# liuhatry/xflow

Hardware: AMD Instinct MI355X
Metric: samples/sec (whole node) + logloss, LR-FTRL Criteo-1TB shape at 1/2/4/8 MI355X (higher is better)
Workload: dtype fp32; 1 GPU; model=LR-FTRL, global_batch=262144, seq_len=39, parallelism=dp1+table-shard1, rows_per_gpu=262144, nnz_per_row=39, slices=1, grad_layout=unique_lr, hashed_features=1000000000, table_slots_per_gpu=2147483648, backend=hip:gfx950:0, a2a_transport=none, input_overlap=False, table_growths=0

## Files before the change

### csrc/engine/engine.cpp

```cpp
#include <cstdlib>
#include "xflow/engine.h"

#include <algorithm>
#include <atomic>
#include <chrono>
#include <cmath>
#include <cstdio>
#include <cstring>
#include <thread>
#include <fstream>
#include <stdexcept>
#include <string>

namespace xflow {

namespace {

uint64_t next_pow2(uint64_t v) {
  uint64_t p = 1;
  while (p < v) p <<= 1;
  return p;
}

constexpr char kMagic[8] = {'X', 'F', 'L', 'O', 'W', 'T', 'B', '1'};
// ... 252 lines not shown
}

void Engine::set_reduction(FwdArgs& fa) const {
  fa.trash_pos = (u32)scratch_.cap;
  if (!red_pairs_) return;
  if (rec_on_) fa.red_records = rec_count_;
  if (red_vmax_) {
    fa.red_vmax = red_vmax_ + vmax_parity_;
    fa.red_vmax_next = red_vmax_ + (vmax_parity_ ^ 1);
    fa.red_dup = red_vmax_ + 2 + vmax_parity_;
    fa.red_dup_next = red_vmax_ + 2 + (vmax_parity_ ^ 1);
    if (mdup_rec_) {
      fa.mdup.rec = mdup_rec_;
      fa.mdup.vmax = red_vmax_ + 4;
      fa.mdup.n = red_vmax_ + 6;
      fa.mdup.acc = mdup_acc_;
      fa.mdup.claim = mdup_claim_;
      fa.mdup.cap = (int64_t)mdup_claim_.capacity();
      fa.mdup.ew = mdup_ew_;
    }
    vmax_parity_ ^= 1;
  }
  fa.red_bcap = ws_->bcap;
  fa.red_cap = scratch_.cap;
  fa.red_nsub = red_nsub_;
  fa.red_pairs = red_pairs_;
  fa.red_sorted = red_sorted_;
  fa.red_sorted_words = (int64_t)red_sorted_.capacity();
  fa.red_hist = red_hist_;
  fa.red_tot = red_tot_;
  fa.red_count = red_count_;
  fa.red_groups = red_groups_;
  fa.red_nb = red_nb_;
  fa.red_maxb = red_maxb_;
  fa.red_rowv = red_rowv_;
}

PullArgs Engine::pull_args(const u64* keys, const int64_t* n_dev, int64_t n, bool insert,
                           u32* out_slot) const {
  PullArgs pa;
  pa.table = table_;
  pa.opt = cfg_.opt;
  pa.keys = keys;
  pa.n_dev = n_dev;
  pa.n_host = n_dev ? 0 : n;
  pa.n_max = n;
  pa.insert = insert;
  pa.out_slot = out_slot;
  return pa;
}

ApplyArgs Engine::apply_args(const u64* keys, const u32* slots, const int64_t* n_dev, int64_t n,
                             int S) const {
  ApplyArgs aa;
  aa.table = table_;
  aa.opt = cfg_.opt;
  aa.keys = keys;
  aa.slots = slots;
  aa.n_dev = n_dev;
  aa.n_host = n_dev ? 0 : n;
  aa.n_max = n;
  aa.S = S;
  aa.pstride = pstride();
  aa.P = cfg_.model.P();
  aa.fm_D = cfg_.model.v_dim;
  return aa;
}

FwdArgs Engine::train_fwd_args(const BatchView& b, const u32* pos, int S) const {
  FwdArgs fa;
  fa.batch = b;
  fa.pos = pos;
  fa.wpull = wpull_;
  fa.grad = grad_;
  fa.stats = stats_;
  fa.model = cfg_.model;
  fa.S = S;
  fa.fx_bad = overflow_;
  fa.fm_vals = fm_vals_;
  set_reduction(fa);
  return fa;
}

FwdArgs Engine::eval_fwd_args(const BatchView& b, float* pctr) const {
  FwdArgs fa;
  fa.batch = b;
  fa.pos = ws_->pos;
  fa.wpull = wpull_;
  fa.pctr = pctr;
  fa.stats = stats_ + 1;
  fa.model = cfg_.model;
  fa.fm_vals = fm_vals_;
  return fa;
}

int Engine::slices_of(const BatchView& b) const {
  if (b.slice_rows <= 0 || b.rows <= 0) return 1;
  return (int)((b.rows + b.slice_rows - 1) / b.slice_rows);
}

const int32_t* Engine::slice_rows_dev(const BatchView& b, int S) {
  if (b.rows == cached_rows_ && b.slice_rows == cached_slice_rows_ && S == cached_S_)
    return slice_rows_;
  const int ng = slice_groups(S);
  slice_rows_.reserve(*be_, (size_t)ng * kSliceGroup, (size_t)ng * kSliceGroup);
  const int64_t sr = b.slice_rows > 0 ? b.slice_rows : b.rows;
  for (int g = 0; g < ng; ++g) {
    int32_t h[kSliceGroup];
    const int n = ng == 1 ? S : kSliceGroup;
    for (int l = 0; l < n; ++l) {
      const int64_t s = (int64_t)g * kSliceGroup + l;
      int64_t rem = s < S ? b.rows - s * sr : 0;
      rem = rem < 0 ? 0 : rem;
      h[l] = (int32_t)(rem < sr ? (rem > 0 ? rem : 1) : sr);
    }
    be_->upload_small(slice_rows_ + (int64_t)g * kSliceGroup, h, sizeof(int32_t) * n);
  }
  cached_S_ = S;
  cached_rows_ = b.rows;
  cached_slice_rows_ = b.slice_rows;
  return slice_rows_;
}

BatchView Engine::group_view(const BatchView& b, int S, int k, const u32*& pos) const {
  if (slice_groups(S) == 1) return b;
  const int64_t sr = b.slice_rows > 0 ? b.slice_rows : b.rows;
  int64_t r0 = (int64_t)k * kSliceGroup * sr;
  r0 = r0 < b.rows ? r0 : b.rows;
  int64_t n = (int64_t)kSliceGroup * sr;
  n = n < b.rows - r0 ? n : b.rows - r0;
  BatchView g = b;
  g.rows = n;
  if (b.row_ptr) {
    g.row_ptr = b.row_ptr + r0;
    g.labels = b.labels + r0;
    return g;
  }
  const int64_t off = b.col_stride > 0 ? r0 : r0 * b.nnz_per_row;
  g.keys = b.keys + off;
  if (b.fgid) g.fgid = b.fgid + off;
  g.labels = b.labels + r0;
  g.nnz = n * b.nnz_per_row;
  pos += off;
  return g;
}

void Engine::ensure_inv() {
  if (ws_->inv) return;
  ws_->inv.alloc(*be_, scratch_.cap + 16);
  be_->memset(ws_->inv + scratch_.cap, 0xFF, 16 * sizeof(u32));
}

void Engine::dedup_(const BatchView& b, int parts, u64* uniq_keys_out, bool want_inv,
                    int64_t* n_copy, bool lead) {
  if (b.nnz > cfg_.max_nnz) throw std::invalid_argument("batch nnz exceeds max_nnz");
  if (b.rows > cfg_.max_rows) throw std::invalid_argument("batch rows exceed max_rows");
  if (b.col_stride > 0 && (b.row_ptr || b.col_stride < b.rows || b.nnz != b.rows * b.nnz_per_row))
    throw std::invalid_argument("field-major batch needs fixed nnz_per_row and col_stride >= rows");
  if (b.nnz == 0) {
    be_->memset(ws_->n_uniq, 0, sizeof(int64_t));
    return;
  }
  const int hb = be_->is_gpu() && parts == 1
                     ? table_.seg_log2 + table_.level + (table_.split > 0 ? 1 : 0)
                     : 0;
  if (parts != scratch_.parts || hb != scratch_.home_bits) {
    be_->fill_u64(scratch_.keys, kEmptyKey, scratch_.cap);
    be_->memset(scratch_.claims, 0, sizeof(unsigned long long));
    scratch_.parts = parts;
    scratch_.home_bits = hb;
  }
  if (++scratch_.epoch > kStampEpochs) {
    scratch_.epoch = 1;
    be_->memset(scratch_.stamps, 0, scratch_.cap);
    if (scratch_.ctl) {
      const unsigned long long z = 0ull;
      be_->upload_small(scratch_.ctl + 4, &z, sizeof(z));
    }
  }
  scratch_.grow = 0.0f;
  if (scratch_.ctl && nnz_seen_ > 0 && b.nnz > nnz_seen_)
    scratch_.grow = (float)((double)b.nnz / (double)nnz_seen_);
  if (b.nnz > nnz_seen_) nnz_seen_ = b.nnz;
  DedupOut o;
  o.pos = ws_->pos;
  o.uniq_keys = uniq_keys_out ? uniq_keys_out : uniq_keys_;
  o.uniq_pos = ws_->uniq_pos;
  o.n_uniq = ws_->n_uniq;
  o.overflow = overflow_;
  o.block_counts = block_counts_;
  o.inv = want_inv ? ws_->inv.get() : nullptr;
  o.n_uniq_copy = n_copy;
  o.cap_out = ws_->bcap;
  o.lead = lead;
  be_->dedup(b.keys, b.nnz, scratch_, o);
}


const char* grad_path_name(GradPath g) {
  switch (g) {
    case GradPath::kCsr: return "csr";
    case GradPath::kUniqueLR: return "unique_lr";
    case GradPath::kUniqueFmBC: return "unique_fm_bc";
    case GradPath::kUniqueRows: return "unique_rows";
    case GradPath::kSlotSums: return "slot_sums";
    case GradPath::kSlotRows: return "slot_rows";
  }
  return "?";
}

StepInputs Engine::step_inputs() const {
  StepInputs in;
  in.gpu = be_->is_gpu();
  in.remaps = be_->remaps_positions();
  in.red_pairs = red_pairs_ != nullptr;
  in.red_rowv = red_rowv_ != nullptr;
  in.fm_vals = fm_vals_;
  in.csr = cfg_.csr;
  in.sum_slices = cfg_.sum_slices;
  in.kind = cfg_.model.kind;
  in.fm_math = cfg_.model.fm_math;
  in.L = table_.L;
  in.scratch_cap = (double)scratch_.cap;
  in.max_nnz = (double)cfg_.max_nnz;
  in.max_rows = (double)cfg_.max_rows;
  in.pstride = pstride();
  in.slice_cap = slice_cap_;
  in.kdim = cfg_.model.kernel_dim();
  in.lead_handoff = cfg_.lead_handoff;
  in.red_rank = cfg_.red_rank;
  in.red_local = cfg_.red_local;
  in.red_apply = cfg_.red_apply;
  return in;
}

StepPlan plan_step(const StepInputs& in, int S) {
  constexpr double k32 = 4294967295.0;
  StepPlan p;
  p.S = S;
  const TableLayout& L = in.L;
  const bool lr16_slot = in.kind == kLR && L.lr16();
  const bool fm_std = in.kind == kFM && in.fm_math == kFmStandard;
  const bool mvm = in.kind == kMVM && in.kdim >= 2;
  const int vnv = fm_std ? 1 + in.kdim : in.kdim;
  const bool std_ok = (fm_std || mvm) && in.gpu && in.red_rowv &&
                      std::ceil(in.max_rows / fmstd_block(vnv - 1)) <= kSegMaxGroups;
  const int csr_min = (in.kind == kLR || fm_std) ? 8 : 4;
  if (in.csr && S >= csr_min && !in.sum_slices && in.red_pairs && in.remaps &&
      (lr16_slot || in.fm_vals || std_ok)) {
    int sl = 0;
    while ((1 << sl) < S) ++sl;
    const int nv = in.fm_vals ? 2 : (std_ok ? vnv : 1);
    if (sl <= red_shift(nv) && in.max_nnz * (double)(1 << sl) < k32) {
      p.csr_slog2 = sl;
      p.csr_rows = std_ok;
      p.grad = GradPath::kCsr;
      return p;
    }
  }
  p.groups = Engine::slice_groups(S);
  p.Sf = p.groups > 1 ? Engine::kSliceGroup : S;
  p.masks = p.Sf > 1 && !in.sum_slices;
  const bool lr16_ok = in.gpu && lr16_slot && in.red_pairs && in.scratch_cap < k32;
  p.upos = in.remaps && in.red_pairs &&
           (p.Sf > 1 || in.kind == kMVM || (in.kind == kFM && in.fm_math == kFmStandard));
  const double key_bound = p.upos ? in.max_nnz : in.scratch_cap;
  const bool red_masks = in.red_pairs && key_bound * in.slice_cap * in.pstride < k32 &&
                         (in.kind == kLR || in.kind == kFM ||
                          (in.kind == kMVM && in.red_rowv && in.kdim >= 2));
  p.lr16 = lr16_ok && (p.Sf == 1 || (p.masks && red_masks));
  p.lr16s = lr16_ok && p.Sf > 1 && !p.lr16;
  p.uqm = p.masks && red_masks;
  p.fmu = in.fm_vals && (p.Sf == 1 || p.uqm);
  p.fm_keep_w = in.fm_vals && p.groups > 1;
  const bool rows_ok = in.gpu && in.red_pairs && key_bound * in.pstride * in.slice_cap < k32;
  p.mvmu = rows_ok && p.Sf == 1 && in.kind == kMVM && in.red_rowv && in.kdim >= 2;
  p.fsu = rows_ok && (p.Sf == 1 || p.uqm) && in.kind == kFM && in.fm_math == kFmStandard;
  p.rowu = p.mvmu || p.fsu;
  p.grpst = in.gpu && L.opt == kFTRL && L.P > 1;
  p.uq = p.Sf > 1 && (p.lr16 || p.fmu || p.fsu);
  p.grad = p.lr16 ? GradPath::kUniqueLR
           : p.fmu ? GradPath::kUniqueFmBC
           : p.rowu ? GradPath::kUniqueRows
           : p.lr16s ? GradPath::kSlotSums
           : GradPath::kSlotRows;
  p.lead = in.lead_handoff && in.gpu && in.kind == kLR && S == 1 && in.red_pairs && !p.upos &&
           in.field_major && in.rows >= kLeadTile && std::fmod(in.rows, (double)kLeadTile) == 0.0 &&
           in.fields >= 1.0 && in.fields <= kLeadMaxFields && in.scratch_cap < 2147483648.0;
  p.red_rank = in.red_rank && in.gpu && S == 1 && in.red_pairs && !p.upos && (p.lr16 || p.fmu);
  p.red_local = in.red_local && p.lead;
  p.red_apply = in.red_apply && p.red_local && p.red_rank && p.lr16;
  return p;
}

void Engine::train_step_csr(const BatchView& b, int S, int slog2) {
  const int32_t* srows = slice_rows_dev(b, S);
  const bool fm = fm_vals_;
  const bool rows = csr_full_rows();
  const int ew = rows ? csr_row_words(table_.L.P) : 0;
  float* stash = fm || rows ? grp_nz_.ensure(*be_, 2 * (size_t)cfg_.max_nnz * table_.L.P)
                            : lr_nz_.ensure(*be_, 2 * (size_t)cfg_.max_nnz);
  PullArgs pa = begin_fused_step(b, true, true);
  pa.out_nz = stash;
  be_->table_pull(pa);

  csr_forward_backward(b, slog2, srows, true);

  ApplyArgs aa = apply_args(uniq_keys_, uniq_slot_, ws_->n_uniq, b.nnz, S);
  aa.fm_compact = fm;
  aa.nz_stash = stash;
  aa.csr_off = csr_off_;
  aa.csr_cnt = csr_cnt_;
  aa.csr_ent = rows ? static_cast<const void*>(csr_vent_.get()) : red_pairs_.get();
  aa.csr_ew = ew;
  aa.csr_long = S > 16 ? csr_long_list(b.nnz) : nullptr;
  aa.csr_long_cap = (int64_t)csr_long_.capacity();
  attach_snapshot(aa);
  be_->table_apply(aa);
  end_step();
}

void Engine::csr_forward_backward(const BatchView& b, int slog2, const int32_t* srows,
                                  bool normalise) {
  csr_off_.ensure(*be_, (size_t)cfg_.max_nnz);
  csr_cnt_.ensure(*be_, (size_t)cfg_.max_nnz);
  FwdArgs fa = train_fwd_args(b, ws_->pos, 1 << slog2);
  fa.agg_ok = true;
  fa.red_nuq = ws_->n_uniq;
  fa.fm_compact = fm_vals_;
  fa.red_csr.off = csr_off_;
  fa.red_csr.cnt = csr_cnt_;
  fa.red_csr.ent = red_pairs_;
  fa.red_csr.slog2 = slog2;
  fa.red_csr.rows = normalise ? srows : nullptr;
  if (csr_full_rows()) {
    const int ew = csr_row_words(table_.L.P);
    fa.red_csr.ent = csr_vent_.ensure(*be_, (size_t)cfg_.max_nnz * ew);
    fa.red_csr.P = table_.L.P;
    fa.red_csr.ew = ew;
  }
  be_->forward_backward(fa);
  ++csr_steps_;
}

u32* Engine::csr_long_list(int64_t n) {
  if (!be_->is_gpu()) return nullptr;
  const int64_t need = 2 * n + (int64_t)(2u << 20) + 4 * 65536;
  csr_long_.reserve(*be_, (size_t)need, (size_t)(need + n / 4));
  return csr_long_;
}

void Engine::w_forward_backward_csr(const BatchView& b, const float* pulled, int64_t n_send,
                                    int S_global, int wb, bool pack, u32* cnt_out, void* ent_out,
                                    const int64_t* counts, int world, bool encoded,
                                    int64_t* totals_out) {
  use_worker_set(wb);
  const int St = S_global > 0 ? S_global : slices_of(b);
  const int sl = csr_slog2(St);
  if (sl < 0 || St < slices_of(b) || St > cfg_.max_slices)
    throw std::invalid_argument("w_forward_backward_csr: S_global off the CSR path");
  if (b.nnz > 0 && !ws_->inv_valid)
    throw std::logic_error("w_forward_backward_csr: needs the partitioned dedup's inv");
  be_->remap_pos(ws_->pos, b.nnz, ws_->inv, (u32)scratch_.cap);
  be_->scatter_rows(pulled, wpull_, nullptr, nullptr, n_send, vstride_);
  csr_forward_backward(b, sl, slice_rows_dev(b, St), true);
  last_nsend_ = n_send;
  if (!pack) return;
  csr_doff_.ensure(*be_, (size_t)cfg_.max_nnz + 1);
  be_->scan_u32(csr_cnt_, csr_doff_, ws_->n_uniq, cfg_.max_nnz);
  be_->csr_pack(csr_off_, csr_cnt_, csr_full_rows() ? static_cast<const void*>(csr_vent_.get()) : red_pairs_.get(),
                csr_doff_, ws_->n_uniq, cfg_.max_nnz, ent_out, csr_entry_bytes());
  be_->copy_d2d(cnt_out, csr_cnt_, sizeof(u32) * (size_t)n_send);
  be_->csr_totals(counts, world, encoded, csr_doff_, totals_out);
}

template <typename Source>
void Engine::apply_by_source(const ApplyArgs& base, const std::vector<int64_t>& src_offsets,
                             int buf, bool stash, const char* need_weights, Source source) {
  const SrvBuf& sb = srv_[buf];
  size_t first_src = 0;
  while (first_src + 1 < src_offsets.size() && src_offsets[first_src + 1] <= src_offsets[first_src])
    ++first_src;
  for (size_t src = 0; src + 1 < src_offsets.size(); ++src) {
    const int64_t o = src_offsets[src], c = src_offsets[src + 1] - o;
    if (c <= 0) continue;
    ApplyArgs aa = base;
    aa.keys = base.keys + o;
    aa.slots = base.slots + o;
    aa.n_host = c;
    aa.n_max = c;
    source(aa, o, c);
    if (aa.fm_compact) {
      aa.pulled = pulled_weights(buf, o);
      if (!aa.pulled && src > first_src) throw std::logic_error(need_weights);
    }
    if (stash) aa.nz_stash = sb.nz + 2 * o;
    stash = false;
    attach_snapshot(aa);
    be_->table_apply(aa);
  }
}

void Engine::s_apply_csr(const u64* recv_keys, const u32* recv_cnt, const void* recv_ent,
                         const std::vector<int64_t>& src_offsets, int S, int buf) {
  if (buf < 0 || buf >= kSrvBufs) throw std::invalid_argument("server buffer must be in [0, kSrvBufs)");
  SrvBuf& sb = srv_[buf];
  sb.keys = nullptr;
  bool stash = sb.nz_fresh;
  stale_stashes();
  const u32* off = csr_off_;
  const u32* cnt = csr_cnt_;
  const void* ent = csr_full_rows() ? static_cast<const void*>(csr_vent_.get()) : red_pairs_.get();
  const int64_t n = src_offsets.empty() ? 0 : src_offsets.back();
  if (n > sb.n) throw std::invalid_argument("s_apply_csr: offsets beyond pull");
  mark_stale_buffer(sb, recv_keys, n);
  if (recv_cnt) {
    csr_roff_.reserve(*be_, (size_t)n + 1, (size_t)(n + n / 4 + 1024));
    be_->scan_u32(recv_cnt, csr_roff_, nullptr, n);
    off = csr_roff_;
    cnt = recv_cnt;
    ent = recv_ent;
  }
  ApplyArgs base = apply_args(recv_keys, sb.slots, nullptr, 0, S);
  base.fm_compact = fm_vals_;
  base.csr_ew = csr_full_rows() ? csr_row_words(table_.L.P) : 0;
  base.csr_ent = ent;
  apply_by_source(base, src_offsets, buf, stash,
                  "s_apply_csr: compact FM rows of several sources need s_pull's weights",
                  [&](ApplyArgs& aa, int64_t o, int64_t c) {
                    aa.csr_off = off + o;
                    aa.csr_cnt = cnt + o;
                    aa.csr_long = S > 16 ? csr_long_list(c) : nullptr;
                    aa.csr_long_cap = (int64_t)csr_long_.capacity();
                  });
}

void Engine::csr_debug(std::vector<u32>& off, std::vector<u32>& cnt, std::vector<u32>& words) {
  off.clear();
  cnt.clear();
  words.clear();
  if (!csr_off_) return;
  const int64_t n = n_unique();
  off.resize((size_t)n);
  cnt.resize((size_t)n);
  be_->copy_d2h(off.data(), csr_off_, sizeof(u32) * (size_t)n);
  be_->copy_d2h(cnt.data(), csr_cnt_, sizeof(u32) * (size_t)n);
  u64 end = 0;
  for (int64_t i = 0; i < n; ++i) end = std::max<u64>(end, (u64)off[i] + cnt[i]);
  const bool rows = csr_vent_ && csr_full_rows();
  const int w = rows ? csr_row_words(table_.L.P) : csr_entry_bytes() / 4;
  words.resize((size_t)end * w);
  if (end) be_->copy_d2h(words.data(), rows ? static_cast<const void*>(csr_vent_.get()) : red_pairs_.get(),
                         sizeof(u32) * (size_t)end * w);
}

std::vector<u64> Engine::unique_keys() {
  std::vector<u64> k((size_t)n_unique());
  if (!k.empty()) be_->copy_d2h(k.data(), uniq_keys_, sizeof(u64) * k.size());
  return k;
}

Engine::RedGeometry Engine::red_geometry(int S, int64_t nuq) {
  RedGeometry g;
  const bool fm_std = cfg_.model.kind == kFM && cfg_.model.fm_math == kFmStandard;
  const bool mvm = cfg_.model.kind == kMVM && cfg_.model.kernel_dim() >= 2;
  const int kd = cfg_.model.kernel_dim();
  const int nv = fm_vals_ ? 2 : (fm_std ? 1 + kd : (mvm ? kd : 1));
  int sl = 0;
  while ((1 << sl) < S) ++sl;
  g.base = red_shift(nv);
  g.maxb = red_maxb_ > 0 ? red_maxb_ : kRedMaxBuckets;
  g.nsub = red_nsub_;
  g.nb = red_nb_;
  g.nuq = nuq >= 0 ? nuq : n_unique();
  const u64 dests = (u64)g.nuq << sl;
  int sh = g.base;
  while (((dests + (1ull << sh) - 1) >> sh) > (u64)kRedMaxBuckets) ++sh;
  if (g.maxb > kRedMaxBuckets && sh - g.base >= 2)
    while (sh > g.base && ((dests + (1ull << (sh - 1)) - 1) >> (sh - 1)) <= (u64)g.maxb) --sh;
  const int min_shift = csr_full_rows() ? kCsrVecMinShift : 0;
  g.shift = sh < min_shift ? min_shift : sh;
  const u64 n = (dests + (1ull << g.shift) - 1) >> g.shift;
  g.needed = (int64_t)n;
  g.buckets = n < (u64)g.nb ? (int)n : g.nb;
  return g;
}

void Engine::train_step(const BatchView& b) {
  stale_stashes();
  use_worker_set(0);
  const int S = slices_of(b);
  if (S > cfg_.max_slices) throw std::invalid_argument("batch has more slices than max_slices");
  if (cfg_.sum_slices && slice_groups(S) > 1)
    throw std::invalid_argument("sum_slices: at most 32 slices per step (ordered pushes: any count)");
  const StepPlan P = plan(S, b.rows, b.nnz_per_row, !b.row_ptr && b.col_stride > 0 && b.col_stride == b.rows);
  if (P.grad == GradPath::kCsr) {
    train_step_csr(b, S, P.csr_slog2);
    return;
  }
  const int ng = P.groups;
  const int ps = pstride();
  const bool masks = P.masks;
  const int32_t* srows = slice_rows_dev(b, S);
  const bool uqm = P.uqm, fm_keep_w = P.fm_keep_w, uq = P.uq, upos = P.upos;
  const double key_bound = upos ? (double)cfg_.max_nnz : (double)scratch_.cap;
  struct {
    float* buf = nullptr;
    int width = 0;
    bool normalised = false;
    bool pull_zeroes = true;
  } uo;
  const size_t un = (size_t)cfg_.max_nnz;
  if (P.red_apply) {
    uo = {nullptr, 1, true, false};
  } else if (P.lr16) {
    uo = {lr_grad_.ensure(*be_, un * slice_cap_), 1, true, true};
  } else if (P.fmu) {
    uo = {fm_grad_.ensure(*be_, 2 * un * slice_cap_), 2, true, true};
  } else if (P.rowu) {
    uo = {row_grad_.ensure(*be_, un * ps * (P.fsu ? slice_cap_ : 1)), ps, false,
          !(P.fsu && P.Sf == 1)};
  }
  float* nz = P.lr16 || P.lr16s ? lr_nz_.ensure(*be_, 2 * un)
              : P.grpst         ? grp_nz_.ensure(*be_, 2 * un * table_.L.P)
                                : nullptr;
  if (fm_keep_w) fm_w_.ensure(*be_, un * ps);
  if (uq) lr_mask_.ensure(*be_, un);

  PullArgs pa = begin_fused_step(b, upos || (uo.buf && !P.red_rank), upos, P.lead);
  if (fm_keep_w) pa.out_w = fm_w_;
  pa.out_nz = nz;
  if (uo.buf && uo.pull_zeroes) {
    pa.zero_out = uo.buf;
    pa.zero_width = uo.width;
  }
  if (uq) {
    pa.zero_out = reinterpret_cast<float*>(lr_mask_.get());
    pa.zero_width = 1;
  }
  be_->table_pull(pa);

  for (int k = 0; k < ng; ++k) {
    const u32* posk = ws_->pos;
    const BatchView bk = group_view(b, S, k, posk);
    const int Sg = group_slices(S, k);
    const int32_t* srk = srows + (int64_t)k * kSliceGroup;
    const bool stash = k == 0;

    FwdArgs fa = train_fwd_args(bk, posk, Sg);
    fa.agg_ok = key_bound * Sg * ps < 4294967295.0;
    if (upos) fa.red_nuq = ws_->n_uniq;
    fa.lead = P.lead;
    fa.red_local = P.red_local;
    if (uq) fa.red_masks = lr_mask_;
    else if (uqm) fa.red_masks = tmask_;
    else if (masks) be_->slice_masks(bk, posk, tmask_);
    fa.fm_compact = fa.red_pairs && fa.agg_ok && cfg_.model.kind == kFM &&
                    cfg_.model.fm_math == kFmReference;
    if (fm_vals_ && !fa.fm_compact) throw std::logic_error("train_step: compact FM rows need the reduction");
    if (uo.buf || P.red_apply) {
      fa.red_out = uo.buf;
      fa.red_inv = upos || P.red_rank ? nullptr : ws_->inv.get();
      if (P.red_rank) {
        fa.red_rank_offs = block_counts_;
        fa.red_rank_stamps = scratch_.stamps;
        fa.red_rank_epoch = scratch_.epoch;
      }
      if (uo.normalised) fa.red_rows = srk;
    }
    if (P.red_apply) {
      fa.red_apply_words = table_.words;
      fa.red_apply_slots = uniq_slot_;
      fa.red_apply_nz = nz;
      fa.red_apply_ftrl = cfg_.opt.ftrl;
      attach_snapshot(fa, b.nnz);
    }
    be_->forward_backward(fa);
    if (P.red_apply) continue;

    ApplyArgs aa = apply_args(uniq_keys_, uniq_slot_, ws_->n_uniq, b.nnz, Sg);
    aa.sum_slices = cfg_.sum_slices;
    aa.fm_compact = fa.fm_compact;
    if (fm_keep_w) aa.pulled = fm_w_;
    aa.nz_stash = stash ? nz : nullptr;
    if (uo.buf) {
      aa.grads = uo.buf;
      aa.gstride = uo.width;
      aa.slice_rows = uo.normalised ? nullptr : srk;
    } else {
      aa.grads = grad_;
      aa.grad_map = upos ? nullptr : ws_->uniq_pos.get();
      aa.zero_after = true;
      aa.slice_rows = srk;
    }
    if (uq) {
      aa.masks = lr_mask_;
      aa.masks_clear = k + 1 < ng;
    } else if (masks) {
      aa.masks = tmask_;
      aa.masks_rw = tmask_;
    }
    attach_snapshot(aa);
    be_->table_apply(aa);
  }
  end_step();
}

PullArgs Engine::begin_fused_step(const BatchView& b, bool want_inv, bool upos, bool lead) {
  if (want_inv) ensure_inv();
  if (lead && upos) throw std::logic_error("begin_fused_step: leader handoff with unique positions");
  dedup_(b, 1, nullptr, want_inv, nullptr, lead);
  ws_->inv_valid = false;
  if (upos) be_->remap_pos(ws_->pos, b.nnz, ws_->inv, (u32)scratch_.cap);
  guard_inserts(b.nnz);
  delta_mark(uniq_keys_, ws_->n_uniq, b.nnz);
  PullArgs pa = pull_args(uniq_keys_, ws_->n_uniq, b.nnz, true, uniq_slot_);
  pa.admit = admit_;
  pa.out_vals = wpull_;
  pa.out_map = upos ? nullptr : ws_->uniq_pos.get();
  pa.pstride = pstride();
  pa.fm_vals = fm_vals_;
  return pa;
}

void Engine::eval_step(const BatchView& b, float* pctr) {
  use_worker_set(0);
  dedup_(b);
  PullArgs pa = pull_args(uniq_keys_, ws_->n_uniq, b.nnz, false, uniq_slot_);
  pa.out_vals = wpull_;
  pa.out_map = ws_->uniq_pos;
  pa.pstride = pstride();
  pa.fm_vals = fm_vals_;
  be_->table_pull(pa);
  be_->forward_backward(eval_fwd_args(b, pctr));
}

void Engine::ensure_host_staging(int64_t n) {
  if (!host_keys_dev_.reserve(*be_, (size_t)n, (size_t)n)) return;
  host_vals_dev_.alloc(*be_, (size_t)n * cfg_.model.P());
  host_slots_dev_.alloc(*be_, (size_t)n);
}

void Engine::push_host(const std::vector<u64>& keys, const std::vector<float>& grads) {
  stale_stashes();
  const int64_t n = (int64_t)keys.size();
  const int P = cfg_.model.P();
  if ((int64_t)grads.size() != n * P) throw std::invalid_argument("push_host: grads != keys*P");
  if (n == 0) return;
  guard_inserts(n);
  ensure_host_staging(n);
  be_->copy_h2d(host_keys_dev_, keys.data(), sizeof(u64) * n);
  be_->copy_h2d(host_vals_dev_, grads.data(), sizeof(float) * n * P);
  delta_mark(host_keys_dev_, nullptr, n);
  be_->table_pull(pull_args(host_keys_dev_, nullptr, n, true, host_slots_dev_));
  ApplyArgs aa = apply_args(host_keys_dev_, host_slots_dev_, nullptr, 1, 1);
  aa.pstride = P;
  for (int64_t i = 0; i < n; ++i) {
    aa.slots = host_slots_dev_ + i;
    aa.grads = host_vals_dev_ + i * P;
    be_->table_apply(aa);
  }
  be_->synchronize();
}

void Engine::prefill(int64_t n, uint64_t seed) {
  if (n > 0) guard_inserts(n);
  if (n < 0 || (uint64_t)n > table_.cap - table_.cap / 16)
    throw std::invalid_argument("prefill: at most 15/16 of the table's slots");
  stale_stashes();
  if (n > 0) delta_needs_full_ = true;
  be_->table_prefill(table_, n, seed);
  be_->synchronize();
  (void)table_size();
}

std::vector<float> Engine::pull_host(const std::vector<u64>& keys) {
  const int64_t n = (int64_t)keys.size();
  const int P = cfg_.model.P();
  std::vector<float> out((size_t)n * P);
  if (n == 0) return out;
  ensure_host_staging(n);
  be_->copy_h2d(host_keys_dev_, keys.data(), sizeof(u64) * n);
  PullArgs pa = pull_args(host_keys_dev_, nullptr, n, false, host_slots_dev_);
  pa.out_vals = host_vals_dev_;
  pa.pstride = P;
  be_->table_pull(pa);
  be_->copy_d2h(out.data(), host_vals_dev_, sizeof(float) * n * P);
  return out;
}

void Engine::w_prepare(const BatchView& b, int world, int64_t* counts_out, u64* send_keys_out,
                       int wb, int64_t seq) {
  if (be_->partitioned_dedup() && (world < 1 || world > kMaxParts))
    throw std::runtime_error("w_prepare: world size " + std::to_string(world) + " outside [1, " +
                             std::to_string(kMaxParts) + "]");
  if (world <= 1) seq = -1;
  use_worker_set(wb);
  if (slices_of(b) > cfg_.max_slices)
    throw std::invalid_argument("batch has more slices than max_slices");
  if (b.nnz == 0) {
    const int64_t c = b.rows == 0 ? -1 : 0;
    be_->fill_u64(reinterpret_cast<u64*>(counts_out), (u64)(seq >= 0 ? encode_count(c, seq) : c),
                  (size_t)(world > 0 ? world : 1));
    be_->memset(ws_->n_uniq, 0, sizeof(int64_t));
    ws_->inv_valid = false;
    ws_->send_map = ws_->uniq_pos;
    return;
  }
  if (be_->partitioned_dedup()) {
    if (red_pairs_ && (cfg_.model.kind == kLR || fm_vals_ || csr_full_rows())) ensure_inv();
    dedup_(b, world, send_keys_out, true, world == 1 ? counts_out : nullptr);
    ws_->inv_valid = ws_->inv != nullptr;
    if (world > 1) be_->partition_counts(scratch_, block_counts_, ws_->n_uniq, counts_out, seq);
    ws_->send_map = ws_->uniq_pos;
    return;
  }
  dedup_(b);
  ws_->inv_valid = false;
  BucketArgs ba;
  ba.uniq_keys = uniq_keys_;
  ba.uniq_pos = ws_->uniq_pos;
  ba.n_dev = ws_->n_uniq;
  ba.n_max = b.nnz;
  ba.world = world;
  ba.counts = counts_out;
  ba.send_keys = send_keys_out;
  ba.send_pos = ws_->send_pos;
  ba.scratch = bucket_ws_;
  ba.seq = seq;
  be_->bucket(ba);
  ws_->send_map = ws_->send_pos;
}

void Engine::ensure_server_capacity(int64_t n, int buf) {
  if (buf < 0 || buf >= kSrvBufs) throw std::invalid_argument("server buffer must be in [0, kSrvBufs)");
  SrvBuf& sb = srv_[buf];
  const size_t cap = (size_t)(n + n / 4 + 1024);
  if (n <= 0 || !sb.slots.reserve(*be_, (size_t)n, cap)) return;
  if (lr16_layout()) sb.nz.alloc(*be_, 2 * cap);
}

bool Engine::lr16_layout() const {
  const TableLayout& L = table_.L;
  return be_->is_gpu() && L.lr16();
}

void Engine::w_forward(const BatchView& b, const float* pulled, int64_t n_send, float* pctr,
                       int wb) {
  use_worker_set(wb);
  be_->scatter_rows(pulled, wpull_, ws_->send_map, nullptr, n_send, vstride_);
  be_->forward_backward(eval_fwd_args(b, pctr));
}

void Engine::s_pull(const u64* recv_keys, int64_t n, float* out_vals, bool insert, int buf,
                    const std::vector<int64_t>& src_offsets, bool keep_weights) {
  ensure_server_capacity(n, buf);
  SrvBuf& sb = srv_[buf];
  sb.n = n;
  sb.vals = out_vals;
  sb.w_valid = false;
  sb.grp = SrcGroups();
  sb.keys = insert && n > 0 ? recv_keys : nullptr;
  if (n == 0) return;
  if (insert) {
    guard_inserts(n);
    group_entries(recv_keys, n, buf, src_offsets);
    delta_mark(recv_keys, nullptr, n);
  }
// ... 800 lines not shown
```

### csrc/hip/hip_backend.hip

```cpp
#include <hip/hip_runtime.h>

#include <cstdlib>
#include <cstring>
#include <vector>

#include "hip_util.h"
#include "kernels.h"
#include "xflow/backend.h"

namespace xflow {

namespace {

class HipBackend final : public Backend {
 public:
  explicit HipBackend(int device) : device_(device) {
    XF_HIP_CHECK(hipSetDevice(device_));
    XF_HIP_CHECK(hipStreamCreateWithFlags(&own_stream_, hipStreamNonBlocking));
    stream_ = own_stream_;
    XF_HIP_CHECK(hipMalloc(&counter_, sizeof(unsigned long long)));
  }
  ~HipBackend() override {
    hipSetDevice(device_);
    if (copy_stream_) (void)hipStreamSynchronize(copy_stream_);
// ... 7 lines not shown
    if (scan_tiles_) {
      (void)hipDeviceSynchronize();
      (void)hipFreeAsync(scan_tiles_, own_stream_);
      (void)hipStreamSynchronize(own_stream_);
    }
    if (split_marks_) (void)hipFree(split_marks_);
    if (own_stream_) (void)hipStreamDestroy(own_stream_);
  }

  void stage_begin(int s) override {
    if (!copy_stream_) {
      XF_HIP_CHECK(hipStreamCreateWithFlags(&copy_stream_, hipStreamNonBlocking));
      for (int i = 0; i < 2; ++i) {
        XF_HIP_CHECK(hipEventCreateWithFlags(&ev_copied_[i], hipEventDisableTiming));
        XF_HIP_CHECK(hipEventCreateWithFlags(&ev_used_[i], hipEventDisableTiming));
      }
    }
    if (copied_pending_[s]) {
      XF_HIP_CHECK(hipEventSynchronize(ev_copied_[s]));
      copied_pending_[s] = false;
    }
    waited_used_[s] = false;
  }
  void* stage_pinned(int s, size_t bytes) override {
    if (bytes > pinned_cap_[s]) {
      if (pinned_[s]) XF_HIP_CHECK(hipHostFree(pinned_[s]));
      pinned_cap_[s] = bytes + bytes / 4;
      XF_HIP_CHECK(hipHostMalloc(&pinned_[s], pinned_cap_[s], hipHostMallocDefault));
    }
    return pinned_[s];
  }
  void stage_copy(int s, void* dst, size_t off, size_t bytes) override {
    if (!bytes) return;
    if (used_pending_[s] && !waited_used_[s]) {
      XF_HIP_CHECK(hipStreamWaitEvent(copy_stream_, ev_used_[s], 0));
      waited_used_[s] = true;
    }
    XF_HIP_CHECK(hipMemcpyAsync(dst, static_cast<char*>(pinned_[s]) + off, bytes,
                                hipMemcpyHostToDevice, copy_stream_));
  }
  void stage_commit(int s) override {
    XF_HIP_CHECK(hipEventRecord(ev_copied_[s], copy_stream_));
    XF_HIP_CHECK(hipStreamWaitEvent(stream_, ev_copied_[s], 0));
    copied_pending_[s] = true;
  }
  void stage_release(int s) override {
    XF_HIP_CHECK(hipEventRecord(ev_used_[s], stream_));
    used_pending_[s] = true;
  }

  bool is_gpu() const override { return true; }
  std::string name() const override { return "hip:gfx950:" + std::to_string(device_); }

  void* alloc(size_t bytes) override {
    void* p = nullptr;
    if (bytes == 0) bytes = 16;
    XF_HIP_CHECK(hipSetDevice(device_));
    XF_HIP_CHECK(hipMalloc(&p, bytes));
    return p;
  }
  void free(void* p) override {
    if (p) (void)hipFree(p);
  }
  void* alloc_stream(size_t bytes) override {
    void* p = nullptr;
    if (bytes == 0) bytes = 16;
    XF_HIP_CHECK(hipSetDevice(device_));
    XF_HIP_CHECK(hipMallocAsync(&p, bytes, stream_));
    return p;
  }
  void free_stream(void* p) override {
    if (p) XF_HIP_CHECK(hipFreeAsync(p, stream_));
  }
  void memset(void* p, int v, size_t bytes) override {
    if (bytes) XF_HIP_CHECK(hipMemsetAsync(p, v, bytes, stream_));
  }
  void fill_u64(u64* p, u64 v, size_t n) override { hip::launch_fill_u64(p, v, n, stream_); }
  void copy_h2d(void* dst, const void* src, size_t bytes) override {
    if (bytes) XF_HIP_CHECK(hipMemcpyAsync(dst, src, bytes, hipMemcpyHostToDevice, stream_));
    XF_HIP_CHECK(hipStreamSynchronize(stream_));
  }
  void copy_d2h(void* dst, const void* src, size_t bytes) override {
    if (bytes) XF_HIP_CHECK(hipMemcpyAsync(dst, src, bytes, hipMemcpyDeviceToHost, stream_));
    XF_HIP_CHECK(hipStreamSynchronize(stream_));
  }
  void copy_d2h_async(void* dst, const void* src, size_t bytes) override {
    if (bytes) XF_HIP_CHECK(hipMemcpyAsync(dst, src, bytes, hipMemcpyDeviceToHost, stream_));
  }
  void copy_h2d_async(void* dst, const void* src, size_t bytes) override {
    if (bytes) XF_HIP_CHECK(hipMemcpyAsync(dst, src, bytes, hipMemcpyHostToDevice, stream_));
  }
  void* staging_alloc(size_t bytes) override {
    void* p = nullptr;
    XF_HIP_CHECK(hipHostMalloc(&p, bytes ? bytes : 16, hipHostMallocDefault));
    return p;
  }
  void staging_free(void* p) override {
    if (p) (void)hipHostFree(p);
  }
  void copy_d2d(void* dst, const void* src, size_t bytes) override {
    if (bytes) XF_HIP_CHECK(hipMemcpyAsync(dst, src, bytes, hipMemcpyDeviceToDevice, stream_));
  }
  void download_small(void* dst, const void* src, size_t bytes) override {
    hip::launch_download_small(dst, src, bytes, stream_);
  }
  void upload_small(void* dst, const void* src, size_t bytes) override {
    hip::launch_upload_small(dst, src, bytes, stream_);
  }
  void synchronize() override { XF_HIP_CHECK(hipStreamSynchronize(stream_)); }
  size_t free_memory() const override {
    size_t fr = 0, tot = 0;
    XF_HIP_CHECK(hipSetDevice(device_));
    XF_HIP_CHECK(hipMemGetInfo(&fr, &tot));
    return fr;
  }
  void snapshot(HostSnap* dst, const u32* mon, unsigned long long seq) override {
    hip::launch_snapshot(dst, mon, seq, stream_);
  }
  void* host_alloc(size_t bytes) override {
    void* p = nullptr;
    XF_HIP_CHECK(hipHostMalloc(&p, bytes ? bytes : 16, hipHostMallocCoherent));
    std::memset(p, 0, bytes ? bytes : 16);
    return p;
  }
  void host_free(void* p) override {
    if (p) (void)hipHostFree(p);
  }
  void* event_create() override {
    hipEvent_t e = nullptr;
    XF_HIP_CHECK(hipEventCreateWithFlags(&e, hipEventDisableTiming));
    return e;
  }
  void event_destroy(void* e) override {
    if (e) (void)hipEventDestroy(static_cast<hipEvent_t>(e));
  }
  void event_record(void* e) override {
    XF_HIP_CHECK(hipEventRecord(static_cast<hipEvent_t>(e), stream_));
  }
  bool event_done(void* e) override {
    const hipError_t r = hipEventQuery(static_cast<hipEvent_t>(e));
    if (r == hipErrorNotReady) return false;
    XF_HIP_CHECK(r);
    return true;
  }
  void set_stream(void* s) override { stream_ = reinterpret_cast<hipStream_t>(s); }
  void* stream() const override { return stream_; }
  void bind_thread() override { XF_HIP_CHECK(hipSetDevice(device_)); }

  void table_clear(const TableView& t) override { hip::launch_table_clear(t, stream_); }
  void dedup(const u64* keys, int64_t nnz, ScratchView s, DedupOut o) override {
    hip::launch_dedup(keys, nnz, s, o, stream_);
  }
  void table_pull(const PullArgs& a) override { hip::launch_table_pull(a, stream_); }
  void table_apply(const ApplyArgs& a) override { hip::launch_table_apply(a, stream_); }
  void forward_backward(const FwdArgs& a) override { hip::launch_forward_backward(a, stream_); }
  void slice_masks(const BatchView& b, const u32* pos, u32* tmask) override {
    hip::launch_slice_masks(b, pos, tmask, stream_);
  }
  void parse_text(const TextParseArgs& a) override { hip::launch_parse_text(a, stream_); }
  bool remaps_positions() const override { return true; }
  void remap_pos(u32* pos, int64_t nnz, const u32* inv, u32 none) override {
    hip::launch_remap_pos(pos, nnz, inv, none, stream_);
  }
  void bucket(const BucketArgs&) override {
    throw std::logic_error("bucket: not on the HIP backend");
  }
  bool partitioned_dedup() const override { return true; }
  void partition_counts(const ScratchView& s, const u32* chunk_offsets, const int64_t* n_uniq,
                        int64_t* counts, int64_t seq) override {
    hip::launch_partition_counts(s, chunk_offsets, n_uniq, counts, seq, stream_);
  }
  bool owner_grouping() const override { return true; }
  void owner_group(const OwnerGroupArgs& a) override { hip::launch_owner_group(a, stream_); }
  void gather_grads(const GatherGradArgs& a) override { hip::launch_gather_grads(a, stream_); }
  bool csr_exchange() const override { return true; }
  void scan_u32(const u32* in, u32* out, const int64_t* n_dev, int64_t n_max) override {
    const size_t words = (size_t)(n_max / 4096 + 4);
    if (words > scan_tiles_words_) {
      if (scan_tiles_) free_stream(scan_tiles_);
      scan_tiles_words_ = words + words / 2;
      scan_tiles_ = static_cast<u32*>(alloc_stream(scan_tiles_words_ * sizeof(u32)));
    }
    hip::launch_scan_u32(in, out, n_dev, n_max, scan_tiles_, stream_);
  }
  void csr_pack(const u32* off, const u32* cnt, const void* src, const u32* doff,
                const int64_t* n_dev, int64_t n_max, void* dst, int entry_bytes) override {
    hip::launch_csr_pack(off, cnt, src, doff, n_dev, n_max, dst, entry_bytes, stream_);
  }
  void csr_totals(const int64_t* counts, int world, bool encoded, const u32* doff,
                  int64_t* totals) override {
    hip::launch_csr_totals(counts, world, encoded, doff, totals, stream_);
  }
  void scatter_rows(const float* src, float* dst, const u32* map, const int64_t* n_dev,
                    int64_t n_max, int width, float* zero_out, int zero_width) override {
    hip::launch_scatter_rows(src, dst, map, n_dev, n_max, width, zero_out, zero_width, stream_);
  }
  void synth_batch(const SynthArgs& a) override { hip::launch_synth(a, stream_); }
  void unpack_block(const UnpackArgs& a) override { hip::launch_unpack_block(a, stream_); }
  void field_major(const void* src, void* dst, int64_t rows, int F, int elem_bytes,
                   bool widen) override {
    hip::launch_field_major(src, dst, rows, F, elem_bytes, widen, stream_);
  }
  void shuffle_rows(const ShuffleArgs& a) override {
    check_shuffle_args(a);
    if (!a.src.row_ptr) {
      hip::launch_shuffle_fixed(a, stream_);
      return;
    }
    if (a.src.rows <= 0) {
      memset(a.row_ptr, 0, sizeof(int32_t));
      return;
    }
    if (!a.len) throw std::invalid_argument("shuffle_rows: a CSR batch needs the len workspace");
    hip::launch_shuffle_len(a, stream_);
    scan_u32(a.len, reinterpret_cast<u32*>(a.row_ptr), nullptr, a.src.rows);
    hip::launch_shuffle_gather(a, stream_);
  }
  void cross_rows(const CrossArgs& a) override {
    check_cross_args(a);
    if (a.src.row_ptr) hip::launch_cross_csr(a, stream_);
    else if (a.src.col_stride > 0) hip::launch_cross_cols(a, stream_);
    else hip::launch_cross_fixed(a, stream_);
  }
  int64_t table_export(const TableView& t, u64* keys_out, u32* words_out,
                       int64_t max_rows) override {
    hip::launch_table_export(t, keys_out, words_out, max_rows, counter_, stream_);
    unsigned long long n = 0;
    copy_d2h(&n, counter_, sizeof(n));
    return (int64_t)n;
  }
  void table_import(const TableView& t, const u64* keys, const u32* words, int64_t n) override {
    hip::launch_table_import(t, keys, words, n, stream_);
  }
  void table_prefill(const TableView& t, int64_t n, u64 seed) override {
    hip::launch_table_prefill(t, n, seed, stream_);
  }
  void table_split(const TableView& t, u64 s0, u64 k) override {
    ensure_marks(t, k);
    hip::launch_table_split(t, s0, k, split_marks_, stream_);
  }
  void table_prune(const TableView& t, const OptSpec& o, float max_n,
                   unsigned long long* dropped) override {
    const int g = t.seg_log2;
    const u64 nseg = t.cap >> g;
    const u64 per_launch = g >= 28 ? 1 : (1ull << (28 - g));
    XF_HIP_CHECK(hipMemsetAsync(counter_, 0, sizeof(unsigned long long), stream_));
    for (u64 s0 = 0; s0 < nseg; s0 += per_launch) {
      const u64 k = nseg - s0 < per_launch ? nseg - s0 : per_launch;
      ensure_marks(t, k);
      hip::launch_table_prune(t, o, max_n, s0, k, split_marks_, counter_, stream_);
    }
    hip::launch_table_prune_finish(t.size, dropped, counter_, stream_);
  }

  void* table_reserve(size_t max_bytes, bool growable) override {
    int vmm = 0;
    XF_HIP_CHECK(hipSetDevice(device_));
    (void)hipDeviceGetAttribute(&vmm, hipDeviceAttributeVirtualMemoryManagementSupported, device_);
    const char* env = std::getenv("XFLOW_TABLE_VMM");
    if ((env && env[0] == '0') || !growable) vmm = 0;
    vm_on_ = false;
    if (vmm) {
      vm_prop_ = hipMemAllocationProp{};
      vm_prop_.type = hipMemAllocationTypePinned;
      vm_prop_.location.type = hipMemLocationTypeDevice;
      vm_prop_.location.id = device_;
      size_t gran = 0;
      if (hipMemGetAllocationGranularity(&gran, &vm_prop_, hipMemAllocationGranularityRecommended) ==
              hipSuccess && gran > 0) {
        vm_gran_ = gran;
        vm_max_ = (max_bytes + gran - 1) / gran * gran;
        void* p = nullptr;
        if (hipMemAddressReserve(&p, vm_max_, gran, nullptr, 0) == hipSuccess) {
          vm_on_ = true;
          vm_base_ = p;
          vm_committed_ = 0;
          return p;
        }
      }
      (void)hipGetLastError();
    }
    fb_bytes_ = 0;
    fb_max_ = max_bytes;
    return nullptr;
  }
  void* table_commit(void* base, size_t bytes) override {
    if (vm_on_) {
      if (bytes <= vm_committed_) return base;
      if (bytes > vm_max_) throw std::runtime_error("xflow: table beyond its reserved range");
      size_t want = (bytes + vm_gran_ - 1) / vm_gran_ * vm_gran_;
      size_t ahead = (vm_committed_ / 8 + vm_gran_ - 1) / vm_gran_ * vm_gran_;
      if (vm_committed_ && want < vm_committed_ + ahead) want = vm_committed_ + ahead;
      if (want > vm_max_) want = vm_max_;
      {
        size_t fr = 0, tot = 0;
        if (hipMemGetInfo(&fr, &tot) == hipSuccess && want - vm_committed_ + (512u << 20) > fr)
          want = (bytes + vm_gran_ - 1) / vm_gran_ * vm_gran_;
      }
      const size_t add = want - vm_committed_;
      char* at = static_cast<char*>(vm_base_) + vm_committed_;
      hipMemGenericAllocationHandle_t h;
      XF_HIP_CHECK(hipMemCreate(&h, add, &vm_prop_, 0));
      XF_HIP_CHECK(hipMemMap(at, add, 0, h, 0));
      hipMemAccessDesc acc{};
      acc.location = vm_prop_.location;
      acc.flags = hipMemAccessFlagsProtReadWrite;
// ... 130 lines not shown
```

### csrc/hip/kernels.h

```cpp
#pragma once

#include <hip/hip_runtime.h>

#include "xflow/backend.h"

namespace xflow {
namespace hip {

void launch_dedup(const u64* keys, int64_t nnz, ScratchView s, DedupOut o, hipStream_t st);
void launch_remap_pos(u32* pos, int64_t nnz, const u32* inv, u32 none, hipStream_t st);
void launch_partition_counts(const ScratchView& s, const u32* chunk_offsets,
                             const int64_t* n_uniq, int64_t* counts, int64_t seq, hipStream_t st);

void launch_table_pull(const PullArgs& a, hipStream_t st);

void launch_table_apply(const ApplyArgs& a, hipStream_t st);
void launch_owner_group(const OwnerGroupArgs& a, hipStream_t st);

void launch_gather_grads(const GatherGradArgs& a, hipStream_t st);
void launch_scatter_rows(const float* src, float* dst, const u32* map, const int64_t* n_dev,
                         int64_t n_max, int width, float* zero_out, int zero_width,
                         hipStream_t st);
void launch_scan_u32(const u32* in, u32* out, const int64_t* n_dev, int64_t n_max, u32* tiles,
                     hipStream_t st);
void launch_csr_pack(const u32* off, const u32* cnt, const void* src, const u32* doff,
                     const int64_t* n_dev, int64_t n_max, void* dst, int entry_bytes,
                     hipStream_t st);
void launch_csr_totals(const int64_t* counts, int world, bool encoded, const u32* doff,
                       int64_t* totals, hipStream_t st);

void launch_fill_u64(u64* p, u64 v, size_t n, hipStream_t st);
void launch_upload_small(void* dst, const void* src, size_t bytes, hipStream_t st);
void launch_download_small(void* host_dst, const void* src, size_t bytes, hipStream_t st);
void launch_snapshot(HostSnap* dst, const u32* mon, unsigned long long seq, hipStream_t st);
void launch_table_clear(const TableView& t, hipStream_t st);
void launch_table_export(const TableView& t, u64* keys_out, u32* words_out, int64_t max_rows,
                         unsigned long long* counter, hipStream_t st);
void launch_table_import(const TableView& t, const u64* keys, const u32* words, int64_t n,
                         hipStream_t st);
void launch_table_prefill(const TableView& t, int64_t n, u64 seed, hipStream_t st);
void launch_table_split(const TableView& t, u64 s0, u64 k, u64* marks, hipStream_t st);
void launch_table_prune(const TableView& t, const OptSpec& o, float max_n, u64 s0, u64 k,
                        u64* marks, unsigned long long* count, hipStream_t st);
void launch_table_prune_finish(unsigned long long* size, unsigned long long* total,
                               const unsigned long long* count, hipStream_t st);
void launch_table_nonzero(const TableView& t, const OptSpec& o, unsigned long long* counter,
                          hipStream_t st);
void launch_delta_mark(u32* bits, int L, const u64* keys, const int64_t* n_dev, int64_t n_host,
                       int64_t n_max, hipStream_t st);
void launch_table_export_marked(const TableView& t, const u32* bits, int L, u64* keys_out,
                                u32* words_out, int64_t max_rows, unsigned long long* counter,
                                hipStream_t st);
void launch_delta_popcount(const u32* bits, int L, unsigned long long* counter, hipStream_t st);

void launch_unpack_block(const UnpackArgs& a, hipStream_t st);
void launch_field_major(const void* src, void* dst, int64_t rows, int F, int elem_bytes, bool widen,
                        hipStream_t st);

void launch_shuffle_fixed(const ShuffleArgs& a, hipStream_t st);
void launch_shuffle_len(const ShuffleArgs& a, hipStream_t st);
void launch_shuffle_gather(const ShuffleArgs& a, hipStream_t st);

void launch_cross_fixed(const CrossArgs& a, hipStream_t st);
void launch_cross_cols(const CrossArgs& a, hipStream_t st);
void launch_cross_csr(const CrossArgs& a, hipStream_t st);

void launch_forward_backward(const FwdArgs& a, hipStream_t st);
void launch_slice_masks(const BatchView& b, const u32* pos, u32* tmask, hipStream_t st);

void launch_parse_text(const TextParseArgs& a, hipStream_t st);

void launch_eval_metrics(const float* pctr, const float* labels, int64_t n, EvalMetrics* out,
                         hipStream_t st);
void launch_eval_grouped(const float* pctr, const float* labels, const u64* groups, int64_t n,
                         GroupedEval* out, GroupTable* table, hipStream_t st);
void launch_row_group_keys(const BatchView& b, int field, u64* out, hipStream_t st);

void launch_synth(const SynthArgs& a, hipStream_t st);

}
}
```

### csrc/hip/kernels_dedup.hip

```cpp
#include "table_common.h"

namespace xflow {
namespace hip {

__device__ __forceinline__ u64 active_cap(const ScratchView& sv) {
  return sv.ctl ? (u64)sv.ctl[0] : sv.cap;
}

__device__ __forceinline__ u64 batch_cap(const ScratchView& sv) {
  return sv.ctl ? (u64)sv.ctl[3] : sv.cap;
}

__device__ __forceinline__ bool batch_spilled(const ScratchView& sv) {
  return sv.ctl && sv.ctl[4] == (unsigned long long)sv.epoch;
}

__global__ void k_scratch_maybe_clear(u64* __restrict__ skeys, u64 cap,
                                      const unsigned long long* __restrict__ claims,
                                      u64 rebuild_at, const unsigned long long* __restrict__ ctl) {
  u64 n = cap;
  if (ctl) {
    n = ctl[2];
    if (n == 0) return;
  } else if (*claims <= rebuild_at) {
    return;
  }
  const u64 stride = (u64)gridDim.x * blockDim.x;
  for (u64 s = (u64)blockIdx.x * blockDim.x + threadIdx.x; s < n; s += stride)
    skeys[s] = kEmptyKey;
}

__global__ void k_scratch_claims_reset(unsigned long long* claims, u64 rebuild_at,
                                       unsigned long long* ctl) {
  if (ctl) {
    if (ctl[2]) {
      ctl[0] = ctl[2];
      ctl[2] = 0ull;
      *claims = 0ull;
    }
  } else if (*claims > rebuild_at) {
    *claims = 0ull;
  }
}

__global__ void k_scratch_grow(unsigned long long* __restrict__ ctl, u64 cap_alloc, float grow) {
  const double need = (double)kScratchHeadroom * (double)ctl[1] * (double)grow;
  u64 want = kScratchMinCap;
  while ((double)want < need && want < cap_alloc) want <<= 1;
  if (want > cap_alloc) want = cap_alloc;
  ctl[2] = want > ctl[0] ? want : 0ull;
}

constexpr int kDedupItems = 4;
constexpr int kDedupChunk = kBlock * kDedupItems;
constexpr int kDedupLog2 = 11;
static_assert((1 << kDedupLog2) == 2 * kDedupChunk, "LDS dedup table sizing");
static_assert(kDedupChunk == kLeadTile, "the handoff's tile is the dedup chunk");

template <bool kLead>
__global__ void __launch_bounds__(kBlock) k_dedup_insert(const u64* __restrict__ keys, int64_t nnz,
                                                         ScratchView sv, u32* __restrict__ pos,
                                                         u32* __restrict__ overflow) {
  constexpr u32 kL = 1u << kDedupLog2;
  __shared__ u64 t_key[kL];
  u64* __restrict__ skeys = sv.keys;
  const u64 cap = active_cap(sv), mask = cap - 1;
  const u32 parts = (u32)sv.parts;
  const u64 R = parts > 1 ? cap / parts : cap;
  const int clog = 63 - __clzll((long long)cap);
  const int hshift = sv.home_bits > clog ? sv.home_bits - clog : 0;
  const int64_t base = (int64_t)blockIdx.x * kDedupChunk + threadIdx.x;
  for (u32 i = threadIdx.x; i < kL; i += kBlock) t_key[i] = kEmptyKey;
  u64 k[kDedupItems], s[kDedupItems];
  u32 h[kDedupItems];
#pragma unroll
  for (int j = 0; j < kDedupItems; ++j) {
    int64_t i = base + (int64_t)j * kBlock;
    k[j] = i < nnz ? sanitize_key(keys[i]) : 0ull;
    const u64 f = fmix64(k[j]);
    s[j] = parts > 1 ? (u64)((u32)(f >> 32) % parts) * R + (((f & 0xffffffffull) * R) >> 32)
                     : (f >> hshift) & mask;
    h[j] = (u32)(f >> (64 - kDedupLog2));
  }
  __syncthreads();
  u32 lead = 0;
#pragma unroll
  for (int j = 0; j < kDedupItems; ++j) {
    if (base + (int64_t)j * kBlock >= nnz) continue;
    u32 x = h[j];
    while (true) {
      const u64 prev = atomicCAS((unsigned long long*)&t_key[x], (unsigned long long)kEmptyKey,
                                 (unsigned long long)k[j]);
      if (prev == kEmptyKey) {
        lead |= 1u << j;
        break;
      }
      if (prev == k[j]) break;
      x = (x + 1) & (kL - 1);
    }
    h[j] = x;
  }
  __syncthreads();
  u64 cur[kDedupItems];
#pragma unroll
  for (int j = 0; j < kDedupItems; ++j) cur[j] = (lead >> j) & 1u ? skeys[s[j]] : k[j];
  unsigned int claimed = 0;
#pragma unroll
  for (int j = 0; j < kDedupItems; ++j) {
    if (!((lead >> j) & 1u)) continue;
    u64 sj = s[j], c = cur[j];
    u64 n = 0;
    while (c != k[j]) {
      if (c == kEmptyKey) {
        u64 prev = atomicCAS((unsigned long long*)&skeys[sj], (unsigned long long)kEmptyKey,
                             (unsigned long long)k[j]);
        if (prev == kEmptyKey) {
          ++claimed;
          break;
        }
        if (prev == k[j]) break;
      }
      if (++n >= R) {
        if (sv.ctl && parts == 1 && cap < sv.cap && n == R) {
          sv.ctl[4] = sv.epoch;
          const u64 Z = sv.cap - cap;
          sj = cap + fmix64(k[j]) % Z;
          c = skeys[sj];
          for (u64 m = 0; c != k[j]; ) {
            if (c == kEmptyKey) {
              u64 prev = atomicCAS((unsigned long long*)&skeys[sj], (unsigned long long)kEmptyKey,
                                   (unsigned long long)k[j]);
              if (prev == kEmptyKey) {
                ++claimed;
                break;
              }
              if (prev == k[j]) break;
            }
            if (++m >= Z) {
              sj = sv.cap;
              break;
            }
            if (++sj == sv.cap) sj = cap;
            c = skeys[sj];
          }
          if (sj < sv.cap) break;
        }
        *overflow = 1u;
        sj = sv.cap;
        break;
      }
      if (parts > 1) {
        ++sj;
        if (sj % R == 0) sj -= R;
      } else {
        sj = (sj + 1) & mask;
      }
      c = skeys[sj];
    }
    XF_DASSERT(sj <= sv.cap);
    if constexpr (kLead) {
      XF_DASSERT(sj < kLeadBit);
      t_key[h[j]] = sj | ((u64)(j * kBlock + (int)threadIdx.x) << 32);
    } else {
      t_key[h[j]] = sj;
    }
    if (sj < sv.cap) sv.stamps[sj] = (unsigned char)sv.epoch;
  }
  __syncthreads();
#pragma unroll
  for (int j = 0; j < kDedupItems; ++j) {
    int64_t i = base + (int64_t)j * kBlock;
    if (i >= nnz) continue;
    const u64 e = t_key[h[j]];
    if constexpr (kLead) pos[i] = (lead >> j) & 1u ? (u32)e : kLeadBit | (u32)(e >> 32);
    else pos[i] = (u32)e;
  }
  block_count_add<kBlock>(sv.claims, claimed);
}

constexpr int kCompactItems = 16;
constexpr int kCompactChunk = kBlock * kCompactItems;
static_assert(kCompactChunk == 1 << kCompactChunkLog2, "k_red_sum ranks slots by these chunks");

__device__ __forceinline__ unsigned int compact_hits(const ScratchView& sv, u64 base, u64 cap,
                                                     unsigned int& cnt) {
  unsigned int hit = 0;
  cnt = 0;
  if (base >= cap) return 0;
  const uint4 q = *reinterpret_cast<const uint4*>(sv.stamps + base);
  const u32 w[4] = {q.x, q.y, q.z, q.w};
  const u32 e = sv.epoch & 0xFFu;
#pragma unroll
  for (int j = 0; j < 16; ++j) hit |= (unsigned int)(((w[j >> 2] >> (8 * (j & 3))) & 0xFFu) == e) << j;
  cnt = __popc(hit);
  return hit;
}

__global__ void __launch_bounds__(kBlock) k_compact_count(ScratchView sv,
                                                          unsigned int* __restrict__ counts) {
  const u64 base = (u64)blockIdx.x * kCompactChunk + (u64)threadIdx.x * kCompactItems;
  unsigned int cnt;
  compact_hits(sv, base, batch_spilled(sv) ? sv.cap : active_cap(sv), cnt);
  unsigned int tot;
  block_exclusive_scan<kBlock>(cnt, &tot);
  if (threadIdx.x == 0) counts[blockIdx.x] = tot;
}

constexpr u64 kCarryRebuildEighths = 3;
static_assert(kCarryRebuildEighths <= 4, "stale claims <= cur / 2 at a batch start");

__global__ void __launch_bounds__(kScanBlock) k_compact_scan(
    unsigned int* __restrict__ counts, int nb, unsigned long long* __restrict__ n_out,
    unsigned long long* __restrict__ claims, unsigned long long* __restrict__ ctl,
    u64 cap_alloc, unsigned long long* __restrict__ n_copy,
    unsigned long long* __restrict__ cap_out, u32 epoch, bool carry_on) {
  if (ctl) {
    const u64 lim = ctl[4] == epoch ? cap_alloc : (u64)ctl[0];
    const u64 nbl = (lim + kCompactChunk - 1) / kCompactChunk;
    if (nbl < (u64)nb) nb = (int)nbl;
  }
  unsigned long long carry = 0;
  for (int c0 = 0; c0 < nb; c0 += kScanBlock) {
    int i = c0 + (int)threadIdx.x;
    unsigned int v = i < nb ? counts[i] : 0u;
    unsigned int tot;
    unsigned int ex = block_exclusive_scan<kScanBlock>(v, &tot);
    if (i < nb) counts[i] = (unsigned int)(carry + ex);
    carry += tot;
  }
  if (threadIdx.x == 0) {
    *n_out = carry;
    if (n_copy) *n_copy = carry;
    if (ctl) {
      const u64 mx = ctl[1] > carry ? ctl[1] : carry;
      ctl[1] = mx;
      u64 want = kScratchMinCap;
      while (want < kScratchHeadroom * mx && want < cap_alloc) want <<= 1;
      if (want > cap_alloc) want = cap_alloc;
      const u64 cur = ctl[0];
      const bool resize = want > cur || want * 4 <= cur;
      const u64 full_at = carry_on ? cur * kCarryRebuildEighths / 8 : cur / 2;
      const bool rebuild = *claims > full_at || resize;
      const bool keep = carry_on && rebuild && !resize && ctl[4] != epoch &&
                        carry * kScratchHeadroom <= cur;
      ctl[3] = cur;
      ctl[2] = rebuild ? want : 0ull;
      ctl[5] = keep ? 1ull : 0ull;
      if (rebuild) {
        ctl[0] = want;
        *claims = keep ? carry : 0ull;
        ctl[6] += 1ull;
        ctl[7] = keep ? carry : 0ull;
      }
    }
    if (cap_out) *cap_out = ctl && ctl[4] != epoch ? ctl[3] : cap_alloc;
  }
}

__global__ void __launch_bounds__(kBlock) k_compact_write(ScratchView sv,
                                                          const unsigned int* __restrict__ offs,
                                                          u64* __restrict__ uk,
                                                          u32* __restrict__ up,
                                                          u32* __restrict__ inv) {
  const u64 base = (u64)blockIdx.x * kCompactChunk + (u64)threadIdx.x * kCompactItems;
  unsigned int cnt;
  unsigned int hit = compact_hits(sv, base, batch_spilled(sv) ? sv.cap : batch_cap(sv), cnt);
  unsigned int tot;
  unsigned int ex = block_exclusive_scan<kBlock>(cnt, &tot);
  unsigned long long dst = (unsigned long long)offs[blockIdx.x] + ex;
  u32 iv[kCompactItems];
  u64 kv[kCompactItems];
  if (hit) {
    const ulonglong2* kp = reinterpret_cast<const ulonglong2*>(sv.keys + base);
#pragma unroll
    for (int q = 0; q < kCompactItems / 2; ++q) {
      const ulonglong2 v = kp[q];
      kv[2 * q] = v.x;
      kv[2 * q + 1] = v.y;
    }
  }
#pragma unroll
  for (int j = 0; j < kCompactItems; ++j) {
    iv[j] = 0xFFFFFFFFu;
    if (!(hit & (1u << j))) continue;
    u64 s = base + (u64)j;
    uk[dst] = kv[j];
    up[dst] = (u32)s;
    iv[j] = (u32)dst;
    ++dst;
  }
  if (inv && hit) {
    uint4* ip = reinterpret_cast<uint4*>(inv + base);
#pragma unroll
    for (int j = 0; j < kCompactItems / 4; ++j)
      ip[j] = make_uint4(iv[4 * j], iv[4 * j + 1], iv[4 * j + 2], iv[4 * j + 3]);
  }
  const u64 fresh = sv.ctl ? (u64)sv.ctl[2] : 0ull;
  if (base < fresh) {
    ulonglong2* kp = reinterpret_cast<ulonglong2*>(sv.keys + base);
    if (hit && sv.ctl[5]) {
#pragma unroll
      for (int j = 0; j < kCompactItems / 2; ++j)
        kp[j] = make_ulonglong2(hit & (1u << (2 * j)) ? kv[2 * j] : kEmptyKey,
                                hit & (1u << (2 * j + 1)) ? kv[2 * j + 1] : kEmptyKey);
    } else {
#pragma unroll
      for (int j = 0; j < kCompactItems / 2; ++j) kp[j] = make_ulonglong2(kEmptyKey, kEmptyKey);
    }
  }
}

constexpr int kRemapPer = 4;

__global__ void __launch_bounds__(kBlock) k_remap_pos(u32* __restrict__ pos, int64_t nnz,
                                                      const u32* __restrict__ inv, u32 none) {
  const int64_t i = ((int64_t)blockIdx.x * kBlock + threadIdx.x) * kRemapPer;
  auto map = [&](u32 u) { return u == 0xFFFFFFFFu ? none : u; };
  if (i + kRemapPer <= nnz) {
    uint4 p[kRemapPer / 4];
#pragma unroll
    for (int q = 0; q < kRemapPer / 4; ++q) p[q] = reinterpret_cast<const uint4*>(pos + i)[q];
    u32 u[kRemapPer];
#pragma unroll
    for (int q = 0; q < kRemapPer / 4; ++q) {
      u[4 * q] = inv[p[q].x];
      u[4 * q + 1] = inv[p[q].y];
      u[4 * q + 2] = inv[p[q].z];
      u[4 * q + 3] = inv[p[q].w];
    }
#pragma unroll
    for (int q = 0; q < kRemapPer / 4; ++q)
      reinterpret_cast<uint4*>(pos + i)[q] =
          make_uint4(map(u[4 * q]), map(u[4 * q + 1]), map(u[4 * q + 2]), map(u[4 * q + 3]));
  } else {
    for (int64_t j = i; j < nnz; ++j) pos[j] = map(inv[pos[j]]);
  }
}

void launch_remap_pos(u32* pos, int64_t nnz, const u32* inv, u32 none, hipStream_t st) {
  if (nnz <= 0) return;
  if (reinterpret_cast<uintptr_t>(pos) & 15) throw std::runtime_error("remap_pos: pos must be 16-byte aligned");
  const int64_t lanes = (nnz + kRemapPer - 1) / kRemapPer;
  hipLaunchKernelGGL(k_remap_pos, dim3((unsigned)((lanes + kBlock - 1) / kBlock)), dim3(kBlock), 0,
                     st, pos, nnz, inv, none);
  XF_HIP_CHECK(hipGetLastError());
}

constexpr int kPartBlock = 1024;

__global__ void __launch_bounds__(kPartBlock) k_partition_counts(
    ScratchView sv, const unsigned int* __restrict__ offs, const int64_t* __restrict__ n_uniq,
    int64_t* __restrict__ counts, int64_t seq) {
  __shared__ int64_t start[kMaxParts + 1];
  const u32 parts = (u32)sv.parts;
  const u64 R = batch_cap(sv) / parts;
  const int lane = threadIdx.x % kWave, w = threadIdx.x / kWave;
  for (u32 o = w; o <= parts; o += kPartBlock / kWave) {
    if (o == 0 || o == parts) {
      if (lane == 0) start[o] = o == 0 ? 0 : *n_uniq;
      continue;
    }
    const u64 b = (u64)o * R, c = b / kCompactChunk, c0 = c * kCompactChunk;
    unsigned int hits = 0;
    for (u64 q = c0 + (u64)lane * 64; q < c0 + (u64)lane * 64 + 64; ++q)
      hits += (q < b && sv.stamps[q] == (unsigned char)sv.epoch) ? 1u : 0u;
#pragma unroll
    for (int d = 32; d > 0; d >>= 1) hits += __shfl_xor(hits, d);
    if (lane == 0) start[o] = (int64_t)offs[c] + hits;
  }
  __syncthreads();
  for (u32 o = threadIdx.x; o < parts; o += kPartBlock) {
    XF_DASSERT(start[o + 1] >= start[o]);
    const int64_t c = start[o + 1] - start[o];
    counts[o] = seq >= 0 ? encode_count(c, seq) : c;
  }
}

void launch_partition_counts(const ScratchView& s, const u32* chunk_offsets,
                             const int64_t* n_uniq, int64_t* counts, int64_t seq, hipStream_t st) {
  if (s.parts < 2 || s.parts > kMaxParts) throw std::runtime_error("partition_counts: bad parts");
  hipLaunchKernelGGL(k_partition_counts, dim3(1), dim3(kPartBlock), 0, st, s, chunk_offsets,
                     n_uniq, counts, seq);
  XF_HIP_CHECK(hipGetLastError());
}

void launch_dedup(const u64* keys, int64_t nnz, ScratchView s, DedupOut o, hipStream_t st) {
  if (nnz <= 0) return;
  if (!s.ctl || s.grow > 0.0f) {
    if (s.ctl) hipLaunchKernelGGL(k_scratch_grow, dim3(1), dim3(1), 0, st, s.ctl, s.cap, s.grow);
    hipLaunchKernelGGL(k_scratch_maybe_clear, dim3(grid_for((int64_t)s.cap)), dim3(kBlock), 0, st,
                       s.keys, s.cap, s.claims, s.rebuild_at, s.ctl);
    hipLaunchKernelGGL(k_scratch_claims_reset, dim3(1), dim3(1), 0, st, s.claims, s.rebuild_at,
                       s.ctl);
  }
  int g1 = (int)((nnz + kDedupChunk - 1) / kDedupChunk);
  if (o.lead) {
    if (nnz % kDedupChunk || s.cap >= kLeadBit || s.parts != 1)
      throw std::runtime_error("dedup: the leader handoff needs whole tiles and < 2^31 slots");
    hipLaunchKernelGGL(k_dedup_insert<true>, dim3(g1), dim3(kBlock), 0, st, keys, nnz, s, o.pos,
                       o.overflow);
  } else {
    hipLaunchKernelGGL(k_dedup_insert<false>, dim3(g1), dim3(kBlock), 0, st, keys, nnz, s, o.pos,
                       o.overflow);
  }
  if (!o.block_counts) throw std::runtime_error("dedup: block_counts workspace missing");
  int g2 = (int)((s.cap + kCompactChunk - 1) / kCompactChunk);
  hipLaunchKernelGGL(k_compact_count, dim3(g2), dim3(kBlock), 0, st, s, o.block_counts);
  hipLaunchKernelGGL(k_compact_scan, dim3(1), dim3(kScanBlock), 0, st, o.block_counts, g2,
                     reinterpret_cast<unsigned long long*>(o.n_uniq), s.claims, s.ctl, s.cap,
                     reinterpret_cast<unsigned long long*>(o.n_uniq_copy), o.cap_out, s.epoch,
                     s.carry);
  hipLaunchKernelGGL(k_compact_write, dim3(g2), dim3(kBlock), 0, st, s, o.block_counts,
                     o.uniq_keys, o.uniq_pos, o.inv);
  XF_HIP_CHECK(hipGetLastError());
}

}
}
```

### csrc/hip/kernels_pull.hip

```cpp
#include "table_common.h"

namespace xflow {
namespace hip {

constexpr int kPullItems = 2;
constexpr int kPullChunk = kBlock * kPullItems;
constexpr int kLineSlots = 4;

__global__ void __launch_bounds__(kBlock) k_pull_lr16(TableView t, FtrlParams fp,
                                                      const u64* __restrict__ keys,
                                                      const int64_t* n_dev, int64_t n_host,
                                                      int64_t n_max, bool insert,
                                                      u32* __restrict__ out_slot,
                                                      float* __restrict__ out_vals,
                                                      const u32* __restrict__ out_map,
                                                      float2* __restrict__ out_nz,
                                                      float* __restrict__ zero_out) {
  const int64_t n = dev_count(n_dev, n_host, n_max);
  if ((int64_t)blockIdx.x * kPullChunk >= n) return;
  const u64 segm = (1ull << t.seg_log2) - 1;
  uint4* slots = reinterpret_cast<uint4*>(t.words);
  const int64_t base = (int64_t)blockIdx.x * kPullChunk + threadIdx.x;
  u64 key[kPullItems], s[kPullItems];
  uint4 v[kPullItems];
#pragma unroll
  for (int j = 0; j < kPullItems; ++j) {
    int64_t i = base + (int64_t)j * kBlock;
    key[j] = i < n ? sanitize_key(keys[i]) : 0ull;
    s[j] = table_home(t, fmix64(key[j]));
  }
#pragma unroll
  for (int j = 0; j < kPullItems; ++j) {
    int64_t i = base + (int64_t)j * kBlock;
    if (i < n) v[j] = slots[s[j]];
  }
  u32 orow[kPullItems];
#pragma unroll
  for (int j = 0; j < kPullItems; ++j) {
    int64_t i = base + (int64_t)j * kBlock;
    orow[j] = (out_map && i < n) ? out_map[i] : (u32)i;
  }
  unsigned int claims = 0;
#pragma unroll
  for (int j = 0; j < kPullItems; ++j) {
    int64_t i = base + (int64_t)j * kBlock;
    if (i >= n) continue;
    u32 slot = kNoSlot;
    float w = 0.0f;
    float2 nz = make_float2(0.0f, 0.0f);
    u64 sj = s[j];
    int q0 = (int)(sj & (kLineSlots - 1)), q1 = q0 + 1;
    uint4 ln[kLineSlots];
#pragma unroll
    for (int q = 0; q < kLineSlots; ++q) ln[q] = v[j];
    bool done = false;
    for (u64 c = 0; c < t.probe_limit && !done;) {
#pragma unroll
      for (int q = 0; q < kLineSlots; ++q) {
        if (q < q0 || q >= q1 || done || c + (u64)(q - q0) >= t.probe_limit) continue;
        const u64 cur = (u64)ln[q].x | ((u64)ln[q].y << 32);
        const u64 sq = (sj & ~(u64)(kLineSlots - 1)) + (u64)q;
        if (cur == key[j]) {
          slot = (u32)sq;
          nz = make_float2(__uint_as_float(ln[q].z), __uint_as_float(ln[q].w));
          w = ftrl_weight(nz.y, nz.x, fp);
          done = true;
        } else if (cur == kEmptyKey) {
          if (!insert) {
            done = true;
          } else {
            const u64 prev = atomicCAS(reinterpret_cast<unsigned long long*>(&slots[sq]),
                                       (unsigned long long)kEmptyKey, (unsigned long long)key[j]);
            if (prev == kEmptyKey) {
              ++claims;
              slot = (u32)sq;
              done = true;
            } else if (prev == key[j]) {
              slot = (u32)sq;
              done = true;
            }
          }
        }
      }
      if (done) break;
      c += (u64)(q1 - q0);
      if (q1 < kLineSlots) {
        q0 = q1;
      } else {
        sj = (sj & ~segm) | (((sj | (u64)(kLineSlots - 1)) + 1) & segm);
        q0 = 0;
      }
      q1 = kLineSlots;
      const uint4* line = slots + (sj & ~(u64)(kLineSlots - 1));
#pragma unroll
      for (int q = 0; q < kLineSlots; ++q)
        if (q >= q0) ln[q] = line[q];
    }
    if (insert && slot == kNoSlot) *t.overflow = 1u;
    if (out_slot) out_slot[i] = slot;
    if (out_vals) out_vals[out_map ? (int64_t)orow[j] : i] = w;
    if (out_nz) out_nz[i] = nz;
    if (zero_out) zero_out[i] = 0.0f;
  }
  block_count_add<kBlock>(t.size, claims);
}

__global__ void __launch_bounds__(kBlock) k_pull_generic(PullArgs a) {
  int64_t n = dev_count(a.n_dev, a.n_host, a.n_max);
  const TableView& t = a.table;
  const TableLayout& L = t.L;
  const int64_t stride = (int64_t)gridDim.x * blockDim.x;
  unsigned int claims = 0;
  for (int64_t i = (int64_t)blockIdx.x * blockDim.x + threadIdx.x; i < n; i += stride) {
    u64 key = sanitize_key(a.keys[i]);
    bool claimed = false;
    u32 slot = probe(t, key, a.insert, claimed);
    claims += claimed;
    if (a.out_slot) a.out_slot[i] = slot;
    if (a.out_vals) {
      float* dst = a.out_vals + (size_t)(a.out_map ? a.out_map[i] : i) * a.pstride;
      if (slot == kNoSlot) {
        for (int p = 0; p < L.P; ++p) dst[p] = absent_weight(key, p, L, a.opt);
      } else {
        const u32* sp = t.words + (u64)slot * L.stride;
        for (int p = 0; p < L.P; ++p) dst[p] = slot_weight(sp, key, p, L, a.opt);
      }
    }
  }
  block_count_add<kBlock>(t.size, claims);
}

constexpr int kProbeItems = 2;
__global__ void __launch_bounds__(kBlock) k_pull_probe(TableView t, const u64* __restrict__ keys,
                                                       const int64_t* n_dev, int64_t n_host,
                                                       int64_t n_max, bool insert,
                                                       u32* __restrict__ out_slot) {
  const int64_t n = dev_count(n_dev, n_host, n_max);
  const int64_t base = (int64_t)blockIdx.x * (kBlock * kProbeItems) + threadIdx.x;
  if ((int64_t)blockIdx.x * (kBlock * kProbeItems) >= n) return;
  unsigned int claims = 0;
#pragma unroll
  for (int j = 0; j < kProbeItems; ++j) {
    int64_t i = base + (int64_t)j * kBlock;
    if (i >= n) continue;
    bool claimed = false;
    out_slot[i] = probe(t, sanitize_key(keys[i]), insert, claimed);
    claims += claimed;
  }
  block_count_add<kBlock>(t.size, claims);
}

__global__ void __launch_bounds__(kBlock) k_pull_values(PullArgs a) {
  const int64_t n = dev_count(a.n_dev, a.n_host, a.n_max);
  const TableLayout& L = a.table.L;
  const PackedLane pl = packed_lane(L.P);
  const int p = pl.p;
  const int gbase = (threadIdx.x % kWave) - p;
  int64_t i = pl.on ? pl.first : n;
  RowPipe pipe;
  pipe.stride = pl.stride;
  pipe.n = n;
  pipe.start(a.out_slot, a.table.words, i, p, L);
  u32 om_nx = (a.out_map && i < n) ? a.out_map[i] : 0u;
  for (; i < n; i += pl.stride) {
    RowPre rp;
    const u32 slot = pipe.next(a.out_slot, a.table.words, i, p, L, rp);
    const u32 om = om_nx;
    if (a.out_map && i + pl.stride < n) om_nx = a.out_map[i + pl.stride];
    float v;
    if (slot == kNoSlot) {
      v = absent_weight(sanitize_key(a.keys[i]), p, L, a.opt);
    } else {
      v = state_weight(rp.key, rp.flag != 0u, rp.s0, rp.s1, p, L, a.opt);
    }
    if (a.out_nz)
      reinterpret_cast<float2*>(a.out_nz)[(size_t)i * L.P + p] =
          make_float2(slot != kNoSlot && rp.flag ? rp.s0 : -1.0f, slot != kNoSlot ? rp.s1 : 0.0f);
    if (a.out_w) {
      a.out_w[(size_t)i * a.pstride + p] = v;
      for (int c = L.P + p; c < a.pstride; c += L.P) a.out_w[(size_t)i * a.pstride + c] = 0.0f;
    }
    if (a.zero_out)
      for (int c = p; c < a.zero_width; c += L.P) a.zero_out[(size_t)i * a.zero_width + c] = 0.0f;
    if (!a.out_vals) continue;
    const size_t row = a.out_map ? (size_t)om : (size_t)i;
    if (a.fm_vals) {
      float sv = 0.0f, qv = 0.0f;
      for (int j = L.p_w; j < L.P; ++j) {
        const float x = __shfl(v, gbase + j);
        sv += x;
        qv += x * x;
      }
      if (p == 0) reinterpret_cast<float4*>(a.out_vals)[row] = make_float4(v, sv, qv, 0.0f);
    } else {
      a.out_vals[row * a.pstride + p] = v;
      for (int c = L.P + p; c < a.pstride; c += L.P) a.out_vals[row * a.pstride + c] = 0.0f;
    }
  }
}

constexpr int kAdmitItems = 2;
constexpr int kAdmitChunk = kBlock * kAdmitItems;

__device__ __forceinline__ void admit_bump(u32* __restrict__ word, int shift, u32 seen) {
  while (((seen >> shift) & 0xFFu) != 0xFFu) {
    const u32 prev = atomicCAS(word, seen, seen + (1u << shift));
    if (prev == seen) break;
    seen = prev;
  }
}

__global__ void __launch_bounds__(kBlock) k_admit_count(AdmitView av,
                                                        const u64* __restrict__ keys,
                                                        const int64_t* n_dev, int64_t n_host,
                                                        int64_t n_max,
                                                        const u32* __restrict__ slots) {
  const int64_t n = dev_count(n_dev, n_host, n_max);
  if ((int64_t)blockIdx.x * kAdmitChunk >= n) return;
  u32* words = reinterpret_cast<u32*>(av.counters);
  const int64_t base = (int64_t)blockIdx.x * kAdmitChunk + threadIdx.x;
  bool on[kAdmitItems];
  AdmitPos pos[kAdmitItems];
  u32 w0[kAdmitItems], w1[kAdmitItems];
#pragma unroll
  for (int j = 0; j < kAdmitItems; ++j) {
    const int64_t i = base + (int64_t)j * kBlock;
    on[j] = i < n && slots[i] == kNoSlot;
    pos[j] = admit_pos(on[j] ? sanitize_key(keys[i]) : 0ull, av.log2);
  }
#pragma unroll
  for (int j = 0; j < kAdmitItems; ++j) {
    if (!on[j]) continue;
    w0[j] = words[pos[j].c0 >> 2];
    w1[j] = words[pos[j].c1 >> 2];
  }
#pragma unroll
  for (int j = 0; j < kAdmitItems; ++j) {
    if (!on[j]) continue;
    admit_bump(words + (pos[j].c0 >> 2), (int)(pos[j].c0 & 3u) * 8, w0[j]);
    admit_bump(words + (pos[j].c1 >> 2), (int)(pos[j].c1 & 3u) * 8, w1[j]);
  }
}

__global__ void __launch_bounds__(kBlock) k_admit_insert(TableView t, AdmitView av,
                                                         const u64* __restrict__ keys,
                                                         const int64_t* n_dev, int64_t n_host,
                                                         int64_t n_max, u32* __restrict__ slots) {
  const int64_t n = dev_count(n_dev, n_host, n_max);
  if ((int64_t)blockIdx.x * kAdmitChunk >= n) return;
  const int64_t base = (int64_t)blockIdx.x * kAdmitChunk + threadIdx.x;
  bool on[kAdmitItems];
  u64 key[kAdmitItems];
  AdmitPos pos[kAdmitItems];
  unsigned int c0[kAdmitItems], c1[kAdmitItems];
// ... 71 lines not shown
```

### csrc/hip/table_common.h

```cpp
#pragma once
#include <cstdlib>
#include <cstring>
#include <type_traits>

#include "kernels.h"
#include "hip_util.h"

namespace xflow {
namespace hip {

constexpr int kGroupGridCap = 8192;

constexpr int kScanBlock = 1024;

__device__ __forceinline__ u32 probe(const TableView& t, u64 key, bool insert, bool& claimed) {
  u64 s = table_home(t, fmix64(key));
  const int stride = t.L.stride;
  for (u64 n = 0; n < t.probe_limit; ++n) {
    u64* kp = reinterpret_cast<u64*>(t.words + s * (u64)stride);
    u64 cur = *kp;
    if (cur == key) return (u32)s;
    if (cur == kEmptyKey) {
      if (!insert) return kNoSlot;
      u64 prev = atomicCAS((unsigned long long*)kp, (unsigned long long)kEmptyKey,
                           (unsigned long long)key);
      if (prev == kEmptyKey) { claimed = true; return (u32)s; }
      if (prev == key) return (u32)s;
    }
    s = table_next(t, s);
  }
  if (insert) *t.overflow = 1u;
  return kNoSlot;
}

struct PackedLane {
  int P, K, g, p;
  bool on;
  int64_t first, stride;
};

__device__ __forceinline__ PackedLane packed_lane(int P) {
  PackedLane r;
  r.P = P;
  r.K = kWave / P;
  const int lane = threadIdx.x % kWave;
  r.g = lane / P;
  r.p = lane - r.g * P;
  r.on = r.g < r.K;
  const int64_t waves = (int64_t)(blockDim.x / kWave);
  r.first = ((int64_t)blockIdx.x * waves + threadIdx.x / kWave) * r.K + r.g;
  r.stride = (int64_t)gridDim.x * waves * r.K;
  return r;
}

struct RowPre {
  u64 key = 0;
  u32 flag = 1;
  float s0 = 0.0f, s1 = 0.0f;
};

__device__ __forceinline__ RowPre row_pre(const u32* __restrict__ words, u32 slot, int p,
                                          const TableLayout& L) {
  RowPre r;
  if (slot == kNoSlot) return r;
  const u32* sp = words + (u64)slot * L.stride;
  r.key = *reinterpret_cast<const u64*>(sp);
  if (L.has_flag) r.flag = sp[L.flag_word];
  if (L.opt == kFTRL) {
    const float2 nz = *reinterpret_cast<const float2*>(sp + 2 + 2 * p);
    r.s0 = nz.x;
    r.s1 = nz.y;
  } else {
    r.s0 = __uint_as_float(sp[2 + p]);
  }
  return r;
}

__device__ __forceinline__ RowPre row_stash(const float2* __restrict__ stash,
                                            const u64* __restrict__ keys, int64_t i, int p,
                                            int P) {
  RowPre r;
  const float2 nz = stash[(size_t)i * P + p];
  r.key = keys[i];
  r.flag = nz.x >= 0.0f ? 1u : 0u;
  r.s0 = nz.x >= 0.0f ? nz.x : 0.0f;
  r.s1 = nz.y;
  return r;
}

struct RowPipe {
  int64_t stride, n;
  u32 s_cur, s_nx;
  RowPre r_nx;
  const float2* stash = nullptr;
  const u64* keys = nullptr;
  __device__ __forceinline__ RowPre row(const u32* words, u32 slot, int64_t i, int p,
                                        const TableLayout& L) const {
    return stash ? row_stash(stash, keys, i, p, L.P) : row_pre(words, slot, p, L);
  }
  __device__ __forceinline__ void start(const u32* __restrict__ slots, const u32* words,
                                        int64_t i, int p, const TableLayout& L) {
    s_cur = i < n ? slots[i] : kNoSlot;
    s_nx = i + stride < n ? slots[i + stride] : kNoSlot;
    if (i < n) r_nx = row(words, s_cur, i, p, L);
  }
  __device__ __forceinline__ u32 next(const u32* __restrict__ slots, const u32* words, int64_t i,
                                      int p, const TableLayout& L, RowPre& r) {
    const u32 slot = s_cur;
    r = r_nx;
    s_cur = s_nx;
    if (i + stride < n) r_nx = row(words, s_cur, i + stride, p, L);
    if (i + 2 * stride < n) s_nx = slots[i + 2 * stride];
    return slot;
  }
};

static int packed_grid(int64_t n, int P) {
  const int64_t keys_per_block = (int64_t)(kBlock / kWave) * (kWave / P);
  const int64_t g = (n + keys_per_block - 1) / keys_per_block;
  return (int)(g < 1 ? 1 : (g < kGroupGridCap ? g : kGroupGridCap));
}

__device__ __forceinline__ float norm_grad(float raw, const int32_t* slice_rows, int s) {
  if (!slice_rows) return raw;
  const int32_t r = slice_rows[s];
  return r < (1 << 24) ? raw / (float)r : (float)((double)raw / (double)r);
}

}
}
```

### csrc/include/xflow/backend.h

```cpp
#pragma once

#include <stddef.h>
#include <stdint.h>

#include <memory>
#include <stdexcept>
#include <string>
#include <vector>

#include "xflow/types.h"

namespace xflow {

constexpr u64 kMaxProbe = 1ull << 16;
constexpr int kMaxSegLog2 = 20;

struct TableView {
  u32* words = nullptr;
  u64 cap = 0;
  TableLayout L;
  unsigned long long* size = nullptr;
  u32* overflow = nullptr;
  u64 probe_limit = 0;
  int seg_log2 = 0;
  int level = 0;
  u64 split = 0;
};

XF_HD u64 table_home(const TableView& t, u64 h) {
  const u64 hi = h >> t.seg_log2;
  u64 b = hi & ((1ull << t.level) - 1);
  if (b < t.split) b = hi & ((2ull << t.level) - 1);
  return (b << t.seg_log2) | (h & ((1ull << t.seg_log2) - 1));
}
XF_HD u64 table_next(const TableView& t, u64 s) {
  const u64 m = (1ull << t.seg_log2) - 1;
  return (s & ~m) | ((s + 1) & m);
}

struct ScratchView {
  u64* keys = nullptr;
  unsigned char* stamps = nullptr;
  u64 cap = 0;
  u32 epoch = 1;
  unsigned long long* claims = nullptr;
  u64 rebuild_at = 0;
  unsigned long long* ctl = nullptr;
  bool carry = false;
  float grow = 0.0f;
  int parts = 1;
  int home_bits = 0;
};
constexpr int kMaxParts = 1024;

constexpr int kCountBits = 40;
constexpr int64_t kSeqMask = (1ll << 23) - 1;
XF_HD int64_t encode_count(int64_t count, int64_t seq) {
  return ((seq & kSeqMask) << kCountBits) | (count + 1);
}
constexpr u32 kStampEpochs = 255;
constexpr u64 kScratchHeadroom = 4;
constexpr u64 kScratchMinCap = 1ull << 16;
constexpr int kScratchCtlWords = 8;
constexpr int kCompactChunkLog2 = 12;

struct DedupOut {
  u32* pos = nullptr;
  u64* uniq_keys = nullptr;
  u32* uniq_pos = nullptr;
  int64_t* n_uniq = nullptr;
  u32* overflow = nullptr;
  u32* block_counts = nullptr;
  u32* inv = nullptr;
  int64_t* n_uniq_copy = nullptr;
  unsigned long long* cap_out = nullptr;
  bool lead = false;
};
constexpr int kLeadTile = 1024;
constexpr u32 kLeadBit = 0x80000000u;
constexpr int kLeadMaxFields = 40;

struct CsrOut {
  u32* off = nullptr;
  u32* cnt = nullptr;
  void* ent = nullptr;
  int slog2 = 0;
  const int32_t* rows = nullptr;
  int ew = 0, P = 0;
};
constexpr int csr_row_words(int P) { return (1 + P + 3) & ~3; }

struct MvmDup {
  float* rec = nullptr;
  u32* n = nullptr;
  u32* vmax = nullptr;
  long long* acc = nullptr;
  u32* claim = nullptr;
  int64_t cap = 0;
  int ew = 0;
};

struct FwdArgs {
  BatchView batch;
  MvmDup mdup;
  const u32* pos = nullptr;
  bool lead = false;
  bool red_local = false;
  u32 trash_pos = 0xFFFFFFFFu;
  const float* wpull = nullptr;
  bool fm_vals = false;
  float* grad = nullptr;
  float* pctr = nullptr;
  LossStats* stats = nullptr;
  ModelSpec model;
  int S = 1;
  bool agg_ok = false;
  u64* red_pairs = nullptr;
  u64* red_sorted = nullptr;
  u32* red_hist = nullptr;
  u32* red_tot = nullptr;
  u32* red_count = nullptr;
  int red_nb = 0;
  int red_maxb = 0;
  int64_t red_sorted_words = 0;
  const unsigned long long* red_bcap = nullptr;
  uint64_t red_cap = 0;
  const int64_t* red_nuq = nullptr;
  unsigned long long* red_records = nullptr;
  u32* red_vmax = nullptr;
  u32* red_vmax_next = nullptr;
  u32* red_dup = nullptr;
  u32* red_dup_next = nullptr;
  int red_nsub = 1;
  int red_groups = 0;
  u32* red_masks = nullptr;
  float* red_out = nullptr;
  const u32* red_inv = nullptr;
  const int32_t* red_rows = nullptr;
  const u32* red_rank_offs = nullptr;
  const unsigned char* red_rank_stamps = nullptr;
  u32 red_rank_epoch = 0;
  u32* red_apply_words = nullptr;
  const u32* red_apply_slots = nullptr;
  const float* red_apply_nz = nullptr;
  FtrlParams red_apply_ftrl;
  struct HostSnap* snap = nullptr;
  const u32* snap_mon = nullptr;
  unsigned long long snap_seq = 0;
  bool fm_compact = false;
  float* red_rowv = nullptr;
  CsrOut red_csr;
  u32* fx_bad = nullptr;
};
constexpr int kRedShift = 14;
constexpr int kRedMaxBuckets = 4096;
constexpr int kCsrVecMinShift = 14;
constexpr int red_shift(int nv) {
  return nv == 1 ? kRedShift : (nv == 2 ? kRedShift - 1 : (nv <= 14 ? 10 : (nv <= 28 ? 9 : 8)));
}
constexpr int fmstd_block(int D) { return D <= 10 ? 512 : (D <= 16 ? 256 : 128); }
constexpr int kSegMaxGroups = 2048;
constexpr int64_t fmstd_lds_at(int D, int slots, int maxb) {
  return (int64_t)slots * 8 * (2 + D) + 2 * fmstd_block(D) + (int64_t)maxb * 4 + 1024;
}
constexpr int fmstd_slots(int D) {
  for (int q = 8; q >= 5; --q)
    if (fmstd_lds_at(D, fmstd_block(D) * q / 4, kRedMaxBuckets) <= 80 * 1024)
      return fmstd_block(D) * q / 4;
  return 2 * fmstd_block(D);
}
constexpr int64_t fmstd_lds(int D, int maxb) { return fmstd_lds_at(D, fmstd_slots(D), maxb); }
constexpr int vec_red_max_buckets(int D) {
  return fmstd_lds(D, 2 * kRedMaxBuckets) <= 160 * 1024 &&
                 (160 * 1024) / fmstd_lds(D, 2 * kRedMaxBuckets) ==
                     (160 * 1024) / fmstd_lds(D, kRedMaxBuckets)
             ? 2 * kRedMaxBuckets
             : kRedMaxBuckets;
}
constexpr int fmstd_slots32(int D) {
  for (int q = 16; q >= 5; --q)
    if ((int64_t)(fmstd_block(D) * q / 4) * (4 + 4 * (1 + D) + 1) +
            (int64_t)vec_red_max_buckets(D) * 4 + 2048 <= 80 * 1024)
      return fmstd_block(D) * q / 4;
  return fmstd_slots(D);
}
constexpr int vec_rec_words(int nv) { return (1 + nv + 3) & ~3; }
constexpr int kLrGroupRows = 1024;
constexpr int kFmGroupRows = 1024;
constexpr int kFmStdMinGroupRows = 128;
constexpr int kMvmGroupRows = 512;

struct AdmitView {
  unsigned char* counters = nullptr;
  int log2 = 0;
  int min_count = 1;
};

struct PullArgs {
  TableView table;
  AdmitView admit;
  OptSpec opt;
  const u64* keys = nullptr;
  const int64_t* n_dev = nullptr;
  int64_t n_host = 0;
  int64_t n_max = 0;
  bool insert = true;
  u32* out_slot = nullptr;
  float* out_vals = nullptr;
  const u32* out_map = nullptr;
  int pstride = 1;
  float* out_nz = nullptr;
  float* zero_out = nullptr;
  int zero_width = 1;
  bool fm_vals = false;
  float* out_w = nullptr;
};

constexpr int kMaxGroupSources = 64;
struct SrcGroups {
  const u32* opos = nullptr;
  const u64* oidx = nullptr;
  int nsrc = 0;
  u32 epoch = 0;
  int64_t offs[kMaxGroupSources + 1] = {};
};

struct OwnerGroupArgs {
  const u64* keys = nullptr;
  int64_t n = 0;
// ... 189 lines not shown
};
struct GroupTable {
  std::vector<u64> key;
  std::vector<int64_t> n, pos;
  std::vector<uint64_t> area2;
  std::vector<int64_t> sump;
};
XF_HD double group_auc_term(int64_t n, int64_t pos, uint64_t area2) {
  return ((double)n * (double)area2) / (2.0 * (double)pos * (double)(n - pos));
}
XF_HD double group_cal_term(int64_t sump, int64_t pos) {
  const double d = (double)sump * (1.0 / 4294967296.0) - (double)pos;
  return d < 0 ? -d : d;
}
XF_HD int64_t group_fx(float p) {
  const double d = (double)(p > 0.0f ? p : 0.0f) * 4294967296.0;
  return (int64_t)__builtin_rint(d);
}
XF_HD u64 row_group_key(const BatchView& b, int64_t r, int field) {
  const RowSpan s = row_span(b, r);
  if (!b.fgid) return field >= 0 && field < s.len ? b.keys[s.at(field)] : kNoGroup;
  for (int j = 0; j < s.len; ++j)
    if (b.fgid[s.at(j)] == field) return b.keys[s.at(j)];
  return kNoGroup;
}

constexpr int kMaxCrosses = 16;
constexpr int kMaxCrossArity = 4;
constexpr int kCrossMaxFields = 64;
struct CrossSpec {
  int n = 0;
  int arity[kMaxCrosses] = {};
  int32_t field[kMaxCrosses][kMaxCrossArity] = {};
  int32_t fgid_base = 0;
};
struct CrossArgs {
  BatchView src;
  int key_bytes = 8;
  CrossSpec spec;
  bool has_seed = false;
  u64 seed = 0;
  u64* keys = nullptr;
  int32_t* fgid = nullptr;
  float* labels = nullptr;
  int32_t* row_ptr = nullptr;
  bool field_major_out = false;
  int64_t col_stride_out = 0;
};
inline int64_t cross_out_stride(const CrossArgs& a) {
  return a.col_stride_out > 0 ? a.col_stride_out
                              : (a.src.col_stride > 0 ? a.src.col_stride : a.src.rows);
}
inline void check_cross_args(const CrossArgs& a) {
  const BatchView& s = a.src;
  const CrossSpec& x = a.spec;
  if (x.n < 1 || x.n > kMaxCrosses) throw std::invalid_argument("cross_rows: 1 to 16 crosses");
  for (int c = 0; c < x.n; ++c) {
    if (x.arity[c] < 2 || x.arity[c] > kMaxCrossArity)
      throw std::invalid_argument("cross_rows: a cross has 2 to 4 fields");
    for (int i = 0; i < x.arity[c]; ++i)
      if (x.field[c][i] < 0) throw std::invalid_argument("cross_rows: a negative field id");
  }
  if (s.rows < 0 || s.nnz < 0 || s.nnz + (int64_t)x.n * s.rows > 0x7fffffffll)
    throw std::invalid_argument("cross_rows: bad batch size (nnz + crosses * rows must fit int32)");
  if (a.fgid && !s.fgid && s.nnz > 0) throw std::invalid_argument("cross_rows: field ids out need field ids in");
  if (s.row_ptr) {
    if (!s.fgid && s.nnz > 0)
      throw std::invalid_argument("cross_rows: a CSR batch needs its field ids (fgid)");
    if (a.key_bytes != 8) throw std::invalid_argument("cross_rows: CSR keys are 8 bytes");
    if (a.field_major_out) throw std::invalid_argument("cross_rows: a CSR batch stays CSR");
    if (a.has_seed) throw std::invalid_argument("cross_rows: a CSR batch is shuffled by shuffle_rows first");
    if (!a.row_ptr) throw std::invalid_argument("cross_rows: a CSR batch needs row_ptr out");
  } else {
    if (s.nnz_per_row <= 0 || s.nnz != s.rows * s.nnz_per_row)
      throw std::invalid_argument("cross_rows: fixed width needs nnz == rows * nnz_per_row");
    if (s.col_stride > 0) {
      if (s.col_stride < s.rows) throw std::invalid_argument("cross_rows: col_stride < rows");
      if (s.fgid || a.has_seed || a.key_bytes != 8 || !a.field_major_out)
        throw std::invalid_argument("cross_rows: a field-major source has u64 keys, no fgid and "
                                    "no seed, and stays field-major");
      if (s.rows > 0 && a.keys == s.keys && cross_out_stride(a) != s.col_stride)
        throw std::invalid_argument("cross_rows: in place needs the source's col_stride");
    } else {
      if (a.key_bytes != 8 && a.key_bytes != 4)
        throw std::invalid_argument("cross_rows: 4- or 8-byte keys");
      if (s.rows > 0 && s.nnz_per_row + x.n > kCrossMaxFields)
        throw std::invalid_argument("cross_rows: fields + crosses exceed 64");
      if (s.rows > 0 && (const void*)a.keys == (const void*)s.keys)
        throw std::invalid_argument("cross_rows: a row-major source is not crossed in place");
    }
    if (a.field_major_out && cross_out_stride(a) < s.rows)
      throw std::invalid_argument("cross_rows: col_stride_out < rows");
  }
  if ((s.rows > 0 && (!s.labels || !a.labels)) || (s.nnz > 0 && !s.keys) ||
      (s.rows > 0 && !a.keys))
    throw std::invalid_argument("cross_rows: null array");
}
XF_HD void row_cross_keys(const BatchView& b, int64_t r, const CrossSpec& x, u64* out) {
  for (int c = 0; c < x.n; ++c) {
    u64 ops[kMaxCrossArity];
    for (int i = 0; i < x.arity[c]; ++i) ops[i] = row_group_key(b, r, x.field[c][i]);
    out[c] = cross_key(x.field[c], ops, x.arity[c]);
  }
}

class Backend {
 public:
  virtual ~Backend() = default;
  virtual bool is_gpu() const = 0;
  virtual std::string name() const = 0;

  virtual void* alloc(size_t bytes) = 0;
  virtual void free(void* p) = 0;
  virtual void* alloc_stream(size_t bytes) { return alloc(bytes); }
  virtual void free_stream(void* p) { free(p); }
  virtual void memset(void* p, int v, size_t bytes) = 0;
  virtual void fill_u64(u64* p, u64 v, size_t n) = 0;
  virtual void copy_h2d(void* dst, const void* src, size_t bytes) = 0;
  virtual void copy_d2h(void* dst, const void* src, size_t bytes) = 0;
  virtual void copy_d2d(void* dst, const void* src, size_t bytes) = 0;
  virtual void copy_d2h_async(void* dst, const void* src, size_t bytes) { copy_d2h(dst, src, bytes); }
  virtual void copy_h2d_async(void* dst, const void* src, size_t bytes) { copy_h2d(dst, src, bytes); }
  virtual void* staging_alloc(size_t bytes) { return host_alloc(bytes); }
  virtual void staging_free(void* p) { host_free(p); }
  virtual void upload_small(void* dst, const void* src, size_t bytes) = 0;
  virtual void download_small(void* host_dst, const void* src, size_t bytes) = 0;
  virtual void synchronize() = 0;
  virtual void set_stream(void* stream) = 0;
  virtual void* stream() const = 0;
  virtual void bind_thread() {}
  virtual size_t free_memory() const { return ~(size_t)0; }
  virtual void snapshot(HostSnap* dst, const u32* mon, unsigned long long seq) = 0;

  virtual void* host_alloc(size_t bytes) = 0;
  virtual void host_free(void* p) = 0;
  virtual void* event_create() { return nullptr; }
  virtual void event_destroy(void* e) { (void)e; }
  virtual void event_record(void* e) { (void)e; }
  virtual bool event_done(void* e) { (void)e; return true; }
  void event_spin(void* e) {
    while (!event_done(e)) {
    }
  }

  virtual void stage_begin(int s) { (void)s; }
  virtual void* stage_pinned(int s, size_t bytes) = 0;
  virtual void stage_copy(int s, void* dst, size_t off, size_t bytes) = 0;
  virtual void stage_commit(int s) { (void)s; }
  virtual void stage_release(int s) { (void)s; }

  virtual void table_clear(const TableView& t) = 0;
  virtual void dedup(const u64* keys, int64_t nnz, ScratchView s, DedupOut o) = 0;
  virtual void table_pull(const PullArgs& a) = 0;
  virtual void table_apply(const ApplyArgs& a) = 0;
  virtual void forward_backward(const FwdArgs& a) = 0;
  virtual void slice_masks(const BatchView& b, const u32* pos, u32* tmask) = 0;
  virtual void parse_text(const TextParseArgs& a) = 0;
  virtual bool remaps_positions() const { return false; }
  virtual void remap_pos(u32* pos, int64_t nnz, const u32* inv, u32 none) {
    (void)pos, (void)nnz, (void)inv, (void)none;
    throw std::runtime_error("remap_pos is not supported by this backend");
  }
  virtual void bucket(const BucketArgs& a) = 0;
  virtual bool partitioned_dedup() const { return false; }
  virtual void partition_counts(const ScratchView& s, const u32* chunk_offsets,
                                const int64_t* n_uniq, int64_t* counts, int64_t seq) {
    (void)s, (void)chunk_offsets, (void)n_uniq, (void)counts, (void)seq;
    throw std::runtime_error("partitioned dedup is not supported by this backend");
  }
  virtual bool owner_grouping() const { return false; }
  virtual void owner_group(const OwnerGroupArgs& a) {
    (void)a;
    throw std::runtime_error("owner grouping is not supported by this backend");
  }
  virtual bool csr_exchange() const { return false; }
  virtual void scan_u32(const u32* in, u32* out, const int64_t* n_dev, int64_t n_max) {
    (void)in, (void)out, (void)n_dev, (void)n_max;
    throw std::runtime_error("scan_u32 is not supported by this backend");
  }
  virtual void csr_pack(const u32* off, const u32* cnt, const void* src, const u32* doff,
                        const int64_t* n_dev, int64_t n_max, void* dst, int entry_bytes) {
    (void)off, (void)cnt, (void)src, (void)doff, (void)n_dev, (void)n_max, (void)dst,
        (void)entry_bytes;
    throw std::runtime_error("csr_pack is not supported by this backend");
  }
  virtual void csr_totals(const int64_t* counts, int world, bool encoded, const u32* doff,
                          int64_t* totals) {
    (void)counts, (void)world, (void)encoded, (void)doff, (void)totals;
    throw std::runtime_error("csr_totals is not supported by this backend");
  }
  virtual void gather_grads(const GatherGradArgs& a) = 0;
  virtual void scatter_rows(const float* src, float* dst, const u32* map,
                            const int64_t* n_dev, int64_t n_max, int width,
                            float* zero_out = nullptr, int zero_width = 1) = 0;
  virtual void synth_batch(const SynthArgs& a) = 0;
  virtual void field_major(const void* src, void* dst, int64_t rows, int F, int elem_bytes,
                           bool widen = false) = 0;
  virtual void unpack_block(const UnpackArgs& a) = 0;
  virtual void shuffle_rows(const ShuffleArgs& a) = 0;
  virtual void cross_rows(const CrossArgs& a) = 0;
  virtual int64_t table_export(const TableView& t, u64* keys_out, u32* words_out,
                               int64_t max_rows) = 0;
  virtual int64_t table_nonzero(const TableView& t, const OptSpec& o) = 0;
  virtual void table_import(const TableView& t, const u64* keys, const u32* words,
                            int64_t n) = 0;
  virtual void delta_mark(u32* bits, int L, const u64* keys, const int64_t* n_dev,
                          int64_t n_host, int64_t n_max) = 0;
  virtual int64_t table_export_marked(const TableView& t, const u32* bits, int L, u64* keys_out,
                                      u32* words_out, int64_t max_rows) = 0;
  virtual int64_t delta_popcount(const u32* bits, int L) = 0;
  virtual void table_prefill(const TableView& t, int64_t n, u64 seed) = 0;
  virtual void table_split(const TableView& t, u64 s0, u64 k) = 0;
  virtual void table_prune(const TableView& t, const OptSpec& o, float max_n,
                           unsigned long long* dropped) = 0;
  virtual void* table_reserve(size_t max_bytes, bool growable) = 0;
  virtual void* table_commit(void* base, size_t bytes) = 0;
  virtual void table_release(void* base) = 0;
  virtual size_t table_committed() const = 0;
  virtual bool table_in_place() const { return true; }
  virtual EvalMetrics eval_metrics(const float* pctr, const float* labels, int64_t n) = 0;
  virtual GroupedEval eval_grouped(const float* pctr, const float* labels, const u64* groups,
                                   int64_t n, GroupTable* table) = 0;
  virtual void row_group_keys(const BatchView& b, int field, u64* out) = 0;
};

std::unique_ptr<Backend> make_cpu_backend();
std::unique_ptr<Backend> make_hip_backend(int device);
bool hip_backend_available();

}
```

### csrc/include/xflow/engine.h

```cpp
#pragma once

#include <memory>
#include <string>
#include <vector>

#include "xflow/backend.h"
#include "xflow/device_buffer.h"

namespace xflow {

struct EngineConfig {
  ModelSpec model;
  OptSpec opt;
  int table_log2_cap = 20;
  int64_t max_rows = 1 << 16;
  int64_t max_nnz = 1 << 22;
  int max_slices = 1;
  bool sum_slices = false;
  double scratch_factor = 2.5;
  int device = -1;
  bool table_grow = true;
  double grow_load = 0.8;
  double grow_start = 0.6;
  int max_log2_cap = 0;
  int monitor_lag = 2;
  int owner_group = 0;
  bool csr = true;
  int admit_min_count = 1;
  int admit_log2 = 0;
  bool lead_handoff = true;
  bool scratch_carry = true;
  bool red_rank = true;
  bool red_local = true;
  bool red_apply = true;
  bool delta_track = false;
  int delta_log2 = 0;
};

struct DeltaStats {
  int log2 = 0;
  int64_t bits_set = 0;
  bool needs_full = false;
};

struct ScratchStats {
  int64_t capacity = 0;
  int64_t occupancy = 0;
  int64_t rebuilds = 0;
  int64_t carried = 0;
};

struct StepInputs {
  bool gpu = false;
  bool remaps = false;
  bool red_pairs = false;
  bool red_rowv = false;
  bool fm_vals = false;
  bool csr = true;
  bool sum_slices = false;
  int kind = kLR;
  int fm_math = kFmReference;
  TableLayout L;
  double scratch_cap = 0.0, max_nnz = 0.0, max_rows = 0.0;
  int pstride = 1, slice_cap = 1;
  int kdim = 1;
  bool lead_handoff = true;
  bool field_major = false;
  double rows = 0.0, fields = 0.0;
  bool red_rank = true;
  bool red_local = true;
  bool red_apply = true;
};

enum class GradPath : int { kCsr = 0, kUniqueLR, kUniqueFmBC, kUniqueRows, kSlotSums, kSlotRows };
const char* grad_path_name(GradPath g);

struct StepPlan {
  int S = 1, groups = 1, Sf = 1;
  int csr_slog2 = -1;
  bool csr_rows = false;
  GradPath grad = GradPath::kSlotRows;
  bool masks = false;
  bool upos = false;
  bool lr16 = false;
  bool lr16s = false;
  bool uqm = false;
  bool fmu = false;
  bool fm_keep_w = false;
  bool mvmu = false, fsu = false, rowu = false;
  bool grpst = false;
  bool uq = false;
  bool lead = false;
  bool red_rank = false;
  bool red_local = false;
  bool red_apply = false;
};

StepPlan plan_step(const StepInputs& in, int S);

class Engine {
 public:
  explicit Engine(const EngineConfig& cfg);
  ~Engine();
  Engine(const Engine&) = delete;
  Engine& operator=(const Engine&) = delete;

  const EngineConfig& config() const { return cfg_; }
  Backend& backend() { return *be_; }
  bool is_gpu() const { return be_->is_gpu(); }
  void set_stream(void* s) { be_->set_stream(s); }
  void synchronize() { be_->synchronize(); }

  void train_step(const BatchView& b);
  void eval_step(const BatchView& b, float* pctr);

  void push_host(const std::vector<u64>& keys, const std::vector<float>& grads);
  void prefill(int64_t n, uint64_t seed);
  void download_small(void* host_dst, const void* src, size_t bytes) {
    be_->download_small(host_dst, src, bytes);
  }
  std::vector<float> pull_host(const std::vector<u64>& keys);

  void w_prepare(const BatchView& b, int world, int64_t* counts_out, u64* send_keys_out,
                 int wb = 0, int64_t seq = -1);
  void s_pull(const u64* recv_keys, int64_t n, float* out_vals, bool insert = true, int buf = 0,
              const std::vector<int64_t>& src_offsets = {}, bool keep_weights = false);
  void w_forward(const BatchView& b, const float* pulled, int64_t n_send, float* pctr, int wb = 0);
  void w_forward_backward(const BatchView& b, const float* pulled, int64_t n_send,
                          float* grads_out, u32* masks_out, int S_global = 0, int wb = 0,
                          int group = 0);
  int csr_slog2(int S) const { return plan(S).csr_slog2; }
  StepInputs step_inputs() const;
  StepPlan plan(int S) const { return plan_step(step_inputs(), S); }
  StepPlan plan(int S, int64_t rows, int64_t fields, bool field_major) const {
    StepInputs in = step_inputs();
    in.rows = (double)rows;
    in.fields = (double)fields;
    in.field_major = field_major;
    return plan_step(in, S);
  }
  int csr_entry_bytes() const {
    return csr_full_rows() ? 4 * csr_row_words(table_.L.P) : (fm_vals_ ? 12 : 8);
  }
  bool csr_full_rows() const {
    return (cfg_.model.kind == kFM && cfg_.model.fm_math == kFmStandard) ||
           (cfg_.model.kind == kMVM && cfg_.model.kernel_dim() >= 2);
  }
  void w_forward_backward_csr(const BatchView& b, const float* pulled, int64_t n_send,
                              int S_global, int wb, bool pack, u32* cnt_out, void* ent_out,
                              const int64_t* counts, int world, bool encoded, int64_t* totals_out);
  void s_apply_csr(const u64* recv_keys, const u32* recv_cnt, const void* recv_ent,
                   const std::vector<int64_t>& src_offsets, int S, int buf = 0);
  void s_apply(const u64* recv_keys, const float* recv_grads, const u32* recv_masks,
               const std::vector<int64_t>& src_offsets, int S, int buf = 0);
  void w_finish();

  EvalMetrics eval_metrics(const float* pctr, const float* labels, int64_t n) {
    return be_->eval_metrics(pctr, labels, n);
  }
  GroupedEval eval_grouped(const float* pctr, const float* labels, const u64* groups, int64_t n,
                           GroupTable* table = nullptr) {
    return be_->eval_grouped(pctr, labels, groups, n, table);
  }
  void row_group_keys(const BatchView& b, int field, u64* out) {
    if (!b.fgid && b.row_ptr)
      throw std::invalid_argument("row_group_keys: a CSR batch needs its field ids (fgid)");
    be_->row_group_keys(b, field, out);
  }

  void shuffle_rows(const BatchView& src, u64 seed, u64* keys, int32_t* fgid, float* labels,
                    int32_t* row_ptr, bool field_major_out, int key_bytes = 8);

  void cross_rows(const CrossArgs& a);

  LossStats read_stats(bool reset, int which = 0);
  int64_t n_unique();
  int64_t table_size();
  int64_t scratch_capacity();
  int64_t batch_capacity();
  ScratchStats scratch_stats();
  uint64_t table_capacity() const { return table_.cap; }
  size_t table_bytes() const { return table_bytes_; }
  bool overflowed();
  int64_t table_growths() const { return growths_; }
  int64_t csr_steps() const { return csr_steps_; }
  void csr_debug(std::vector<u32>& off, std::vector<u32>& cnt, std::vector<u32>& words);
  std::vector<u64> unique_keys();
  struct RedGeometry {
    int base = 0, shift = 0, buckets = 0, maxb = 0, nsub = 1, nb = 0;
    int64_t nuq = 0, needed = 0;
  };
  RedGeometry red_geometry(int S, int64_t nuq = -1);
  int64_t table_splits() const { return splits_; }
  size_t admit_bytes() const { return admit_.counters ? (size_t)1 << admit_.log2 : 0; }
  int admit_log2() const { return admit_.counters ? admit_.log2 : 0; }
  std::vector<uint8_t> admit_counts(const std::vector<u64>& keys);
  void admit_export(uint8_t* dst);
  void admit_import(const uint8_t* src);
  std::vector<u32> server_slots(int buf);
  std::vector<int64_t> table_geometry() const {
    return {table_.seg_log2, table_.level, (int64_t)table_.split,
            (int64_t)(table_.cap >> table_.seg_log2)};
  }
  size_t table_committed() const;
  double grow_seconds() const { return grow_s_; }
  int64_t monitor_waits() const { return monitor_waits_; }
  double monitor_wait_seconds() const { return monitor_wait_s_; }
  void count_records(bool on);
  int64_t take_records();
  void grow_table(int log2_cap);
  int64_t prune(float max_n = -1.0f);
  int64_t pruned_keys() const { return pruned_keys_; }
  void end_step();
  int64_t nonzero_weights() { return be_->table_nonzero(table_, cfg_.opt); }
  int pstride() const { return cfg_.model.pstride(); }
  int value_width() const { return vstride_; }
  int grad_width() const { return sharded_fm_compact() ? 2 : pstride(); }
  int slices_of(const BatchView& b) const;
  static constexpr int kSliceGroup = 32;
  static int slice_groups(int S) { return S <= kSliceGroup ? 1 : (S + kSliceGroup - 1) / kSliceGroup; }
  static int group_slices(int S, int group) {
    if (S <= kSliceGroup) return S;
    const int n = S - group * kSliceGroup;
    return n >= kSliceGroup ? kSliceGroup : (n < 2 ? 2 : n);
  }

  void export_table(std::vector<u64>& keys, std::vector<u32>& words);
  void import_table(const std::vector<u64>& keys, const std::vector<u32>& words);
  void export_into(u64* keys, u32* words, int64_t n);
  void import_from(const u64* keys, const u32* words, int64_t n);
  int state_words() const { return table_.L.stride - 2; }
  const TableLayout& layout() const { return table_.L; }
  void save(const std::string& path);
  void load(const std::string& path);
  int64_t delta_count();
  void delta_export(std::vector<u64>& keys, std::vector<u32>& words);
  void save_delta(const std::string& path);
  void delta_clear();
  DeltaStats delta_stats();
  int delta_log2() const { return delta_log2_; }
  bool delta_needs_full() const { return delta_bits_ && delta_needs_full_; }

  std::vector<int64_t> parse_text(const char* text, int64_t n, u64* keys, int32_t* fgid,
                                  int32_t* row_ptr, float* labels, int64_t max_rows,
                                  int64_t max_nnz, int64_t row_mod = 1);

  BatchView synth_batch(const SynthArgs& a, int64_t slice_rows);
  BatchView stage_host_batch(const BatchView& host);
  BatchView stage_host_batch_async(const BatchView& host);
  void stage_release();

 private:
  static const EngineConfig& validated(const EngineConfig& cfg);
  EngineConfig cfg_;
  std::unique_ptr<Backend> be_;
  TableView table_;
  struct TableRange {
    Engine* e = nullptr;
    ~TableRange() {
      if (e) e->be_->table_release(e->table_.words);
    }
  } table_range_;
  AdmitView admit_;
  size_t table_bytes_ = 0;
  ScratchView scratch_;
  DeviceBuffer<unsigned char> admit_counters_;
  DeviceBuffer<u32> delta_bits_;
  int delta_log2_ = 0;
  bool delta_needs_full_ = false;
  uint64_t delta_gen_ = 0;
  void delta_mark(const u64* keys, const int64_t* n_dev, int64_t n) {
    if (delta_bits_) be_->delta_mark(delta_bits_, delta_log2_, keys, n_dev, n, n);
  }
  int64_t delta_to_device(DeviceBuffer<u64>& dk, DeviceBuffer<u32>& dw);
  DeviceBuffer<u64> scratch_keys_;
  DeviceBuffer<unsigned char> scratch_stamps_;
  DeviceBuffer<unsigned long long> scratch_claims_, scratch_ctl_;

  template <typename Sink>
  void d2h_stream(const void* src, size_t bytes, Sink sink);
  template <typename Fill>
  void h2d_stream(void* dst, size_t bytes, Fill fill);
  void table_from_device(const u64* dk, const u32* dw, int64_t n);
  DeviceBuffer<char, Mem::kStaging> stage_io_[2];
  void ensure_host_staging(int64_t n);
  void ensure_server_capacity(int64_t n, int buf = 0);
  struct WorkerSet {
    DeviceBuffer<u32> pos;
    DeviceBuffer<u32> uniq_pos;
    DeviceBuffer<u32> inv;
    DeviceBuffer<int64_t> n_uniq;
    DeviceBuffer<u32> send_pos;
    const u32* send_map = nullptr;
    bool inv_valid = false;
    DeviceBuffer<unsigned long long> bcap;
  };
  WorkerSet wset_[2];
  WorkerSet* ws_ = &wset_[0];
  void use_worker_set(int wb);
  DeviceBuffer<u64> own_keys_;
  int64_t own_fill_ = 0;
  int own_nsrc_ = 0;
  u32 own_epoch_ = 0;
  bool group_entries(const u64* recv_keys, int64_t n, int buf,
                     const std::vector<int64_t>& src_offsets);
  const int32_t* slice_rows_dev(const BatchView& b, int S);
  BatchView group_view(const BatchView& b, int S, int k, const u32*& pos) const;
  int slice_cap_ = 1;
  void dedup_(const BatchView& b, int parts = 1, u64* uniq_keys_out = nullptr,
              bool want_inv = false, int64_t* n_copy = nullptr, bool lead = false);
  bool sharded_fm_compact() const {
    return red_pairs_ && cfg_.model.kind == kFM && cfg_.model.fm_math == kFmReference &&
           (double)scratch_.cap * slice_cap_ * pstride() < 4294967295.0;
  }
  bool fm_vals_ = false;
  int vstride_ = 1;
  const float* pulled_weights(int buf, int64_t off) const;

  DeviceBuffer<u64> uniq_keys_;
  DeviceBuffer<u32> uniq_slot_;
  DeviceBuffer<u32> block_counts_;
  DeviceBuffer<u32> mon_;
  u32* overflow_ = nullptr;
  DeviceBuffer<float> wpull_;
  DeviceBuffer<float> grad_;
  DeviceBuffer<u32> tmask_;
  DeviceBuffer<u64> red_pairs_;
  DeviceBuffer<u64> red_sorted_;
  DeviceBuffer<u32> red_hist_;
  DeviceBuffer<u32> red_tot_;
  DeviceBuffer<u32> red_count_;
  DeviceBuffer<float> red_rowv_;
  DeviceBuffer<float> lr_grad_;
  DeviceBuffer<float> lr_nz_;
  int64_t nnz_seen_ = 0;
  DeviceBuffer<u32> lr_mask_;
  DeviceBuffer<float> fm_grad_;
  DeviceBuffer<float> row_grad_;
  DeviceBuffer<float> fm_w_;
  int red_nb_ = 0;
  int red_nsub_ = 1;
  int red_maxb_ = 0;
  int red_groups_ = 0;
  void set_reduction(FwdArgs& fa) const;
  PullArgs pull_args(const u64* keys, const int64_t* n_dev, int64_t n, bool insert,
                     u32* out_slot) const;
  ApplyArgs apply_args(const u64* keys, const u32* slots, const int64_t* n_dev, int64_t n,
                       int S) const;
  FwdArgs train_fwd_args(const BatchView& b, const u32* pos, int S) const;
  FwdArgs eval_fwd_args(const BatchView& b, float* pctr) const;
  PullArgs begin_fused_step(const BatchView& b, bool want_inv, bool upos, bool lead = false);
  template <typename Source>
  void apply_by_source(const ApplyArgs& base, const std::vector<int64_t>& src_offsets, int buf,
                       bool stash, const char* need_weights, Source source);
  DeviceBuffer<u32> csr_off_;
  DeviceBuffer<u32> csr_cnt_;
  DeviceBuffer<float> csr_vent_;
  DeviceBuffer<float> mdup_rec_;
  DeviceBuffer<long long> mdup_acc_;
  DeviceBuffer<u32> mdup_claim_;
  int mdup_ew_ = 0;
  int64_t csr_steps_ = 0;
  void train_step_csr(const BatchView& b, int S, int slog2);
  DeviceBuffer<u32> csr_doff_;
  StreamBuffer<u32> csr_long_;
  u32* csr_long_list(int64_t n);
  StreamBuffer<u32> csr_roff_;
  void csr_forward_backward(const BatchView& b, int slog2, const int32_t* srows, bool normalise);
  bool reduction_masks(bool unique_positions) const;
  void ensure_inv();
  DeviceBuffer<LossStats> stats_;
  DeviceBuffer<int64_t> bucket_ws_;
  DeviceBuffer<int32_t> slice_rows_;
  int64_t cached_rows_ = -1, cached_slice_rows_ = -1;
  int cached_S_ = -1;
  int64_t last_nsend_ = 0;

  struct StageSet {
    DeviceBuffer<u64> keys;
    DeviceBuffer<int32_t> rowptr;
    DeviceBuffer<int32_t> fgid;
    DeviceBuffer<float> labels;
  };
  StageSet aset_[2];
  int astage_next_ = 0, astage_last_ = -1;
  DeviceBuffer<u64> st_keys_;
  DeviceBuffer<int32_t> st_rowptr_;
  DeviceBuffer<int32_t> st_fgid_;
  DeviceBuffer<float> st_labels_;

 public:
  static constexpr int kSrvBufs = 64;
 private:
  struct SrvBuf {
    DeviceBuffer<u32> slots;
    int64_t n = 0;
    const u64* keys = nullptr;
    DeviceBuffer<float> nz;
    bool nz_fresh = false;
    const float* vals = nullptr;
    DeviceBuffer<float> w;
    bool w_valid = false;
    DeviceBuffer<u32> own_pos;
    DeviceBuffer<u64> own_idx;
    SrcGroups grp;
    uint64_t delta_gen = 0;
  };
  SrvBuf srv_[kSrvBufs];
  void stale_stashes() {
    for (SrvBuf& b : srv_) b.nz_fresh = false;
  }
  void mark_stale_buffer(SrvBuf& sb, const u64* keys, int64_t n) {
    if (!delta_bits_ || sb.delta_gen == delta_gen_ || n <= 0) return;
    delta_mark(keys, nullptr, n < sb.n ? n : sb.n);
    sb.delta_gen = delta_gen_;
  }
  bool lr16_layout() const;

  static constexpr int kSnaps = 64;
  HostBuffer<HostSnap> snaps_;
  int64_t snap_adds_[kSnaps] = {};
  bool snap_carried_ = false;
  bool snap_ready(int64_t seq) const;
  void close_snapshot();
  void attach_snapshot(ApplyArgs& aa);
  void attach_snapshot(FwdArgs& fa, int64_t n_max);
  template <typename Args>
  void attach_snapshot_to(Args& a, int64_t n_max);
  int64_t snap_seq_ = 0;
  int64_t snap_seen_ = 0;
  int64_t known_size_ = 0;
  int64_t known_adds_ = 0;
  int64_t queued_adds_ = 0;
  int64_t growths_ = 0, splits_ = 0, monitor_waits_ = 0;
  DeviceBuffer<unsigned long long> pruned_dev_;
  int64_t pruned_keys_ = 0;
  double grow_s_ = 0.0;
  u64 max_segs_ = 0;
  double monitor_wait_s_ = 0.0;
  DeviceBuffer<float> grp_nz_;
  DeviceBuffer<unsigned long long> rec_count_;
  DeviceBuffer<u32> red_vmax_;
  DeviceBuffer<u32> text_ws_;
  DeviceBuffer<long long> text_counts_;
  DeviceBuffer<u32> shuf_len_;
  mutable int vmax_parity_ = 0;
  bool rec_on_ = false;
  int log2_cap_ = 0, max_log2_cap_ = 31;
  void poll_snapshots(int64_t wait_upto);
  void guard_inserts(int64_t n);
  void remap_server_slots();
  u64 segments_for(double keys, double u0, double u1) const;
  static constexpr double kHardLoad = 0.9;
  void split_to(u64 nseg);

  DeviceBuffer<u64> host_keys_dev_;
  DeviceBuffer<float> host_vals_dev_;
  DeviceBuffer<u32> host_slots_dev_;
};

}
```

### csrc/python/module.cpp

```cpp
#include <pybind11/numpy.h>
#include <pybind11/pybind11.h>
#include <pybind11/stl.h>

#include <algorithm>
#include <atomic>
#include <charconv>
#include <cstdint>
#include <cstdio>
#include <cstring>
#include <thread>
#include <vector>
#include <string>

#include "../comm/async_ps.h"
#include "../comm/rccl_comm.h"
#include "../comm/sharded_step.h"
#include "xflow/engine.h"
#include "xflow/reader.h"
#include "xflow/trainer.h"

namespace py = pybind11;
using namespace xflow;

namespace {

template <typename T>
T* P(uintptr_t a) {
  return reinterpret_cast<T*>(a);
}

template <typename T>
py::array_t<T> to_np(const std::vector<T>& v) {
  py::array_t<T> a((py::ssize_t)v.size());
  if (!v.empty()) std::memcpy(a.mutable_data(), v.data(), sizeof(T) * v.size());
  return a;
}

py::dict block_to_dict(const CsrBlock& b) {
  py::dict d;
  d["row_ptr"] = to_np(b.row_ptr);
  d["keys"] = to_np(b.keys);
  d["fgid"] = to_np(b.fgid);
  d["labels"] = to_np(b.labels);
  d["max_fgid"] = b.max_fgid;
  return d;
}

py::dict stats_dict(const LossStats& s) {
  py::dict d;
  d["ln_loss"] = s.ln_loss;
  d["log2_lik"] = s.log2_lik;
  d["rows"] = s.rows;
  d["positives"] = s.positives;
  return d;
}

ModelSpec model_from(py::dict d) {
  ModelSpec m;
  if (d.contains("kind")) m.kind = d["kind"].cast<int>();
  if (d.contains("v_dim")) m.v_dim = d["v_dim"].cast<int>();
  if (d.contains("fm_math")) m.fm_math = d["fm_math"].cast<int>();
  if (d.contains("mvm_math")) m.mvm_math = d["mvm_math"].cast<int>();
  if (d.contains("fm_mfma")) m.fm_mfma = d["fm_mfma"].cast<bool>() ? 1 : 0;
  return m;
}

OptSpec opt_from(py::dict d) {
  OptSpec o;
  if (d.contains("kind")) o.kind = d["kind"].cast<int>();
  if (d.contains("alpha")) o.ftrl.alpha = d["alpha"].cast<float>();
  if (d.contains("beta")) o.ftrl.beta = d["beta"].cast<float>();
  if (d.contains("lambda1")) o.ftrl.lambda1 = d["lambda1"].cast<float>();
  if (d.contains("lambda2")) o.ftrl.lambda2 = d["lambda2"].cast<float>();
  if (d.contains("lr")) o.sgd.lr = d["lr"].cast<float>();
  if (d.contains("sgd_v_init")) o.sgd.v_init = d["sgd_v_init"].cast<float>();
  if (d.contains("v_init_scale")) o.v_init_scale = d["v_init_scale"].cast<float>();
  if (d.contains("seed")) o.seed = d["seed"].cast<uint64_t>();
  return o;
}

py::dict plan_dict(const StepPlan& p) {
  py::dict d;
  d["S"] = p.S;
  d["groups"] = p.groups;
  d["Sf"] = p.Sf;
  d["csr_slog2"] = p.csr_slog2;
  d["csr_rows"] = p.csr_rows;
  d["grad"] = grad_path_name(p.grad);
  d["masks"] = p.masks;
  d["upos"] = p.upos;
  d["lr16"] = p.lr16;
  d["lr16s"] = p.lr16s;
  d["uqm"] = p.uqm;
  d["fmu"] = p.fmu;
  d["fm_keep_w"] = p.fm_keep_w;
  d["mvmu"] = p.mvmu;
  d["fsu"] = p.fsu;
  d["rowu"] = p.rowu;
  d["grpst"] = p.grpst;
  d["uq"] = p.uq;
  d["lead"] = p.lead;
  d["red_rank"] = p.red_rank;
  return d;
}

StepInputs inputs_from(py::dict d) {
  StepInputs in;
  const ModelSpec m = model_from(d["model"].cast<py::dict>());
  const OptSpec o = opt_from(d["opt"].cast<py::dict>());
  in.kind = m.kind;
  in.fm_math = m.fm_math;
  in.L = TableLayout::make(m, o);
  in.pstride = m.pstride();
  auto flag = [&](const char* k, bool def) { return d.contains(k) ? d[k].cast<bool>() : def; };
  in.gpu = flag("gpu", true);
  in.remaps = flag("remaps", in.gpu);
  in.red_pairs = flag("red_pairs", in.gpu);
  in.red_rowv = flag("red_rowv", in.gpu && (m.kind == kMVM || (m.kind == kFM && m.fm_math == kFmStandard)));
  in.fm_vals = flag("fm_vals", in.gpu && m.kind == kFM && m.fm_math == kFmReference);
  in.csr = flag("csr", true);
  in.sum_slices = flag("sum_slices", false);
  in.max_nnz = d.contains("max_nnz") ? d["max_nnz"].cast<double>() : (double)(1 << 22);
  in.scratch_cap = d.contains("scratch_cap") ? d["scratch_cap"].cast<double>() : 4.0 * in.max_nnz;
  in.slice_cap = d.contains("slice_cap") ? d["slice_cap"].cast<int>() : Engine::kSliceGroup;
  in.max_rows = d.contains("max_rows") ? d["max_rows"].cast<double>() : (double)(1 << 16);
  in.kdim = m.kernel_dim();
  in.lead_handoff = flag("lead_handoff", true);
  in.red_rank = flag("red_rank", true);
  in.red_local = flag("red_local", true);
  in.red_apply = flag("red_apply", true);
  in.field_major = flag("field_major", false);
  in.rows = d.contains("rows") ? d["rows"].cast<double>() : 0.0;
  in.fields = d.contains("fields") ? d["fields"].cast<double>() : 0.0;
  return in;
}

}

PYBIND11_MODULE(_xflow_native, m) {
  m.doc() = "xflow-amd native core: HBM hash-table engine, gfx950 kernels, libffm reader";

  m.def("hip_available", &hip_backend_available);
  m.def(
      "plan_step",
      [](py::dict inputs, int S, bool batch) {
        const StepPlan p = plan_step(inputs_from(inputs), S);
        py::dict d = plan_dict(p);
        if (batch) {
          d["red_local"] = p.red_local;
          d["red_apply"] = p.red_apply;
        }
        return d;
      },
      py::arg("inputs"), py::arg("S"), py::arg("batch") = false);
  m.def("write_pred", [](const std::string& path, py::array_t<float> pctr,
                         py::array_t<int32_t> labels) {
    const int64_t n = pctr.size();
    if (labels.size() != n) throw std::invalid_argument("write_pred: lengths differ");
    const float* p = pctr.data();
    const int32_t* y = labels.data();
    py::gil_scoped_release nogil;
    const int64_t per = 1 << 18;
    const int64_t nchunk = (n + per - 1) / per;
    std::vector<std::string> out((size_t)nchunk);
    std::atomic<int64_t> next{0};
    auto work = [&]() {
      for (int64_t c = next++; c < nchunk; c = next++) {
        const int64_t lo = c * per, hi = lo + per < n ? lo + per : n;
        std::string& b = out[(size_t)c];
        b.resize((size_t)(hi - lo) * 24);
        char* q = &b[0];
        for (int64_t i = lo; i < hi; ++i) {
          q = std::to_chars(q, q + 16, (double)p[i], std::chars_format::general, 6).ptr;
          const int yi = y[i] ? 1 : 0;
          *q++ = '\t';
          *q++ = (char)('0' + (1 - yi));
          *q++ = '\t';
          *q++ = (char)('0' + yi);
          *q++ = '\n';
        }
        b.resize((size_t)(q - &b[0]));
      }
    };
    const unsigned hw = std::thread::hardware_concurrency();
    const int nt = (int)std::min<int64_t>(nchunk, hw ? (hw < 16 ? hw : 16) : 4);
    std::vector<std::thread> th;
    for (int t = 1; t < nt; ++t) th.emplace_back(work);
    work();
    for (std::thread& t : th) t.join();
    FILE* f = std::fopen(path.c_str(), "wb");
    if (!f) throw std::runtime_error("write_pred: cannot open " + path);
    bool ok = true;
    for (const std::string& b : out) ok = ok && std::fwrite(b.data(), 1, b.size(), f) == b.size();
    ok = (std::fclose(f) == 0) && ok;
    if (!ok) throw std::runtime_error("write_pred: write failed " + path);
  });
  m.def("shuffle_permutation", [](int64_t n, uint64_t seed) {
    if (n < 0) throw std::invalid_argument("shuffle_permutation: n < 0");
    py::array_t<int64_t> out((py::ssize_t)n);
    int64_t* o = out.mutable_data();
    const ShufflePerm pi = shuffle_perm((u64)n, seed);
    for (int64_t i = 0; i < n; ++i) o[i] = (int64_t)pi.at((u64)i);
    return out;
  }, py::arg("n"), py::arg("seed"));
  m.def("feature_hash", [](py::bytes b) {
    std::string s = b;
    return feature_hash(s.data(), s.size());
  });
  m.def("parse_libffm", [](py::bytes b) {
    std::string s = b;
    CsrBlock blk;
    parse_libffm(s.data(), s.size(), blk);
    return block_to_dict(blk);
  });
  m.def("reference_auc", [](py::array_t<int32_t> labels, py::array_t<float> pctr) {
    auto l = labels.unchecked<1>();
    auto p = pctr.unchecked<1>();
    std::vector<std::pair<int, float>> v;
    for (py::ssize_t i = 0; i < l.shape(0); ++i) v.emplace_back(l(i), p(i));
    EvalResult r = reference_auc(v);
    py::dict d;
    d["logloss_printed"] = r.logloss_printed;
    d["ln_logloss"] = r.ln_logloss;
    d["auc"] = r.auc;
    d["tp"] = r.tp;
    d["n"] = r.n;
    d["line"] = r.line;
    return d;
  });

  py::class_<BatchView>(m, "BatchView")
      .def(py::init<>())
      .def_property("keys", [](const BatchView& b) { return (uintptr_t)b.keys; },
                    [](BatchView& b, uintptr_t v) { b.keys = P<const u64>(v); })
      .def_property("row_ptr", [](const BatchView& b) { return (uintptr_t)b.row_ptr; },
                    [](BatchView& b, uintptr_t v) { b.row_ptr = P<const int32_t>(v); })
      .def_property("fgid", [](const BatchView& b) { return (uintptr_t)b.fgid; },
                    [](BatchView& b, uintptr_t v) { b.fgid = P<const int32_t>(v); })
      .def_property("labels", [](const BatchView& b) { return (uintptr_t)b.labels; },
                    [](BatchView& b, uintptr_t v) { b.labels = P<const float>(v); })
      .def_readwrite("rows", &BatchView::rows)
      .def_readwrite("nnz", &BatchView::nnz)
      .def_readwrite("nnz_per_row", &BatchView::nnz_per_row)
      .def_readwrite("slice_rows", &BatchView::slice_rows)
      .def_readwrite("col_stride", &BatchView::col_stride);

  py::class_<RcclComm>(m, "RcclComm")
      .def_static("unique_id",
                  []() {
                    auto v = RcclComm::unique_id();
                    return py::bytes(reinterpret_cast<const char*>(v.data()), v.size());
                  })
      .def(py::init([](py::bytes id, int world, int rank, int device) {
             std::string s = id;
             std::vector<uint8_t> v(s.begin(), s.end());
             py::gil_scoped_release nogil;
             return new RcclComm(v, world, rank, device);
           }),
           py::arg("id"), py::arg("world"), py::arg("rank"), py::arg("device"))
      .def_property_readonly("world", &RcclComm::world)
      .def_property_readonly("rank", &RcclComm::rank)
      .def("alltoallv",
           [](RcclComm& c, uintptr_t send, std::vector<int64_t> sc, uintptr_t recv,
              std::vector<int64_t> rc, int elem_bytes, uintptr_t stream) {
             c.alltoallv(P<const void>(send), sc, P<void>(recv), rc, elem_bytes, stream);
           })
      .def("alltoall",
           [](RcclComm& c, uintptr_t send, uintptr_t recv, int64_t count, int elem_bytes,
              uintptr_t stream) { c.alltoall(P<const void>(send), P<void>(recv), count,
                                             elem_bytes, stream); })
      .def("alltoallv_group",
           [](RcclComm& c, std::vector<uintptr_t> sends, std::vector<uintptr_t> recvs,
              std::vector<int> elem_bytes, std::vector<std::vector<int64_t>> sc,
              std::vector<std::vector<int64_t>> rc, uintptr_t stream) {
             std::vector<RcclComm::A2AOp> ops;
             const size_t n = sends.size();
             if (recvs.size() != n || elem_bytes.size() != n || sc.size() != n || rc.size() != n)
               throw std::invalid_argument("alltoallv_group: list lengths differ");
             for (size_t i = 0; i < n; ++i)
               ops.push_back({P<const void>(sends[i]), sc[i], P<void>(recvs[i]), rc[i],
                              elem_bytes[i]});
             c.alltoallv_group(ops, stream);
           })
      .def("send_recv",
           [](RcclComm& c, std::vector<int> peers, std::vector<uintptr_t> sends,
              std::vector<int64_t> send_bytes, std::vector<uintptr_t> recvs,
              std::vector<int64_t> recv_bytes, uintptr_t stream) {
             c.send_recv(peers, sends, send_bytes, recvs, recv_bytes, stream);
           })
      .def("abort", &RcclComm::abort);

  py::class_<ShardedStep>(m, "ShardedStep")
      .def(py::init([](Engine& e, RcclComm* comm, int world, int rank, bool early_keys,
                       int staleness) {
             return new ShardedStep(e, comm, world, rank, early_keys, staleness);
           }),
           py::arg("engine"), py::arg("comm"), py::arg("world"), py::arg("rank"),
           py::arg("early_keys") = true, py::arg("staleness") = 0, py::keep_alive<1, 2>(),
           py::keep_alive<1, 3>())
      .def("flush", &ShardedStep::flush, py::call_guard<py::gil_scoped_release>())
      .def_readwrite("p2p_ops", &ShardedStep::p2p_ops)
      .def("train_step",
           [](ShardedStep& s, const BatchView& b, int64_t id, int S, py::object next,
              int64_t next_id, py::object prefetch) {
             BatchView nv;
             const bool has = !next.is_none();
             if (has) nv = next.cast<BatchView>();
             std::function<void()> pf;
             if (!prefetch.is_none()) {
               pf = [prefetch]() {
                 py::gil_scoped_acquire gil;
                 prefetch();
               };
             }
             bool ok;
             {
               py::gil_scoped_release nogil;
               ok = s.train_step(b, id, S, has ? &nv : nullptr, next_id, pf);
             }
             return ok;
           },
           py::arg("batch"), py::arg("id"), py::arg("S"), py::arg("next") = py::none(),
           py::arg("next_id") = 0, py::arg("prefetch") = py::none())
      .def("eval_step",
           [](ShardedStep& s, const BatchView& b, uintptr_t pctr) {
             return s.eval_step(b, P<float>(pctr));
           },
           py::call_guard<py::gil_scoped_release>())
      .def_readwrite("host_waits", &ShardedStep::host_waits)
      .def_readwrite("mid_step_waits", &ShardedStep::mid_step_waits)
      .def_readwrite("buffer_growths", &ShardedStep::buffer_growths)
      .def_readwrite("csr_exchanges", &ShardedStep::csr_exchanges)
      .def_readwrite("csr_waits", &ShardedStep::csr_waits)
      .def_readwrite("csr_wait_s", &ShardedStep::csr_wait_s)
      .def_readwrite("early_key_exchanges", &ShardedStep::early_key_exchanges)
      .def_readwrite("inline_prepares", &ShardedStep::inline_prepares)
      .def_readwrite("empty_steps", &ShardedStep::empty_steps)
      .def_readwrite("bytes_moved", &ShardedStep::bytes_moved)
      .def_readwrite("drop_exchanges", &ShardedStep::drop_exchanges)
      .def_readwrite("host_wait_s", &ShardedStep::host_wait_s)
      .def_readonly("last_send", &ShardedStep::last_send)
      .def_readonly("last_recv", &ShardedStep::last_recv);

  py::class_<AsyncPS>(m, "AsyncPS")
      .def(py::init([](Engine& worker, Engine& server, int world, int rank, int staleness,
                       int slices, std::string name, double timeout_s, int slow_ms,
                       double pair_frac, int device) {
             AsyncPS::Config c;
             c.world = world;
             c.rank = rank;
             c.staleness = staleness;
             c.slices = slices;
             c.name = name;
             c.timeout_s = timeout_s;
             c.slow_ms = slow_ms;
             c.pair_frac = pair_frac;
             c.device = device;
             return new AsyncPS(worker, server, c);
           }),
           py::arg("worker"), py::arg("server"), py::arg("world"), py::arg("rank"),
           py::arg("staleness"), py::arg("slices"), py::arg("name"), py::arg("timeout_s") = 600.0,
           py::arg("slow_ms") = 0, py::arg("pair_frac") = 1.0, py::arg("device") = -1,
           py::keep_alive<1, 2>(), py::keep_alive<1, 3>())
      .def("handle",
           [](const AsyncPS& a) {
             auto v = a.handle();
             return py::bytes(reinterpret_cast<const char*>(v.data()), v.size());
           })
      .def("connect",
           [](AsyncPS& a, std::vector<py::bytes> hs) {
             std::vector<std::vector<uint8_t>> v;
             for (auto& h : hs) {
               std::string s = h;
               v.emplace_back(s.begin(), s.end());
             }
             a.connect(v);
           })
      .def("start", &AsyncPS::start)
      .def("train_step", &AsyncPS::train_step, py::call_guard<py::gil_scoped_release>())
      .def("eval_step",
           [](AsyncPS& a, const BatchView& b, uintptr_t pctr) { return a.eval_step(b, P<float>(pctr)); },
           py::call_guard<py::gil_scoped_release>())
      .def("finish", &AsyncPS::finish, py::call_guard<py::gil_scoped_release>())
      .def("stop", &AsyncPS::stop, py::call_guard<py::gil_scoped_release>())
      .def("log", [](const AsyncPS& a) { return to_np(a.log()); })
      .def_property_readonly("serving", &AsyncPS::serving)
      .def_property_readonly("transport", &AsyncPS::transport)
      .def_property_readonly("csr", &AsyncPS::csr)
      .def_readonly("steps", &AsyncPS::steps)
      .def_readonly("evals", &AsyncPS::evals)
      .def_readwrite("bytes_moved", &AsyncPS::bytes_moved)
      .def_readwrite("max_staleness", &AsyncPS::max_staleness)
      .def_readwrite("max_lead", &AsyncPS::max_lead)
      .def_readwrite("wait_slot_s", &AsyncPS::wait_slot_s)
      .def_readwrite("wait_pull_s", &AsyncPS::wait_pull_s)
      .def_readwrite("sync_s", &AsyncPS::sync_s)
      .def_readonly("served_pulls", &AsyncPS::served_pulls)
      .def_readonly("applied_pushes", &AsyncPS::applied_pushes)
      .def_readonly("server_busy_s", &AsyncPS::server_busy_s);

  py::class_<Engine>(m, "Engine")
      .def(py::init([](py::dict model, py::dict opt, int table_log2_cap, int64_t max_rows,
                       int64_t max_nnz, int max_slices, bool sum_slices, double scratch_factor,
                       int device, bool table_grow, double grow_load, int max_log2_cap,
                       int monitor_lag, int owner_group, double grow_start, bool csr,
                       int admit_min_count, int admit_log2, bool lead_handoff,
                       bool scratch_carry, bool red_rank, bool delta_track, int delta_log2,
                       bool red_local, bool red_apply) {
             EngineConfig c;
             c.red_local = red_local;
             c.red_apply = red_apply;
             c.delta_track = delta_track;
             c.delta_log2 = delta_log2;
             c.red_rank = red_rank;
             c.lead_handoff = lead_handoff;
             c.scratch_carry = scratch_carry;
             c.admit_min_count = admit_min_count;
             c.admit_log2 = admit_log2;
             c.owner_group = owner_group;
             c.csr = csr;
             c.table_grow = table_grow;
             c.grow_load = grow_load;
             c.grow_start = grow_start;
             c.max_log2_cap = max_log2_cap;
             c.monitor_lag = monitor_lag;
             c.model = model_from(model);
             c.opt = opt_from(opt);
             c.table_log2_cap = table_log2_cap;
             c.max_rows = max_rows;
             c.max_nnz = max_nnz;
             c.max_slices = max_slices;
             c.sum_slices = sum_slices;
             c.scratch_factor = scratch_factor;
             c.device = device;
             return new Engine(c);
           }),
           py::arg("model"), py::arg("opt"), py::arg("table_log2_cap") = 20,
           py::arg("max_rows") = 1 << 16, py::arg("max_nnz") = 1 << 22,
           py::arg("max_slices") = 1, py::arg("sum_slices") = false,
           py::arg("scratch_factor") = 2.5, py::arg("device") = -1,
           py::arg("table_grow") = true, py::arg("grow_load") = 0.8, py::arg("max_log2_cap") = 0,
           py::arg("monitor_lag") = 2, py::arg("owner_group") = 0, py::arg("grow_start") = 0.6,
           py::arg("csr") = true, py::arg("admit_min_count") = 1, py::arg("admit_log2") = 0,
           py::arg("lead_handoff") = true, py::arg("scratch_carry") = true,
           py::arg("red_rank") = true, py::arg("delta_track") = false,
           py::arg("delta_log2") = 0, py::arg("red_local") = true,
           py::arg("red_apply") = true)
      .def("delta_count", &Engine::delta_count, py::call_guard<py::gil_scoped_release>())
      .def("delta_export",
           [](Engine& e) {
             std::vector<u64> k;
             std::vector<u32> w;
             {
               py::gil_scoped_release nogil;
               e.delta_export(k, w);
             }
             return py::make_tuple(to_np(k), to_np(w));
           })
      .def("save_delta", &Engine::save_delta, py::call_guard<py::gil_scoped_release>())
      .def_property_readonly("delta_log2", &Engine::delta_log2)
      .def_property_readonly("delta_needs_full", &Engine::delta_needs_full)
      .def("delta_clear", &Engine::delta_clear, py::call_guard<py::gil_scoped_release>())
      .def("delta_stats",
           [](Engine& e) {
             DeltaStats s;
             {
               py::gil_scoped_release nogil;
               s = e.delta_stats();
             }
             py::dict d;
             d["log2"] = s.log2;
             d["bits_set"] = s.bits_set;
             d["needs_full"] = s.needs_full;
             return d;
           })
      .def_property_readonly("admit_bytes", &Engine::admit_bytes)
      .def_property_readonly("admit_log2", &Engine::admit_log2)
      .def("admit_counts",
           [](Engine& e, py::array_t<uint64_t, py::array::c_style | py::array::forcecast> keys) {
             std::vector<u64> k(keys.data(), keys.data() + keys.size());
             return to_np(e.admit_counts(k));
           })
      .def("admit_export",
           [](Engine& e) {
             py::array_t<uint8_t> a((py::ssize_t)e.admit_bytes());
             uint8_t* p = a.mutable_data();
             {
               py::gil_scoped_release nogil;
               e.admit_export(p);
             }
             return a;
           })
      .def("admit_import",
           [](Engine& e, py::array_t<uint8_t, py::array::c_style | py::array::forcecast> a) {
             if ((size_t)a.size() != e.admit_bytes())
               throw std::invalid_argument("admit_import: size mismatch");
             const uint8_t* p = a.data();
             py::gil_scoped_release nogil;
             e.admit_import(p);
           })
      .def("server_slots", [](Engine& e, int buf) { return to_np(e.server_slots(buf)); },
           py::arg("buf") = 0)
      .def_property_readonly("table_growths", &Engine::table_growths)
      .def_property_readonly("csr_steps", &Engine::csr_steps)
      .def("step_plan",
           [](const Engine& e, int S, int64_t rows, int64_t fields, bool field_major) {
             const StepPlan p = e.plan(S, rows, fields, field_major);
             py::dict d = plan_dict(p);
             d["red_local"] = p.red_local;
             d["red_apply"] = p.red_apply;
             return d;
           },
           py::arg("S"), py::arg("rows") = 0, py::arg("fields") = 0, py::arg("field_major") = false)
      .def_property_readonly("table_splits", &Engine::table_splits)
      .def_property_readonly("table_geometry", &Engine::table_geometry)
      .def_property_readonly("table_committed", &Engine::table_committed)
      .def_property_readonly("grow_seconds", &Engine::grow_seconds)
      .def_property_readonly("monitor_waits", &Engine::monitor_waits)
      .def_property_readonly("monitor_wait_seconds", &Engine::monitor_wait_seconds)
      .def("parse_text",
           [](Engine& e, uintptr_t text, int64_t n, uintptr_t keys, uintptr_t fgid,
              uintptr_t row_ptr, uintptr_t labels, int64_t max_rows, int64_t max_nnz,
              int64_t row_mod) {
             return e.parse_text(P<const char>(text), n, P<u64>(keys), P<int32_t>(fgid),
                                 P<int32_t>(row_ptr), P<float>(labels), max_rows, max_nnz,
                                 row_mod);
           },
           py::arg("text"), py::arg("n"), py::arg("keys"), py::arg("fgid"), py::arg("row_ptr"),
           py::arg("labels"), py::arg("max_rows"), py::arg("max_nnz"), py::arg("row_mod") = 1,
           py::call_guard<py::gil_scoped_release>())
      .def("count_records", &Engine::count_records)
      .def("take_records", &Engine::take_records, py::call_guard<py::gil_scoped_release>())
      .def("grow_table", &Engine::grow_table, py::call_guard<py::gil_scoped_release>())
      .def("prune", &Engine::prune, py::arg("max_n") = -1.0f,
           py::call_guard<py::gil_scoped_release>())
      .def_property_readonly("pruned_keys", &Engine::pruned_keys)
      .def("end_step", &Engine::end_step, py::call_guard<py::gil_scoped_release>())
      .def_property_readonly("is_gpu", &Engine::is_gpu)
      .def_property_readonly("backend_name", [](Engine& e) { return e.backend().name(); })
      .def_property_readonly("pstride", &Engine::pstride)
      .def_property_readonly("grad_width", &Engine::grad_width)
      .def_property_readonly("value_width", &Engine::value_width)
      .def_property_readonly("P", [](Engine& e) { return e.config().model.P(); })
      .def_property_readonly("state_words", &Engine::state_words)
      .def_property_readonly("table_capacity", &Engine::table_capacity)
      .def_property_readonly("table_bytes", &Engine::table_bytes)
      .def_property_readonly("layout", [](Engine& e) {
        const TableLayout& L = e.layout();
        py::dict d;
        d["kind"] = e.config().model.kind;
        d["P"] = L.P;
        d["opt"] = L.opt;
        d["stride"] = L.stride;
        return d;
      })
      .def("set_stream", [](Engine& e, uintptr_t s) { e.set_stream(reinterpret_cast<void*>(s)); })
      .def("synchronize", &Engine::synchronize, py::call_guard<py::gil_scoped_release>())
      .def("train_step", &Engine::train_step, py::call_guard<py::gil_scoped_release>())
      .def("eval_step",
           [](Engine& e, const BatchView& b, uintptr_t pctr) { e.eval_step(b, P<float>(pctr)); },
           py::call_guard<py::gil_scoped_release>())
      .def("slices_of", &Engine::slices_of)
      .def_static("slice_groups", &Engine::slice_groups)
      .def_static("group_slices", &Engine::group_slices)
      .def_readonly_static("slice_group", &Engine::kSliceGroup)
      .def("push_host",
           [](Engine& e, py::array_t<uint64_t> keys, py::array_t<float> grads) {
             std::vector<u64> k(keys.data(), keys.data() + keys.size());
             std::vector<float> g(grads.data(), grads.data() + grads.size());
             e.push_host(k, g);
           })
      .def("eval_metrics",
           [](Engine& e, uintptr_t pctr, uintptr_t labels, int64_t n) {
             EvalMetrics m;
             {
               py::gil_scoped_release nogil;
               m = e.eval_metrics(P<const float>(pctr), P<const float>(labels), n);
             }
             EvalResult r = eval_result(m);
             py::dict d;
             d["n"] = m.n;
             d["tp"] = m.tp;
             d["area"] = m.area;
             d["log2_sum"] = m.log2_sum;
             d["ln_sum"] = m.ln_sum;
             d["logloss_printed"] = r.logloss_printed;
             d["ln_logloss"] = r.ln_logloss;
             d["auc"] = r.auc;
             d["line"] = r.line;
             return d;
           })
      .def("eval_grouped",
           [](Engine& e, uintptr_t pctr, uintptr_t labels, uintptr_t groups, int64_t n,
              bool per_group) {
             GroupedEval g;
             GroupTable t;
             {
               py::gil_scoped_release nogil;
               g = e.eval_grouped(P<const float>(pctr), P<const float>(labels),
                                  P<const u64>(groups), n, per_group ? &t : nullptr);
             }
             py::dict d;
             d["n"] = g.n;
             d["n_nogroup"] = g.n_nogroup;
             d["groups"] = g.groups;
             d["groups_used"] = g.groups_used;
             d["rows_used"] = g.rows_used;
             d["gauc_num"] = g.gauc_num;
             d["cal_abs"] = g.cal_abs;
             if (per_group) {
               py::dict p;
               p["key"] = to_np(t.key);
               p["n"] = to_np(t.n);
               p["pos"] = to_np(t.pos);
               p["area2"] = to_np(t.area2);
               p["sump"] = to_np(t.sump);
               d["per_group"] = p;
             }
             return d;
           },
           py::arg("pctr"), py::arg("labels"), py::arg("groups"), py::arg("n"),
           py::arg("per_group") = false)
      .def("row_group_keys",
           [](Engine& e, const BatchView& b, int field, uintptr_t out) {
             e.row_group_keys(b, field, P<u64>(out));
           },
           py::call_guard<py::gil_scoped_release>())
      .def("shuffle_rows",
           [](Engine& e, const BatchView& b, uint64_t seed, uintptr_t keys, uintptr_t fgid,
              uintptr_t labels, uintptr_t row_ptr, bool field_major_out, int key_bytes) {
             e.shuffle_rows(b, seed, P<u64>(keys), P<int32_t>(fgid), P<float>(labels),
                            P<int32_t>(row_ptr), field_major_out, key_bytes);
           },
           py::arg("batch"), py::arg("seed"), py::arg("keys"), py::arg("fgid"), py::arg("labels"),
           py::arg("row_ptr"), py::arg("field_major_out"), py::arg("key_bytes") = 8,
           py::call_guard<py::gil_scoped_release>())
      .def("cross_rows",
           [](Engine& e, const BatchView& b, const std::vector<std::vector<int32_t>>& crosses,
              int32_t fgid_base, py::object seed, uintptr_t keys, uintptr_t fgid, uintptr_t labels,
              uintptr_t row_ptr, bool field_major_out, int key_bytes, int64_t col_stride_out) {
             CrossArgs a;
             a.src = b;
             a.key_bytes = key_bytes;
             if (crosses.size() > (size_t)kMaxCrosses)
               throw std::invalid_argument("cross_rows: 1 to 16 crosses");
             a.spec.n = (int)crosses.size();
             for (size_t c = 0; c < crosses.size(); ++c) {
               if (crosses[c].size() > (size_t)kMaxCrossArity)
                 throw std::invalid_argument("cross_rows: a cross has 2 to 4 fields");
               a.spec.arity[c] = (int)crosses[c].size();
               for (size_t i = 0; i < crosses[c].size(); ++i) a.spec.field[c][i] = crosses[c][i];
             }
             a.spec.fgid_base = fgid_base;
             a.has_seed = !seed.is_none();
             if (a.has_seed) a.seed = seed.cast<uint64_t>();
             a.keys = P<u64>(keys);
             a.fgid = P<int32_t>(fgid);
             a.labels = P<float>(labels);
             a.row_ptr = P<int32_t>(row_ptr);
             a.field_major_out = field_major_out;
             a.col_stride_out = col_stride_out;
             py::gil_scoped_release nogil;
             e.cross_rows(a);
// ... 319 lines not shown
```

### xflow_amd/config.py

```python
from __future__ import annotations

import dataclasses
import os
from dataclasses import dataclass, field

MODEL_KINDS = {"lr": 0, "fm": 1, "mvm": 2}
MODEL_NAMES = {v: k for k, v in MODEL_KINDS.items()}
OPT_KINDS = {"ftrl": 0, "sgd": 1}
FM_MATH = {"reference": 0, "standard": 1}
MVM_MATH = {"compat": 0, "fixed": 1}


def model_kind(m) -> int:
    if isinstance(m, int):
        if m not in MODEL_NAMES:
            raise ValueError(f"model index must be 0 (LR), 1 (FM) or 2 (MVM), got {m}")
        return m
    m = str(m).lower()
    if m in ("0", "1", "2"):
        return int(m)
    if m not in MODEL_KINDS:
        raise ValueError(f"unknown model {m!r}; expected lr/fm/mvm")
    return MODEL_KINDS[m]


MAX_CROSSES = 16
MAX_CROSS_ARITY = 4


def check_crosses(crosses) -> list:
    out = [tuple(int(f) for f in c) for c in crosses]
    if not 1 <= len(out) <= MAX_CROSSES:
        raise ValueError(f"crosses: 1 to {MAX_CROSSES} crosses, got {len(out)}")
    for c in out:
        if not 2 <= len(c) <= MAX_CROSS_ARITY:
            raise ValueError(f"cross {c}: a cross has 2 to {MAX_CROSS_ARITY} fields")
        if min(c) < 0 or max(c) >= 1 << 31:
            raise ValueError(f"cross {c}: field ids are non-negative int32")
        if len(set(c)) != len(c):
            raise ValueError(f"cross {c}: a field is repeated")
    if len(set(out)) != len(out):
        raise ValueError(f"crosses {out}: a cross is given twice")
    return out


def parse_crosses(text: str) -> list:
    text = (text or "").strip()
    if not text:
        return []
    try:
        raw = [tuple(int(f) for f in c.split("x")) for c in text.split(",")]
    except ValueError:
        raise ValueError(f"--cross {text!r}: crosses are field ids joined by 'x', separated by "
                         f"commas (3x7,1x2x5)") from None
    return check_crosses(raw)


def format_crosses(crosses) -> str:
    return ",".join("x".join(str(f) for f in c) for c in crosses)


@dataclass
class ModelConfig:
    kind: str = "lr"
    v_dim: int = 10
    fm_math: str = "reference"
    mvm_math: str = "compat"
    fm_mfma: bool = False

    def native(self) -> dict:
        return {"kind": model_kind(self.kind), "v_dim": int(self.v_dim),
                "fm_math": FM_MATH[self.fm_math], "mvm_math": MVM_MATH[self.mvm_math],
                "fm_mfma": bool(self.fm_mfma)}

    @property
    def params_per_key(self) -> int:
        k = model_kind(self.kind)
        return 1 if k == 0 else (1 + self.v_dim if k == 1 else self.v_dim)


@dataclass
class OptimConfig:
    kind: str = "ftrl"
    alpha: float = 5e-2
    beta: float = 1.0
    lambda1: float = 5e-5
    lambda2: float = 10.0
    lr: float = 1e-3
    sgd_v_init: float = 1e-3
    v_init_scale: float = 1e-2
    seed: int = 0x5EED

    def native(self) -> dict:
        d = dataclasses.asdict(self)
        d["kind"] = OPT_KINDS[self.kind]
        return d


@dataclass
class EngineConfig:
    table_log2_cap: int = 22
    max_rows: int = 1 << 16
    max_nnz: int = 1 << 22
    max_slices: int = 1
    sum_slices: bool = False
    scratch_factor: float = 2.5
    table_grow: bool = True
    grow_load: float = 0.8
    grow_start: float = 0.6
    max_log2_cap: int = 0
    monitor_lag: int = 2
    owner_group: int = 0
    csr: bool = True
    admit_min_count: int = 1
    admit_log2: int = 0
    lead_handoff: bool = True
    scratch_carry: bool = True
    red_rank: bool = True
    red_local: bool = True
    red_apply: bool = True
    delta_track: bool = False
    delta_log2: int = 0


@dataclass
class TrainConfig:
    train_prefix: str = ""
    test_prefix: str = ""
    epochs: int = 60
    threads: int = 0
    train_block_bytes: int = 2 << 20
    block_rows: int = 0
    fixed_width: bool = True
    resident: bool = False
    shuffle: bool = False
    shuffle_seed: int = 0
    copy_threads: int = 8
    gpu_parse: bool = False
    test_block_bytes: int = 0
    serial_slices: bool = False
    keep_remainder: bool = False
    mvm_predict_compat: bool = False
    init_push: bool = True
    pred_dir: str = "."
    write_pred: bool = True
    checkpoint_dir: str = ""
    save_every: int = 0
    resume_dir: str = ""
    save_delta: bool = False
    delta_full_every: int = 8
    prune_every: int = 0
    prune_max_n: float = -1.0
    gauc_field: int = -1
    crosses: list = field(default_factory=list)
    cross_field_base: int = -1
    metrics_file: str = ""
    async_p2p: bool = False
    async_ps: bool = False
    staleness: int = 1
    model: ModelConfig = field(default_factory=ModelConfig)
    optim: OptimConfig = field(default_factory=OptimConfig)
    engine: EngineConfig = field(default_factory=EngineConfig)

    def resolved_threads(self) -> int:
        if self.threads > 0:
            return self.threads
        hc = int(os.environ.get("XFLOW_HARDWARE_CONCURRENCY", "0") or 0)
        return hc if hc > 0 else (os.cpu_count() or 1)

    def resolved_test_block(self) -> int:
        if self.test_block_bytes > 0:
            return self.test_block_bytes
        return (4 << 20) if model_kind(self.model.kind) == 0 else (2 << 20)
```

### xflow_amd/engine.py

```python
from __future__ import annotations

from dataclasses import dataclass
from typing import Optional

import numpy as np
import torch

from xflow_amd import native
from xflow_amd.config import EngineConfig, ModelConfig, OptimConfig, check_crosses


@dataclass
class Batch:

    keys: torch.Tensor
    labels: torch.Tensor
    row_ptr: Optional[torch.Tensor] = None
    fgid: Optional[torch.Tensor] = None
    nnz_per_row: int = 0
    slice_rows: int = 0
    field_major: bool = False

    @property
    def rows(self) -> int:
        return int(self.labels.numel())

    @property
    def nnz(self) -> int:
        return int(self.keys.numel())

    def view(self):
        n = native.load()
        v = n.BatchView()
        v.keys = self.keys.data_ptr()
        v.labels = self.labels.data_ptr()
        v.row_ptr = self.row_ptr.data_ptr() if self.row_ptr is not None else 0
        v.fgid = self.fgid.data_ptr() if self.fgid is not None else 0
        v.rows = self.rows
        v.nnz = self.nnz
        v.nnz_per_row = self.nnz_per_row
        v.slice_rows = self.slice_rows
        v.col_stride = self.rows if self.field_major else 0
        return v

    def check(self, device: torch.device, compact_ok: bool = False) -> None:
        for name, t, dt in (("keys", self.keys, torch.int64), ("labels", self.labels, torch.float32),
                            ("row_ptr", self.row_ptr, torch.int32), ("fgid", self.fgid, torch.int32)):
            if t is None:
                continue
            if name == "keys" and compact_ok and t.dtype == torch.int32:
                dt = torch.int32
            if t.dtype != dt:
                raise TypeError(f"batch.{name} must be {dt}, got {t.dtype}")
            if t.device != device:
                raise ValueError(f"batch.{name} on {t.device}, engine on {device}")
            if not t.is_contiguous():
                raise ValueError(f"batch.{name} must be contiguous")
        if self.row_ptr is None:
            if self.nnz_per_row <= 0 or self.nnz != self.rows * self.nnz_per_row:
                raise ValueError("fixed-width batch needs nnz == rows * nnz_per_row")
        elif self.row_ptr.numel() != self.rows + 1:
            raise ValueError("row_ptr must have rows+1 entries")
        if self.field_major and self.row_ptr is not None:
            raise ValueError("field-major batches are fixed-width (no row_ptr)")

    def to_field_major(self, engine: "Engine | None" = None) -> "Batch":
        if self.field_major:
            return self
        if self.row_ptr is not None:
            raise ValueError("only fixed-width batches have a field-major form")
        F = self.nnz_per_row
        if engine is not None and F <= 64:
            def t(x, widen=False):
                if x is None:
                    return None
                y = (torch.empty(x.numel(), dtype=torch.int64, device=x.device) if widen
                     else torch.empty_like(x))
                engine._sync_stream()
                engine.native.field_major(x.data_ptr(), y.data_ptr(), self.rows, F,
                                          x.element_size(), widen)
                return y
        else:
            def t(x, widen=False):
                if x is None:
                    return None
                y = x.view(self.rows, F).t().contiguous().view(-1)
                return widen_keys(y) if widen else y
        return Batch(keys=t(self.keys, self.keys.dtype == torch.int32), labels=self.labels,
                     fgid=t(self.fgid), nnz_per_row=F, slice_rows=self.slice_rows,
                     field_major=True)


def widen_keys(keys: torch.Tensor) -> torch.Tensor:
    if keys.dtype == torch.int64:
        return keys
    if keys.dtype != torch.int32:
        raise TypeError(f"keys must be int64 or compact int32, got {keys.dtype}")
    return keys.to(torch.int64) & 0xFFFFFFFF


def shuffle_permutation(n: int, seed: int) -> np.ndarray:
    return native.load().shuffle_permutation(int(n), int(seed) & 0xFFFFFFFFFFFFFFFF)


CROSS_SALT = 0xC3A5C85C97CB3127
_M64 = (1 << 64) - 1


def _fmix64(h: int) -> int:
    h &= _M64
    h ^= h >> 33
    h = (h * 0xFF51AFD7ED558CCD) & _M64
    h ^= h >> 33
    h = (h * 0xC4CEB9FE1A85EC53) & _M64
    h ^= h >> 33
    return h


def cross_keys(fields, ops) -> np.ndarray:
    fields = [int(f) for f in fields]
    if isinstance(ops, np.ndarray):
        a = ops if ops.dtype == np.uint64 else ops.astype(np.int64).view(np.uint64)
    else:
        flat = np.array(ops, dtype=object).reshape(-1)
        a = np.array([int(v) & _M64 for v in flat], dtype=np.uint64)
    a = a.reshape(-1, len(fields))
    out = np.empty(len(a), dtype=np.uint64)
    h0 = _fmix64(CROSS_SALT + len(fields))
    for r, row in enumerate(a.tolist()):
        h = h0
        for f, v in zip(fields, row):
            h = _fmix64(h ^ (f & 0xFFFFFFFF))
            h = _fmix64(h ^ v)
        out[r] = sanitize_key(h)
    return out


def sanitize_key(k: int) -> int:
    return _M64 - 1 if k == _M64 else k


def _device_index(device: torch.device) -> int:
    if device.type == "cpu":
        return -1
    if device.type != "cuda":
        raise ValueError(f"unsupported device {device}")
    return device.index if device.index is not None else torch.cuda.current_device()


class Engine:

    def __init__(self, model: ModelConfig | None = None, optim: OptimConfig | None = None,
                 engine: EngineConfig | None = None, device: str | torch.device = "cpu"):
        self.model = model or ModelConfig()
        self.optim = optim or OptimConfig()
        self.cfg = engine or EngineConfig()
        self.device = torch.device(device)
        if self.device.type == "cuda":
            native.require_hip()
            if self.device.index is None:
                self.device = torch.device("cuda", torch.cuda.current_device())
        n = native.load()
        self._e = n.Engine(self.model.native(), self.optim.native(),
                           table_log2_cap=self.cfg.table_log2_cap, max_rows=self.cfg.max_rows,
                           max_nnz=self.cfg.max_nnz, max_slices=self.cfg.max_slices,
                           sum_slices=self.cfg.sum_slices, scratch_factor=self.cfg.scratch_factor,
                           device=_device_index(self.device), table_grow=self.cfg.table_grow,
                           grow_load=self.cfg.grow_load, max_log2_cap=self.cfg.max_log2_cap,
                           monitor_lag=self.cfg.monitor_lag, owner_group=self.cfg.owner_group,
                           grow_start=self.cfg.grow_start, csr=self.cfg.csr,
                           admit_min_count=self.cfg.admit_min_count,
                           admit_log2=self.cfg.admit_log2,
                           lead_handoff=self.cfg.lead_handoff,
                           scratch_carry=self.cfg.scratch_carry,
                           red_rank=self.cfg.red_rank,
                           red_local=self.cfg.red_local,
                           red_apply=self.cfg.red_apply,
                           delta_track=self.cfg.delta_track,
                           delta_log2=self.cfg.delta_log2)
        if self.is_gpu != (self.device.type == "cuda"):
            raise RuntimeError("native engine backend does not match the requested device")

    @property
    def native(self):
        return self._e

    @property
    def is_gpu(self) -> bool:
        return bool(self._e.is_gpu)

    @property
    def backend_name(self) -> str:
        return self._e.backend_name

    @property
    def pstride(self) -> int:
        return int(self._e.pstride)

    @property
    def grad_width(self) -> int:
        return int(self._e.grad_width)

    @property
    def value_width(self) -> int:
        return int(self._e.value_width)

    @property
    def params_per_key(self) -> int:
        return int(self._e.P)

    def _sync_stream(self) -> None:
        if self.is_gpu:
            self._e.set_stream(torch.cuda.current_stream(self.device).cuda_stream)

    def train_step(self, batch: Batch) -> None:
        batch.check(self.device)
        self._sync_stream()
        self._e.train_step(batch.view())

    def eval_step(self, batch: Batch, pctr: torch.Tensor | None = None) -> torch.Tensor:
        batch.check(self.device)
        if pctr is None:
            pctr = torch.empty(batch.rows, dtype=torch.float32, device=self.device)
        self._sync_stream()
        self._e.eval_step(batch.view(), pctr.data_ptr())
        return pctr

    def train_view(self, view) -> None:
        self._sync_stream()
        self._e.train_step(view)

    def synth_batch(self, rows: int, vocab, zipf_s, hash_space: int, seed: int, step: int,
                    planted_scale: float = 0.3, planted_bias: float = -1.2, slice_rows: int = 0,
                    out: Batch | None = None, field_major: bool = False):
        self._sync_stream()
        kw = {}
        if out is not None:
            kw = dict(keys=out.keys.data_ptr(), labels=out.labels.data_ptr(),
                      fgid=out.fgid.data_ptr() if out.fgid is not None else 0)
        v = self._e.synth_batch(int(rows), [int(x) for x in vocab], [float(s) for s in zipf_s],
                                int(hash_space), int(seed), int(step), float(planted_scale),
                                float(planted_bias), int(slice_rows), field_major=bool(field_major),
                                **kw)
        if out is None:
            return v
        out.nnz_per_row = len(vocab)
        out.slice_rows = int(slice_rows)
        out.field_major = bool(field_major)
        return out

    def push(self, keys, grads) -> None:
        self._e.push_host(np.asarray(keys, dtype=np.uint64),
                          np.asarray(grads, dtype=np.float32).reshape(-1))

    def prefill(self, n: int, seed: int = 0x5eed) -> None:
        self._sync_stream()
        self._e.prefill(int(n), int(seed))

    def admit_bytes(self) -> int:
        return int(self._e.admit_bytes)

    @property
    def admit_log2(self) -> int:
        return int(self._e.admit_log2)

    def admit_counts(self, keys) -> np.ndarray:
        self._sync_stream()
        return self._e.admit_counts(np.ascontiguousarray(keys, dtype=np.uint64))

    def admit_export(self) -> np.ndarray:
        self._sync_stream()
        return self._e.admit_export()

    def admit_import(self, counters: np.ndarray) -> None:
        self._sync_stream()
        self._e.admit_import(np.ascontiguousarray(counters, dtype=np.uint8))

    def delta_stats(self) -> dict:
        self._sync_stream()
        d = self._e.delta_stats()
        return {"log2": int(d["log2"]), "bits_set": int(d["bits_set"]),
                "needs_full": bool(d["needs_full"])}

    @property
    def delta_log2(self) -> int:
        return int(self._e.delta_log2)

    @property
    def delta_needs_full(self) -> bool:
        return bool(self._e.delta_needs_full)

    def delta_count(self) -> int:
        self._sync_stream()
        return int(self._e.delta_count())

    def delta_export(self):
        self._sync_stream()
        return self._e.delta_export()

    def save_delta(self, path: str) -> None:
        self._sync_stream()
        self._e.save_delta(path)

    def delta_clear(self) -> None:
        self._sync_stream()
        self._e.delta_clear()

    def server_slots(self, buf: int = 0) -> np.ndarray:
        self._sync_stream()
        return self._e.server_slots(int(buf))

    def pull(self, keys) -> np.ndarray:
        k = np.asarray(keys, dtype=np.uint64)
        return self._e.pull_host(k).reshape(len(k), self.params_per_key)

    def w_prepare(self, batch: Batch, world: int, counts: torch.Tensor, send_keys: torch.Tensor,
                  wb: int = 0, seq: int = -1):
        batch.check(self.device)
        self._sync_stream()
        self._e.w_prepare(batch.view(), world, counts.data_ptr(), send_keys.data_ptr(), int(wb),
                          int(seq))

    def s_pull(self, recv_keys: torch.Tensor, n: int, out_vals: torch.Tensor,
               insert: bool = True, buf: int = 0, offsets=None, keep_weights: bool = False) -> None:
        self._sync_stream()
        self._e.s_pull(recv_keys.data_ptr(), int(n), out_vals.data_ptr(), insert, int(buf),
                       [int(o) for o in offsets] if offsets is not None else [],
                       bool(keep_weights))

    def w_forward(self, batch: Batch, pulled: torch.Tensor, n_send: int,
# ... 321 lines not shown
```

Baseline: 799.5 million samples/s.

## Fuse dedup compaction write with LR16 table pull into one kernel

Adds a compact_pull kernel that performs the dedup compaction store and the FTRL LR16 table lookup/insert in one pass. Keys stay in shared memory, so the separate uniq-keys readback and one kernel launch are avoided. Pulled weights are written back per scratch-chunk position into wpull. The path is on by default for the one-slice LR lead-handoff step with red_apply, and shared helpers are moved into a common header. A block with more than 1024 hits has to re-read keys from global memory, and it uses extra shared memory that may lower occupancy.

```diff
diff --git a/csrc/engine/engine.cpp b/csrc/engine/engine.cpp
--- a/csrc/engine/engine.cpp
+++ b/csrc/engine/engine.cpp
@@ -428,7 +428,7 @@
 }
 
 void Engine::dedup_(const BatchView& b, int parts, u64* uniq_keys_out, bool want_inv,
-                    int64_t* n_copy, bool lead) {
+                    int64_t* n_copy, bool lead, bool no_write) {
   if (b.nnz > cfg_.max_nnz) throw std::invalid_argument("batch nnz exceeds max_nnz");
   if (b.rows > cfg_.max_rows) throw std::invalid_argument("batch rows exceed max_rows");
   if (b.col_stride > 0 && (b.row_ptr || b.col_stride < b.rows || b.nnz != b.rows * b.nnz_per_row))
@@ -469,6 +469,8 @@
   o.n_uniq_copy = n_copy;
   o.cap_out = ws_->bcap;
   o.lead = lead;
+  o.no_write = no_write;
+  dedup_out_ = o;
   be_->dedup(b.keys, b.nnz, scratch_, o);
 }
 
@@ -507,6 +509,9 @@
   in.red_rank = cfg_.red_rank;
   in.red_local = cfg_.red_local;
   in.red_apply = cfg_.red_apply;
+  in.compact_pull = cfg_.compact_pull;
+  in.admission = admit_.counters != nullptr;
+  in.parts = 1;
   return in;
 }
 
@@ -566,6 +571,8 @@
   p.red_rank = in.red_rank && in.gpu && S == 1 && in.red_pairs && !p.upos && (p.lr16 || p.fmu);
   p.red_local = in.red_local && p.lead;
   p.red_apply = in.red_apply && p.red_local && p.red_rank && p.lr16;
+  p.compact_pull = in.compact_pull && in.gpu && p.lr16 && p.lead && p.red_apply && !in.admission &&
+                   in.parts == 1;
   return p;
 }
 
@@ -803,7 +810,7 @@
   if (fm_keep_w) fm_w_.ensure(*be_, un * ps);
   if (uq) lr_mask_.ensure(*be_, un);
 
-  PullArgs pa = begin_fused_step(b, upos || (uo.buf && !P.red_rank), upos, P.lead);
+  PullArgs pa = begin_fused_step(b, upos || (uo.buf && !P.red_rank), upos, P.lead, P.compact_pull);
   if (fm_keep_w) pa.out_w = fm_w_;
   pa.out_nz = nz;
   if (uo.buf && uo.pull_zeroes) {
@@ -814,7 +821,12 @@
     pa.zero_out = reinterpret_cast<float*>(lr_mask_.get());
     pa.zero_width = 1;
   }
-  be_->table_pull(pa);
+  if (P.compact_pull) {
+    be_->compact_pull(scratch_, dedup_out_, pa);
+    delta_mark(uniq_keys_, ws_->n_uniq, b.nnz);
+  } else {
+    be_->table_pull(pa);
+  }
 
   for (int k = 0; k < ng; ++k) {
     const u32* posk = ws_->pos;
@@ -882,14 +894,17 @@
   end_step();
 }
 
-PullArgs Engine::begin_fused_step(const BatchView& b, bool want_inv, bool upos, bool lead) {
+PullArgs Engine::begin_fused_step(const BatchView& b, bool want_inv, bool upos, bool lead,
+                                  bool compact_pull) {
   if (want_inv) ensure_inv();
   if (lead && upos) throw std::logic_error("begin_fused_step: leader handoff with unique positions");
-  dedup_(b, 1, nullptr, want_inv, nullptr, lead);
+  if (compact_pull && upos) throw std::logic_error("begin_fused_step: compact_pull with unique positions");
+  if (compact_pull) guard_inserts(b.nnz);
+  dedup_(b, 1, nullptr, want_inv, nullptr, lead, compact_pull);
   ws_->inv_valid = false;
   if (upos) be_->remap_pos(ws_->pos, b.nnz, ws_->inv, (u32)scratch_.cap);
-  guard_inserts(b.nnz);
-  delta_mark(uniq_keys_, ws_->n_uniq, b.nnz);
+  if (!compact_pull) guard_inserts(b.nnz);
+  if (!compact_pull) delta_mark(uniq_keys_, ws_->n_uniq, b.nnz);
   PullArgs pa = pull_args(uniq_keys_, ws_->n_uniq, b.nnz, true, uniq_slot_);
   pa.admit = admit_;
   pa.out_vals = wpull_;
diff --git a/csrc/hip/hip_backend.hip b/csrc/hip/hip_backend.hip
--- a/csrc/hip/hip_backend.hip
+++ b/csrc/hip/hip_backend.hip
@@ -183,6 +183,9 @@
     hip::launch_dedup(keys, nnz, s, o, stream_);
   }
   void table_pull(const PullArgs& a) override { hip::launch_table_pull(a, stream_); }
+  void compact_pull(const ScratchView& s, const DedupOut& o, const PullArgs& a) override {
+    hip::launch_compact_pull(s, o, a, stream_);
+  }
   void table_apply(const ApplyArgs& a) override { hip::launch_table_apply(a, stream_); }
   void forward_backward(const FwdArgs& a) override { hip::launch_forward_backward(a, stream_); }
   void slice_masks(const BatchView& b, const u32* pos, u32* tmask) override {
diff --git a/csrc/hip/kernels.h b/csrc/hip/kernels.h
--- a/csrc/hip/kernels.h
+++ b/csrc/hip/kernels.h
@@ -13,6 +13,9 @@
                              const int64_t* n_uniq, int64_t* counts, int64_t seq, hipStream_t st);
 
 void launch_table_pull(const PullArgs& a, hipStream_t st);
+
+void launch_compact_pull(const ScratchView& s, const DedupOut& o, const PullArgs& a,
+                         hipStream_t st);
 
 void launch_table_apply(const ApplyArgs& a, hipStream_t st);
 void launch_owner_group(const OwnerGroupArgs& a, hipStream_t st);
diff --git a/csrc/hip/kernels_compact_pull.hip b/csrc/hip/kernels_compact_pull.hip
--- /dev/null
+++ b/csrc/hip/kernels_compact_pull.hip
@@ -0,0 +1,101 @@
+#include "table_common.h"
+
+namespace xflow {
+namespace hip {
+
+constexpr int kCpList = 1024;
+constexpr int kCpItems = kCpList / kBlock;
+
+__global__ void __launch_bounds__(kBlock) k_compact_pull_lr16(
+    ScratchView sv, const unsigned int* __restrict__ offs, u64* __restrict__ uk,
+    u32* __restrict__ up, u32* __restrict__ inv, TableView t, FtrlParams fp,
+    u32* __restrict__ out_slot, float2* __restrict__ out_nz, float* __restrict__ wpull) {
+  __shared__ u64 l_key[kCpList];
+  __shared__ unsigned short l_loc[kCpList];
+  __shared__ float l_w[kCompactChunk];
+  const u64 base = (u64)blockIdx.x * kCompactChunk + (u64)threadIdx.x * kCompactItems;
+  unsigned int cnt;
+  const unsigned int hit = compact_hits(sv, base, batch_spilled(sv) ? sv.cap : batch_cap(sv), cnt);
+  unsigned int tot;
+  const unsigned int ex = block_exclusive_scan<kBlock>(cnt, &tot);
+  const unsigned int off0 = offs[blockIdx.x];
+  u64 kv[kCompactItems];
+  compact_store(sv, base, hit, (unsigned long long)off0 + ex, kv, uk, up, inv);
+
+  {
+    unsigned int e = ex;
+#pragma unroll
+    for (int j = 0; j < kCompactItems; ++j) {
+      if (!(hit & (1u << j))) continue;
+      if (e < (unsigned int)kCpList) {
+        l_key[e] = kv[j];
+        l_loc[e] = (unsigned short)(threadIdx.x * kCompactItems + j);
+      }
+      ++e;
+    }
+  }
+  __syncthreads();
+  const uint4* slots = reinterpret_cast<const uint4*>(t.words);
+  unsigned int claims = 0;
+  for (unsigned int r0 = 0; r0 < tot; r0 += kCpList) {
+    const unsigned int m = tot - r0 < (unsigned int)kCpList ? tot - r0 : (unsigned int)kCpList;
+    if (r0) {
+#pragma unroll
+      for (int q = 0; q < kCpItems; ++q) {
+        const unsigned int i = threadIdx.x + q * kBlock;
+        if (i >= m) continue;
+        const u64 u = (u64)off0 + r0 + i;
+        l_key[i] = uk[u];
+        l_loc[i] = (unsigned short)(up[u] & (u32)(kCompactChunk - 1));
+      }
+    }
+    uint4 v[kCpItems];
+#pragma unroll
+    for (int q = 0; q < kCpItems; ++q) {
+      const unsigned int i = threadIdx.x + q * kBlock;
+      if (i < m) v[q] = slots[table_home(t, fmix64(sanitize_key(l_key[i])))];
+    }
+#pragma unroll
+    for (int q = 0; q < kCpItems; ++q) {
+      const unsigned int i = threadIdx.x + q * kBlock;
+      if (i >= m) continue;
+      const u64 key = sanitize_key(l_key[i]);
+      const Lr16Pulled r = pull_lr16_resolve(t, fp, key, table_home(t, fmix64(key)), v[q], true, claims);
+      const u64 u = (u64)off0 + r0 + i;
+      out_slot[u] = r.slot;
+      out_nz[u] = r.nz;
+      l_w[l_loc[i]] = r.w;
+    }
+  }
+  __syncthreads();
+  if (hit) {
+    const float4* lw = reinterpret_cast<const float4*>(l_w + threadIdx.x * kCompactItems);
+    float4* wp = reinterpret_cast<float4*>(wpull + base);
+#pragma unroll
+    for (int j = 0; j < kCompactItems / 4; ++j) {
+      const float4 x = lw[j];
+      wp[j] = make_float4(hit & (1u << (4 * j)) ? x.x : 0.0f, hit & (2u << (4 * j)) ? x.y : 0.0f,
+                          hit & (4u << (4 * j)) ? x.z : 0.0f, hit & (8u << (4 * j)) ? x.w : 0.0f);
+    }
+  }
+  block_count_add<kBlock>(t.size, claims);
+}
+
+void launch_compact_pull(const ScratchView& s, const DedupOut& o, const PullArgs& a,
+                         hipStream_t st) {
+  if (a.n_max <= 0) return;
+  if (!a.table.L.lr16() || !a.insert || a.admit.counters || a.out_w || a.zero_out ||
+      !a.out_slot || !a.out_nz || !a.out_vals || a.out_map != o.uniq_pos || a.pstride != 1 ||
+      a.keys != o.uniq_keys || a.n_dev != o.n_uniq || s.parts != 1 || !o.block_counts)
+    throw std::runtime_error("compact_pull: the one-slice LR handoff step only (plan_step)");
+  if (reinterpret_cast<uintptr_t>(a.out_vals) & 15)
+    throw std::runtime_error("compact_pull: out_vals must be 16-byte aligned");
+  const int g = (int)((s.cap + kCompactChunk - 1) / kCompactChunk);
+  hipLaunchKernelGGL(k_compact_pull_lr16, dim3(g), dim3(kBlock), 0, st, s, o.block_counts,
+                     o.uniq_keys, o.uniq_pos, o.inv, a.table, a.opt.ftrl, a.out_slot,
+                     reinterpret_cast<float2*>(a.out_nz), a.out_vals);
+  XF_HIP_CHECK(hipGetLastError());
+}
+
+}
+}
diff --git a/csrc/hip/kernels_dedup.hip b/csrc/hip/kernels_dedup.hip
--- a/csrc/hip/kernels_dedup.hip
+++ b/csrc/hip/kernels_dedup.hip
@@ -2,18 +2,6 @@
 
 namespace xflow {
 namespace hip {
-
-__device__ __forceinline__ u64 active_cap(const ScratchView& sv) {
-  return sv.ctl ? (u64)sv.ctl[0] : sv.cap;
-}
-
-__device__ __forceinline__ u64 batch_cap(const ScratchView& sv) {
-  return sv.ctl ? (u64)sv.ctl[3] : sv.cap;
-}
-
-__device__ __forceinline__ bool batch_spilled(const ScratchView& sv) {
-  return sv.ctl && sv.ctl[4] == (unsigned long long)sv.epoch;
-}
 
 __global__ void k_scratch_maybe_clear(u64* __restrict__ skeys, u64 cap,
                                       const unsigned long long* __restrict__ claims,
@@ -178,24 +166,6 @@
   block_count_add<kBlock>(sv.claims, claimed);
 }
 
-constexpr int kCompactItems = 16;
-constexpr int kCompactChunk = kBlock * kCompactItems;
-static_assert(kCompactChunk == 1 << kCompactChunkLog2, "k_red_sum ranks slots by these chunks");
-
-__device__ __forceinline__ unsigned int compact_hits(const ScratchView& sv, u64 base, u64 cap,
-                                                     unsigned int& cnt) {
-  unsigned int hit = 0;
-  cnt = 0;
-  if (base >= cap) return 0;
-  const uint4 q = *reinterpret_cast<const uint4*>(sv.stamps + base);
-  const u32 w[4] = {q.x, q.y, q.z, q.w};
-  const u32 e = sv.epoch & 0xFFu;
-#pragma unroll
-  for (int j = 0; j < 16; ++j) hit |= (unsigned int)(((w[j >> 2] >> (8 * (j & 3))) & 0xFFu) == e) << j;
-  cnt = __popc(hit);
-  return hit;
-}
-
 __global__ void __launch_bounds__(kBlock) k_compact_count(ScratchView sv,
                                                           unsigned int* __restrict__ counts) {
   const u64 base = (u64)blockIdx.x * kCompactChunk + (u64)threadIdx.x * kCompactItems;
@@ -267,47 +237,8 @@
   unsigned int hit = compact_hits(sv, base, batch_spilled(sv) ? sv.cap : batch_cap(sv), cnt);
   unsigned int tot;
   unsigned int ex = block_exclusive_scan<kBlock>(cnt, &tot);
-  unsigned long long dst = (unsigned long long)offs[blockIdx.x] + ex;
-  u32 iv[kCompactItems];
   u64 kv[kCompactItems];
-  if (hit) {
-    const ulonglong2* kp = reinterpret_cast<const ulonglong2*>(sv.keys + base);
-#pragma unroll
-    for (int q = 0; q < kCompactItems / 2; ++q) {
-      const ulonglong2 v = kp[q];
-      kv[2 * q] = v.x;
-      kv[2 * q + 1] = v.y;
-    }
-  }
-#pragma unroll
-  for (int j = 0; j < kCompactItems; ++j) {
-    iv[j] = 0xFFFFFFFFu;
-    if (!(hit & (1u << j))) continue;
-    u64 s = base + (u64)j;
-    uk[dst] = kv[j];
-    up[dst] = (u32)s;
-    iv[j] = (u32)dst;
-    ++dst;
-  }
-  if (inv && hit) {
-    uint4* ip = reinterpret_cast<uint4*>(inv + base);
-#pragma unroll
-    for (int j = 0; j < kCompactItems / 4; ++j)
-      ip[j] = make_uint4(iv[4 * j], iv[4 * j + 1], iv[4 * j + 2], iv[4 * j + 3]);
-  }
-  const u64 fresh = sv.ctl ? (u64)sv.ctl[2] : 0ull;
-  if (base < fresh) {
-    ulonglong2* kp = reinterpret_cast<ulonglong2*>(sv.keys + base);
-    if (hit && sv.ctl[5]) {
-#pragma unroll
-      for (int j = 0; j < kCompactItems / 2; ++j)
-        kp[j] = make_ulonglong2(hit & (1u << (2 * j)) ? kv[2 * j] : kEmptyKey,
-                                hit & (1u << (2 * j + 1)) ? kv[2 * j + 1] : kEmptyKey);
-    } else {
-#pragma unroll
-      for (int j = 0; j < kCompactItems / 2; ++j) kp[j] = make_ulonglong2(kEmptyKey, kEmptyKey);
-    }
-  }
+  compact_store(sv, base, hit, (unsigned long long)offs[blockIdx.x] + ex, kv, uk, up, inv);
 }
 
 constexpr int kRemapPer = 4;
@@ -410,8 +341,9 @@
                      reinterpret_cast<unsigned long long*>(o.n_uniq), s.claims, s.ctl, s.cap,
                      reinterpret_cast<unsigned long long*>(o.n_uniq_copy), o.cap_out, s.epoch,
                      s.carry);
-  hipLaunchKernelGGL(k_compact_write, dim3(g2), dim3(kBlock), 0, st, s, o.block_counts,
-                     o.uniq_keys, o.uniq_pos, o.inv);
+  if (!o.no_write)
+    hipLaunchKernelGGL(k_compact_write, dim3(g2), dim3(kBlock), 0, st, s, o.block_counts,
+                       o.uniq_keys, o.uniq_pos, o.inv);
   XF_HIP_CHECK(hipGetLastError());
 }
 
diff --git a/csrc/hip/kernels_pull.hip b/csrc/hip/kernels_pull.hip
--- a/csrc/hip/kernels_pull.hip
+++ b/csrc/hip/kernels_pull.hip
@@ -5,7 +5,6 @@
 
 constexpr int kPullItems = 2;
 constexpr int kPullChunk = kBlock * kPullItems;
-constexpr int kLineSlots = 4;
 
 __global__ void __launch_bounds__(kBlock) k_pull_lr16(TableView t, FtrlParams fp,
                                                       const u64* __restrict__ keys,
@@ -18,8 +17,7 @@
                                                       float* __restrict__ zero_out) {
   const int64_t n = dev_count(n_dev, n_host, n_max);
   if ((int64_t)blockIdx.x * kPullChunk >= n) return;
-  const u64 segm = (1ull << t.seg_log2) - 1;
-  uint4* slots = reinterpret_cast<uint4*>(t.words);
+  const uint4* slots = reinterpret_cast<const uint4*>(t.words);
   const int64_t base = (int64_t)blockIdx.x * kPullChunk + threadIdx.x;
   u64 key[kPullItems], s[kPullItems];
   uint4 v[kPullItems];
@@ -45,61 +43,10 @@
   for (int j = 0; j < kPullItems; ++j) {
     int64_t i = base + (int64_t)j * kBlock;
     if (i >= n) continue;
-    u32 slot = kNoSlot;
-    float w = 0.0f;
-    float2 nz = make_float2(0.0f, 0.0f);
-    u64 sj = s[j];
-    int q0 = (int)(sj & (kLineSlots - 1)), q1 = q0 + 1;
-    uint4 ln[kLineSlots];
-#pragma unroll
-    for (int q = 0; q < kLineSlots; ++q) ln[q] = v[j];
-    bool done = false;
-    for (u64 c = 0; c < t.probe_limit && !done;) {
-#pragma unroll
-      for (int q = 0; q < kLineSlots; ++q) {
-        if (q < q0 || q >= q1 || done || c + (u64)(q - q0) >= t.probe_limit) continue;
-        const u64 cur = (u64)ln[q].x | ((u64)ln[q].y << 32);
-        const u64 sq = (sj & ~(u64)(kLineSlots - 1)) + (u64)q;
-        if (cur == key[j]) {
-          slot = (u32)sq;
-          nz = make_float2(__uint_as_float(ln[q].z), __uint_as_float(ln[q].w));
-          w = ftrl_weight(nz.y, nz.x, fp);
-          done = true;
-        } else if (cur == kEmptyKey) {
-          if (!insert) {
-            done = true;
-          } else {
-            const u64 prev = atomicCAS(reinterpret_cast<unsigned long long*>(&slots[sq]),
-                                       (unsigned long long)kEmptyKey, (unsigned long long)key[j]);
-            if (prev == kEmptyKey) {
-              ++claims;
-              slot = (u32)sq;
-              done = true;
-            } else if (prev == key[j]) {
-              slot = (u32)sq;
-              done = true;
-            }
-          }
-        }
-      }
-      if (done) break;
-      c += (u64)(q1 - q0);
-      if (q1 < kLineSlots) {
-        q0 = q1;
-      } else {
-        sj = (sj & ~segm) | (((sj | (u64)(kLineSlots - 1)) + 1) & segm);
-        q0 = 0;
-      }
-      q1 = kLineSlots;
-      const uint4* line = slots + (sj & ~(u64)(kLineSlots - 1));
-#pragma unroll
-      for (int q = 0; q < kLineSlots; ++q)
-        if (q >= q0) ln[q] = line[q];
-    }
-    if (insert && slot == kNoSlot) *t.overflow = 1u;
-    if (out_slot) out_slot[i] = slot;
-    if (out_vals) out_vals[out_map ? (int64_t)orow[j] : i] = w;
-    if (out_nz) out_nz[i] = nz;
+    const Lr16Pulled r = pull_lr16_resolve(t, fp, key[j], s[j], v[j], insert, claims);
+    if (out_slot) out_slot[i] = r.slot;
+    if (out_vals) out_vals[out_map ? (int64_t)orow[j] : i] = r.w;
+    if (out_nz) out_nz[i] = r.nz;
     if (zero_out) zero_out[i] = 0.0f;
   }
   block_count_add<kBlock>(t.size, claims);
diff --git a/csrc/hip/table_common.h b/csrc/hip/table_common.h
--- a/csrc/hip/table_common.h
+++ b/csrc/hip/table_common.h
@@ -121,6 +121,147 @@
   return (int)(g < 1 ? 1 : (g < kGroupGridCap ? g : kGroupGridCap));
 }
 
+__device__ __forceinline__ u64 active_cap(const ScratchView& sv) {
+  return sv.ctl ? (u64)sv.ctl[0] : sv.cap;
+}
+
+__device__ __forceinline__ u64 batch_cap(const ScratchView& sv) {
+  return sv.ctl ? (u64)sv.ctl[3] : sv.cap;
+}
+
+__device__ __forceinline__ bool batch_spilled(const ScratchView& sv) {
+  return sv.ctl && sv.ctl[4] == (unsigned long long)sv.epoch;
+}
+
+constexpr int kCompactItems = 16;
+constexpr int kCompactChunk = kBlock * kCompactItems;
+static_assert(kCompactChunk == 1 << kCompactChunkLog2, "k_red_sum ranks slots by these chunks");
+
+__device__ __forceinline__ unsigned int compact_hits(const ScratchView& sv, u64 base, u64 cap,
+                                                     unsigned int& cnt) {
+  unsigned int hit = 0;
+  cnt = 0;
+  if (base >= cap) return 0;
+  const uint4 q = *reinterpret_cast<const uint4*>(sv.stamps + base);
+  const u32 w[4] = {q.x, q.y, q.z, q.w};
+  const u32 e = sv.epoch & 0xFFu;
+#pragma unroll
+  for (int j = 0; j < 16; ++j) hit |= (unsigned int)(((w[j >> 2] >> (8 * (j & 3))) & 0xFFu) == e) << j;
+  cnt = __popc(hit);
+  return hit;
+}
+
+__device__ __forceinline__ void compact_store(const ScratchView& sv, u64 base, unsigned int hit,
+                                              unsigned long long dst, u64 (&kv)[kCompactItems],
+                                              u64* __restrict__ uk, u32* __restrict__ up,
+                                              u32* __restrict__ inv) {
+  u32 iv[kCompactItems];
+  if (hit) {
+    const ulonglong2* kp = reinterpret_cast<const ulonglong2*>(sv.keys + base);
+#pragma unroll
+    for (int q = 0; q < kCompactItems / 2; ++q) {
+      const ulonglong2 v = kp[q];
+      kv[2 * q] = v.x;
+      kv[2 * q + 1] = v.y;
+    }
+  }
+#pragma unroll
+  for (int j = 0; j < kCompactItems; ++j) {
+    iv[j] = 0xFFFFFFFFu;
+    if (!(hit & (1u << j))) continue;
+    u64 s = base + (u64)j;
+    uk[dst] = kv[j];
+    up[dst] = (u32)s;
+    iv[j] = (u32)dst;
+    ++dst;
+  }
+  if (inv && hit) {
+    uint4* ip = reinterpret_cast<uint4*>(inv + base);
+#pragma unroll
+    for (int j = 0; j < kCompactItems / 4; ++j)
+      ip[j] = make_uint4(iv[4 * j], iv[4 * j + 1], iv[4 * j + 2], iv[4 * j + 3]);
+  }
+  const u64 fresh = sv.ctl ? (u64)sv.ctl[2] : 0ull;
+  if (base < fresh) {
+    ulonglong2* kp = reinterpret_cast<ulonglong2*>(sv.keys + base);
+    if (hit && sv.ctl[5]) {
+#pragma unroll
+      for (int j = 0; j < kCompactItems / 2; ++j)
+        kp[j] = make_ulonglong2(hit & (1u << (2 * j)) ? kv[2 * j] : kEmptyKey,
+                                hit & (1u << (2 * j + 1)) ? kv[2 * j + 1] : kEmptyKey);
+    } else {
+#pragma unroll
+      for (int j = 0; j < kCompactItems / 2; ++j) kp[j] = make_ulonglong2(kEmptyKey, kEmptyKey);
+    }
+  }
+}
+
+constexpr int kLineSlots = 4;
+
+struct Lr16Pulled {
+  u32 slot = kNoSlot;
+  float w = 0.0f;
+  float2 nz = make_float2(0.0f, 0.0f);
+};
+
+__device__ __forceinline__ Lr16Pulled pull_lr16_resolve(const TableView& t, const FtrlParams& fp,
+                                                        u64 key, u64 s, uint4 v0, bool insert,
+                                                        unsigned int& claims) {
+  const u64 segm = (1ull << t.seg_log2) - 1;
+  uint4* slots = reinterpret_cast<uint4*>(t.words);
+  Lr16Pulled r;
+  u64 sj = s;
+  int q0 = (int)(sj & (kLineSlots - 1)), q1 = q0 + 1;
+  uint4 ln[kLineSlots];
+#pragma unroll
+  for (int q = 0; q < kLineSlots; ++q) ln[q] = v0;
+  bool done = false;
+  for (u64 c = 0; c < t.probe_limit && !done;) {
+#pragma unroll
+    for (int q = 0; q < kLineSlots; ++q) {
+      if (q < q0 || q >= q1 || done || c + (u64)(q - q0) >= t.probe_limit) continue;
+      const u64 cur = (u64)ln[q].x | ((u64)ln[q].y << 32);
+      const u64 sq = (sj & ~(u64)(kLineSlots - 1)) + (u64)q;
+      if (cur == key) {
+        r.slot = (u32)sq;
+        r.nz = make_float2(__uint_as_float(ln[q].z), __uint_as_float(ln[q].w));
+        r.w = ftrl_weight(r.nz.y, r.nz.x, fp);
+        done = true;
+      } else if (cur == kEmptyKey) {
+        if (!insert) {
+          done = true;
+        } else {
+          const u64 prev = atomicCAS(reinterpret_cast<unsigned long long*>(&slots[sq]),
+                                     (unsigned long long)kEmptyKey, (unsigned long long)key);
+          if (prev == kEmptyKey) {
+            ++claims;
+            r.slot = (u32)sq;
+            done = true;
+          } else if (prev == key) {
+            r.slot = (u32)sq;
+            done = true;
+          }
+        }
+      }
+    }
+    if (done) break;
+    c += (u64)(q1 - q0);
+    if (q1 < kLineSlots) {
+      q0 = q1;
+    } else {
+      sj = (sj & ~segm) | (((sj | (u64)(kLineSlots - 1)) + 1) & segm);
+      q0 = 0;
+    }
+    q1 = kLineSlots;
+    const uint4* line = slots + (sj & ~(u64)(kLineSlots - 1));
+#pragma unroll
+    for (int q = 0; q < kLineSlots; ++q)
+      if (q >= q0) ln[q] = line[q];
+  }
+  if (insert && r.slot == kNoSlot) *t.overflow = 1u;
+  return r;
+}
+
 __device__ __forceinline__ float norm_grad(float raw, const int32_t* slice_rows, int s) {
   if (!slice_rows) return raw;
   const int32_t r = slice_rows[s];
diff --git a/csrc/include/xflow/backend.h b/csrc/include/xflow/backend.h
--- a/csrc/include/xflow/backend.h
+++ b/csrc/include/xflow/backend.h
@@ -75,6 +75,7 @@
   int64_t* n_uniq_copy = nullptr;
   unsigned long long* cap_out = nullptr;
   bool lead = false;
+  bool no_write = false;
 };
 constexpr int kLeadTile = 1024;
 constexpr u32 kLeadBit = 0x80000000u;
@@ -570,6 +571,10 @@
   virtual void table_clear(const TableView& t) = 0;
   virtual void dedup(const u64* keys, int64_t nnz, ScratchView s, DedupOut o) = 0;
   virtual void table_pull(const PullArgs& a) = 0;
+  virtual void compact_pull(const ScratchView& s, const DedupOut& o, const PullArgs& a) {
+    (void)s, (void)o, (void)a;
+    throw std::runtime_error("compact_pull is not supported by this backend");
+  }
   virtual void table_apply(const ApplyArgs& a) = 0;
   virtual void forward_backward(const FwdArgs& a) = 0;
   virtual void slice_masks(const BatchView& b, const u32* pos, u32* tmask) = 0;
diff --git a/csrc/include/xflow/engine.h b/csrc/include/xflow/engine.h
--- a/csrc/include/xflow/engine.h
+++ b/csrc/include/xflow/engine.h
@@ -33,6 +33,7 @@
   bool red_rank = true;
   bool red_local = true;
   bool red_apply = true;
+  bool compact_pull = true;
   bool delta_track = false;
   int delta_log2 = 0;
 };
@@ -70,6 +71,9 @@
   bool red_rank = true;
   bool red_local = true;
   bool red_apply = true;
+  bool compact_pull = true;
+  bool admission = false;
+  int parts = 1;
 };
 
 enum class GradPath : int { kCsr = 0, kUniqueLR, kUniqueFmBC, kUniqueRows, kSlotSums, kSlotRows };
@@ -94,6 +98,7 @@
   bool red_rank = false;
   bool red_local = false;
   bool red_apply = false;
+  bool compact_pull = false;
 };
 
 StepPlan plan_step(const StepInputs& in, int S);
@@ -308,7 +313,9 @@
   BatchView group_view(const BatchView& b, int S, int k, const u32*& pos) const;
   int slice_cap_ = 1;
   void dedup_(const BatchView& b, int parts = 1, u64* uniq_keys_out = nullptr,
-              bool want_inv = false, int64_t* n_copy = nullptr, bool lead = false);
+              bool want_inv = false, int64_t* n_copy = nullptr, bool lead = false,
+              bool no_write = false);
+  DedupOut dedup_out_;
   bool sharded_fm_compact() const {
     return red_pairs_ && cfg_.model.kind == kFM && cfg_.model.fm_math == kFmReference &&
            (double)scratch_.cap * slice_cap_ * pstride() < 4294967295.0;
@@ -349,7 +356,8 @@
                        int S) const;
   FwdArgs train_fwd_args(const BatchView& b, const u32* pos, int S) const;
   FwdArgs eval_fwd_args(const BatchView& b, float* pctr) const;
-  PullArgs begin_fused_step(const BatchView& b, bool want_inv, bool upos, bool lead = false);
+  PullArgs begin_fused_step(const BatchView& b, bool want_inv, bool upos, bool lead = false,
+                            bool compact_pull = false);
   template <typename Source>
   void apply_by_source(const ApplyArgs& base, const std::vector<int64_t>& src_offsets, int buf,
                        bool stash, const char* need_weights, Source source);
diff --git a/csrc/python/module.cpp b/csrc/python/module.cpp
--- a/csrc/python/module.cpp
+++ b/csrc/python/module.cpp
@@ -129,6 +129,9 @@
   in.red_rank = flag("red_rank", true);
   in.red_local = flag("red_local", true);
   in.red_apply = flag("red_apply", true);
+  in.compact_pull = flag("compact_pull", true);
+  in.admission = flag("admission", false);
+  in.parts = d.contains("parts") ? d["parts"].cast<int>() : 1;
   in.field_major = flag("field_major", false);
   in.rows = d.contains("rows") ? d["rows"].cast<double>() : 0.0;
   in.fields = d.contains("fields") ? d["fields"].cast<double>() : 0.0;
@@ -143,16 +146,17 @@
   m.def("hip_available", &hip_backend_available);
   m.def(
       "plan_step",
-      [](py::dict inputs, int S, bool batch) {
+      [](py::dict inputs, int S, bool batch, bool pull) {
         const StepPlan p = plan_step(inputs_from(inputs), S);
         py::dict d = plan_dict(p);
         if (batch) {
           d["red_local"] = p.red_local;
           d["red_apply"] = p.red_apply;
         }
+        if (pull) d["compact_pull"] = p.compact_pull;
         return d;
       },
-      py::arg("inputs"), py::arg("S"), py::arg("batch") = false);
+      py::arg("inputs"), py::arg("S"), py::arg("batch") = false, py::arg("pull") = false);
   m.def("write_pred", [](const std::string& path, py::array_t<float> pctr,
                          py::array_t<int32_t> labels) {
     const int64_t n = pctr.size();
@@ -406,8 +410,9 @@
                        int monitor_lag, int owner_group, double grow_start, bool csr,
                        int admit_min_count, int admit_log2, bool lead_handoff,
                        bool scratch_carry, bool red_rank, bool delta_track, int delta_log2,
-                       bool red_local, bool red_apply) {
+                       bool red_local, bool red_apply, bool compact_pull) {
              EngineConfig c;
+             c.compact_pull = compact_pull;
              c.red_local = red_local;
              c.red_apply = red_apply;
              c.delta_track = delta_track;
@@ -445,7 +450,7 @@
            py::arg("lead_handoff") = true, py::arg("scratch_carry") = true,
            py::arg("red_rank") = true, py::arg("delta_track") = false,
            py::arg("delta_log2") = 0, py::arg("red_local") = true,
-           py::arg("red_apply") = true)
+           py::arg("red_apply") = true, py::arg("compact_pull") = true)
       .def("delta_count", &Engine::delta_count, py::call_guard<py::gil_scoped_release>())
       .def("delta_export",
            [](Engine& e) {
@@ -509,6 +514,7 @@
              py::dict d = plan_dict(p);
              d["red_local"] = p.red_local;
              d["red_apply"] = p.red_apply;
+             d["compact_pull"] = p.compact_pull;
              return d;
            },
            py::arg("S"), py::arg("rows") = 0, py::arg("fields") = 0, py::arg("field_major") = false)
diff --git a/xflow_amd/config.py b/xflow_amd/config.py
--- a/xflow_amd/config.py
+++ b/xflow_amd/config.py
@@ -119,6 +119,7 @@
     red_rank: bool = True
     red_local: bool = True
     red_apply: bool = True
+    compact_pull: bool = True
     delta_track: bool = False
     delta_log2: int = 0
 
diff --git a/xflow_amd/engine.py b/xflow_amd/engine.py
--- a/xflow_amd/engine.py
+++ b/xflow_amd/engine.py
@@ -176,6 +176,7 @@
                            red_rank=self.cfg.red_rank,
                            red_local=self.cfg.red_local,
                            red_apply=self.cfg.red_apply,
+                           compact_pull=self.cfg.compact_pull,
                            delta_track=self.cfg.delta_track,
                            delta_log2=self.cfg.delta_log2)
         if self.is_gpu != (self.device.type == "cuda"):
```

Measured after the change: 791.2 million samples/s. 0.99x the previous value.
